# lucidrains/DALLE-pytorch

Hardware: NVIDIA B200
Metric: DALL-E fwd+bwd tokens/sec at seq=1280, dim=1024 (higher is better)
Workload: dtype bf16

## Files before the change

dalle_pytorch_b200/_lib.py:

```python
import ctypes
import os
import subprocess
import threading

_HERE = os.path.dirname(os.path.abspath(__file__))
LIB_PATH = os.environ.get('DALLE_B200_LIB') or os.path.join(_HERE, 'libdalle_b200.so')
CSRC = os.path.join(_HERE, 'csrc')

c_int, c_float, c_void_p, c_int64 = ctypes.c_int, ctypes.c_float, ctypes.c_void_p, ctypes.c_int64

F32, BF16 = 0, 1
ATTN_FULL, ATTN_AXIAL_ROW, ATTN_AXIAL_COL, ATTN_CONV_LIKE, ATTN_STATIC = 0, 1, 2, 3, 4
EPI_STORE, EPI_QKV, EPI_RESID, EPI_GEGLU, EPI_GEGLU_BWD = 0, 1, 2, 3, 4
GEMM_AUTO, GEMM_SIMT, GEMM_TCGEN05, GEMM_SMALLM = 0, 1, 2, 3


class LnShiftFwdParams(ctypes.Structure):
    _fields_ = [('batch', c_int), ('n', c_int), ('d', c_int), ('text_len', c_int), ('fmap', c_int),
                ('do_ln', c_int), ('do_shift', c_int), ('out_dtype', c_int), ('eps', c_float),
                ('x', c_void_p), ('gamma', c_void_p), ('beta', c_void_p), ('out', c_void_p),
                ('mean', c_void_p), ('rstd', c_void_p)]


class LnShiftBwdParams(ctypes.Structure):
    _fields_ = [('batch', c_int), ('n', c_int), ('d', c_int), ('text_len', c_int), ('fmap', c_int),
                ('do_ln', c_int), ('do_shift', c_int), ('dout_dtype', c_int),
                ('d_out', c_void_p), ('x', c_void_p), ('mean', c_void_p), ('rstd', c_void_p), ('gamma', c_void_p),
                ('dres', c_void_p), ('dx', c_void_p), ('dgamma', c_void_p), ('dbeta', c_void_p),
                ('up_y', c_void_p), ('up_scale', c_void_p), ('up_sign', c_float), ('up_dy', c_void_p), ('up_dscale', c_void_p),
                ('up_dbias', c_void_p)]


class GemmParams(ctypes.Structure):
    _fields_ = [('M', c_int), ('N', c_int), ('K', c_int), ('dtype', c_int), ('backend', c_int),
                ('A', c_void_p), ('lda', c_int64), ('a_mn_major', c_int),
                ('B', c_void_p), ('ldb', c_int64), ('b_mn_major', c_int),
                ('epilogue', c_int),
                ('C', c_void_p), ('ldc', c_int64), ('c_dtype', c_int), ('bias', c_void_p), ('split_k_ok', c_int),
                ('C_multicast', c_void_p), ('c_scale', c_float),
                ('q', c_void_p), ('k', c_void_p), ('v', c_void_p), ('cos_t', c_void_p), ('sin_t', c_void_p),
                ('seq_n', c_int), ('heads', c_int), ('dim_head', c_int), ('pos_offset', c_int), ('q_scale', c_float),
                ('resid', c_void_p), ('scale', c_void_p), ('sign', c_float), ('y_out', c_void_p), ('out', c_void_p),
                ('u_out', c_void_p), ('h_out', c_void_p), ('hidden', c_int), ('u_in', c_void_p), ('du_out', c_void_p)]


class AttnFwdParams(ctypes.Structure):
    _fields_ = [('batch', c_int), ('heads', c_int), ('n_q', c_int), ('n_k', c_int), ('dim_head', c_int),
                ('dtype', c_int), ('pattern', c_int), ('causal', c_int), ('stable', c_int),
                ('text_len', c_int), ('fmap', c_int), ('kernel_size', c_int), ('dilation', c_int), ('gather', c_int), ('kv_rows', c_int),
                ('key_mask', c_void_p), ('static_mask', c_void_p), ('static_ld', c_int64),
                ('q', c_void_p), ('k', c_void_p), ('v', c_void_p), ('out', c_void_p), ('lse', c_void_p)]


class AttnBwdParams(ctypes.Structure):
    _fields_ = [('f', AttnFwdParams), ('d_out', c_void_p), ('cos_t', c_void_p), ('sin_t', c_void_p),
                ('q_scale', c_float), ('delta', c_void_p), ('dqkv', c_void_p)]


class ScaleBwdParams(ctypes.Structure):
    _fields_ = [('rows', c_int), ('d', c_int), ('dtype', c_int), ('sign', c_float),
                ('d_out', c_void_p), ('y', c_void_p), ('scale', c_void_p), ('dy', c_void_p),
                ('dscale', c_void_p), ('dbias', c_void_p)]


class AdamParams(ctypes.Structure):
    _fields_ = [('p', c_void_p), ('g', c_void_p), ('m', c_void_p), ('v', c_void_p), ('count', c_int64),
                ('lr', c_float), ('beta1', c_float), ('beta2', c_float), ('eps', c_float), ('weight_decay', c_float),
                ('step', c_int), ('max_norm', c_float), ('gnorm_sq', c_void_p)]


_STRUCTS = (LnShiftFwdParams, LnShiftBwdParams, GemmParams, AttnFwdParams, AttnBwdParams, ScaleBwdParams, AdamParams)

_lib = None
_lock = threading.Lock()


def build(force=False, verbose=False):
    if force:
        for f in os.listdir(os.path.join(CSRC, 'build')) if os.path.isdir(os.path.join(CSRC, 'build')) else []:
            if f.endswith('.o'):
                os.remove(os.path.join(CSRC, 'build', f))
    r = subprocess.run(['bash', os.path.join(CSRC, 'build.sh')], capture_output=True, text=True)
    if verbose or r.returncode != 0:
        print(r.stdout)
        print(r.stderr)
    if r.returncode != 0:
        raise RuntimeError('building libdalle_b200.so failed:\n' + r.stdout + r.stderr)
    return LIB_PATH


def _declare(lib):
    lib.dalle_b200_version.restype = c_int
    lib.dalle_b200_last_error.restype = ctypes.c_char_p
    lib.dalle_b200_device_ok.argtypes = [c_int]
    lib.dalle_b200_abi_sizes.argtypes = [ctypes.POINTER(c_int), c_int]
    for name, st in (('ln_shift_fwd', LnShiftFwdParams), ('ln_shift_bwd', LnShiftBwdParams), ('gemm', GemmParams),
                     ('attn_fwd', AttnFwdParams), ('attn_bwd', AttnBwdParams), ('scale_bwd', ScaleBwdParams)):
        fn = getattr(lib, 'dalle_b200_' + name)
        fn.argtypes = [ctypes.POINTER(st), c_void_p]
        fn.restype = c_int
    lib.dalle_b200_gemm_select.argtypes = [ctypes.POINTER(GemmParams)]
    lib.dalle_b200_gemm_select.restype = c_int
    lib.dalle_b200_colsum.argtypes = [c_void_p, c_int, c_int, c_int, c_void_p, c_void_p]
    lib.dalle_b200_qkv_rotary.argtypes = [c_void_p, c_void_p, c_void_p, c_void_p, c_void_p, c_void_p, c_int, c_int, c_int, c_int, c_int, c_int, c_float, c_int, c_void_p]
    lib.dalle_b200_geglu_bwd.argtypes = [c_void_p, c_void_p, c_void_p, c_void_p, c_int, c_int, c_int, c_void_p]
    lib.dalle_b200_ce_fwd.argtypes = [c_void_p, c_int, c_int, c_int, c_void_p, c_float, c_void_p, c_void_p, c_void_p]
    lib.dalle_b200_ce_bwd.argtypes = [c_void_p, c_int, c_int, c_int, c_void_p, c_float, c_void_p, c_void_p, c_void_p]
    lib.dalle_b200_cast_bf16.argtypes = [c_void_p, c_void_p, c_int64, c_void_p]
    lib.dalle_b200_mc_add.argtypes = [c_void_p, c_void_p, c_int64, c_float, c_void_p]
    lib.dalle_b200_split_bf16x3.argtypes = [c_void_p, c_void_p, c_int64, c_int, c_int, c_int, c_void_p]
    lib.dalle_b200_resid_scale.argtypes = [c_void_p, c_int, c_void_p, c_void_p, c_float, c_void_p, c_int64, c_int, c_void_p]
    lib.dalle_b200_sample_topk_gumbel.argtypes = [c_void_p, c_int, c_int, c_int, c_int64, c_int, c_float, c_void_p, ctypes.c_uint64, ctypes.c_uint64, c_void_p, c_void_p]
    lib.dalle_b200_sample_guided_topk_gumbel.argtypes = [c_void_p, c_void_p, c_int, c_int, c_int, c_int64, c_float, c_int, c_float, c_void_p, ctypes.c_uint64, ctypes.c_uint64,
                                                          c_void_p, c_void_p]
    lib.dalle_b200_decode_shift.argtypes = [c_void_p, c_void_p, c_int, c_int, c_int, c_void_p, c_void_p, c_void_p, c_int, c_int, c_void_p]
    lib.dalle_b200_decode_kv_append.argtypes = [c_void_p, c_void_p, c_void_p, c_void_p, c_int, c_int, c_int, c_int, c_void_p, c_void_p]
    lib.dalle_b200_dropout.argtypes = [c_void_p, c_void_p, c_int, c_int64, c_float, ctypes.c_uint64, ctypes.c_uint64, c_void_p]
    lib.dalle_b200_geglu_fwd.argtypes = [c_void_p, c_void_p, c_int64, c_int, c_void_p]
    lib.dalle_b200_axpby.argtypes = [c_void_p, c_void_p, c_float, c_void_p, c_int64, c_void_p]
    lib.dalle_b200_sumsq.argtypes = [c_void_p, c_int64, c_void_p, c_void_p]
    lib.dalle_b200_adam.argtypes = [ctypes.POINTER(AdamParams), c_void_p]
    lib.dalle_b200_embed_fwd.argtypes = [c_void_p, c_void_p, c_void_p, c_int, c_int, c_int, c_int, c_int, c_int, c_void_p]
    lib.dalle_b200_embed_bwd.argtypes = [c_void_p, c_void_p, c_void_p, c_int, c_int, c_int, c_int, c_int, c_int, c_void_p]
    sizes = (c_int * 8)()
    n = lib.dalle_b200_abi_sizes(sizes, 8)
    assert n == len(_STRUCTS)
    for i, st in enumerate(_STRUCTS):
        if ctypes.sizeof(st) != sizes[i]:
            raise RuntimeError(f'ABI mismatch for {st.__name__}: ctypes {ctypes.sizeof(st)} vs C {sizes[i]}')


def lib():
    global _lib
    if _lib is not None:
        return _lib
    with _lock:
        if _lib is None:
            if not os.path.exists(LIB_PATH):
                build()
            l = ctypes.CDLL(LIB_PATH)
            _declare(l)
            _lib = l
    return _lib


def check(rc, what=''):
    if rc != 0:
        msg = lib().dalle_b200_last_error().decode('utf-8', 'replace')
        raise RuntimeError(f'libdalle_b200 {what} failed (status {rc}): {msg}')


EXPORTED = ['dalle_b200_version', 'dalle_b200_last_error', 'dalle_b200_device_ok', 'dalle_b200_abi_sizes',
            'dalle_b200_ln_shift_fwd', 'dalle_b200_ln_shift_bwd', 'dalle_b200_gemm', 'dalle_b200_gemm_select', 'dalle_b200_attn_fwd',
            'dalle_b200_attn_bwd', 'dalle_b200_scale_bwd', 'dalle_b200_colsum', 'dalle_b200_qkv_rotary', 'dalle_b200_geglu_bwd', 'dalle_b200_ce_fwd', 'dalle_b200_ce_bwd', 'dalle_b200_cast_bf16', 'dalle_b200_mc_add', 'dalle_b200_split_bf16x3', 'dalle_b200_resid_scale', 'dalle_b200_dropout', 'dalle_b200_sample_topk_gumbel', 'dalle_b200_sample_guided_topk_gumbel', 'dalle_b200_decode_shift', 'dalle_b200_decode_kv_append', 'dalle_b200_geglu_fwd',
            'dalle_b200_axpby', 'dalle_b200_embed_fwd', 'dalle_b200_embed_bwd', 'dalle_b200_sumsq', 'dalle_b200_adam', 'dalle_b200_debug_attn_timeline']
```

dalle_pytorch_b200/csrc/api.cu:

```cuda
#include <cstdarg>
#include <cstdlib>
#include <cstring>
#include <mutex>

#include "common.cuh"

namespace db200 {
bool pdl_enabled() {
  static const bool on = [] { const char* v = std::getenv("DALLE_B200_PDL"); return !(v && v[0] == '0'); }();
  return on;
}

std::string& last_error_slot() {
  static thread_local std::string s;
  return s;
}

int set_error(int code, const char* fmt, ...) {
  char buf[1024];
  va_list ap;
  va_start(ap, fmt);
  vsnprintf(buf, sizeof(buf), fmt, ap);
  va_end(ap);
  last_error_slot() = buf;
  return code;
}

int sm_count() {
  static std::atomic<int> cached[64];
  int dev = 0;
  if (cudaGetDevice(&dev) != cudaSuccess || dev < 0 || dev >= 64) return 148;
  if (cached[dev] == 0) {
    int n = 0;
    if (cudaDeviceGetAttribute(&n, cudaDevAttrMultiProcessorCount, dev) != cudaSuccess || n <= 0) n = 148;
    cached[dev] = n;
  }
  return cached[dev];
}

int ln_shift_fwd_launch(const db200_ln_shift_fwd_params& P, cudaStream_t st);
int ln_shift_bwd_launch(const db200_ln_shift_bwd_params& P, cudaStream_t st);
int scale_bwd_launch(const db200_scale_bwd_params& P, cudaStream_t st);
int colsum_launch(const void* x, int dtype, int rows, int cols, float* out, cudaStream_t st);
int ce_fwd_launch(const void* logits, int dtype, int rows, int vocab, const long long* labels, float coef, float* row_lse, float* loss_acc, cudaStream_t st);
int ce_bwd_launch(void* logits, int dtype, int rows, int vocab, const long long* labels, float coef, const float* row_lse, const float* upstream, cudaStream_t st);
int qkv_rotary_launch(const void* qkv, void* q, void* k, void* v, const float* cos_t, const float* sin_t, int dtype, int rows, int seq_n, int heads,
                      int dh, int pos_offset, float q_scale, int n_alloc, cudaStream_t st);
int geglu_bwd_launch(const void* dh, const void* u, void* du, float* dbias, int dtype, int rows, int hidden, cudaStream_t st);
int cast_bf16_launch(const float* src, void* dst, int64_t count, cudaStream_t st);
int split_bf16x3_launch(const float* src, void* dst, int64_t rows, int cols, int concat_rows, int pat, cudaStream_t st);
int resid_scale_launch(const void* y, int dtype, const float* resid, const float* scale, float sign, float* out, int64_t rows, int d, cudaStream_t st);
int mc_add_launch(const float* src, void* mc_dst, int64_t count, float scale, cudaStream_t st);
int sample_topk_gumbel_launch(const void* logits, int dtype, int rows, int vocab, long long ld, int k, float temperature, const float* gumbel,
                              unsigned long long seed, unsigned long long offset, long long* out, cudaStream_t st);
int sample_guided_topk_gumbel_launch(const void* cond, const void* null_logits, int dtype, int rows, int vocab, long long ld, float cond_scale, int k,
                                     float temperature, const float* gumbel, unsigned long long seed, unsigned long long offset, long long* out,
                                     cudaStream_t st);
int dropout_launch(const void* x, void* y, int dtype, int64_t count, float p, unsigned long long seed, unsigned long long offset, cudaStream_t st);
int geglu_fwd_launch(const float* u, float* h, int64_t rows, int hidden, cudaStream_t st);
int axpby_launch(const float* a, const float* b, float alpha, float* y, int64_t count, cudaStream_t st);
int sumsq_launch(const float* x, int64_t count, float* out, cudaStream_t st);
int adam_launch(const db200_adam_params& P, cudaStream_t st);
int embed_launch(bool bwd, const long long* ids, const float* a, float* o, int batch, int seg_len, int n, int seg_off, int d, int vocab, cudaStream_t st);
int gemm_simt_launch(const db200_gemm_params& p, cudaStream_t st);
bool gemm_tcgen05_supported(const db200_gemm_params& p, const char** why);
int gemm_tcgen05_launch(const db200_gemm_params& p, cudaStream_t st);
bool gemm_smallm_supported(const db200_gemm_params& p, const char** why);
int gemm_smallm_launch(const db200_gemm_params& p, cudaStream_t st);
int attn_fwd_simt_launch(const db200_attn_fwd_params& p, cudaStream_t st);
int attn_bwd_simt_launch(const db200_attn_bwd_params& p, cudaStream_t st);
bool attn_mma_supported(const db200_attn_fwd_params& p);
int attn_fwd_mma_launch(const db200_attn_fwd_params& p, cudaStream_t st);
int attn_bwd_mma_launch(const db200_attn_bwd_params& p, cudaStream_t st);
bool attn_tc_supported(const db200_attn_fwd_params& p);
bool attn_gather_ok(const db200_attn_fwd_params& p, const char** why);
int attn_fwd_tc_launch(const db200_attn_fwd_params& p, cudaStream_t st);
int attn_bwd_tc_launch(const db200_attn_bwd_params& p, cudaStream_t st);
int attn_debug_timeline(long long* out, int count);
bool attn_decode_supported(const db200_attn_fwd_params& p);
int attn_decode_launch(const db200_attn_fwd_params& p, cudaStream_t st);
int decode_shift_launch(const float* h, void* y, int out_dtype, int batch, int d, float* ring_top, float* ring_left, const long long* pos,
                        int text_len, int fmap, cudaStream_t st);
int decode_kv_append_launch(const void* k_new, const void* v_new, void* k_cache, void* v_cache, int dtype, int bh, int dh, int kv_rows,
                            const long long* pos, cudaStream_t st);

static bool dtype_ok(int d) { return d == DB200_F32 || d == DB200_BF16; }
static bool aligned16(const void* p) { return (reinterpret_cast<uintptr_t>(p) & 15) == 0; }

static int env_choice(const char* name, const char* a, const char* b) {
  const char* v = getenv(name);
  if (!v) return 0;
  if (!strcmp(v, a)) return 1;
  if (!strcmp(v, b)) return 2;
  return 0;
}

}

using namespace db200;

extern "C" {

int dalle_b200_version(void) { return DALLE_B200_VERSION; }
int dalle_b200_debug_attn_timeline(long long* out, int count) { return db200::attn_debug_timeline(out, count); }

const char* dalle_b200_last_error(void) { return last_error_slot().c_str(); }

int dalle_b200_device_ok(int dev) {
  cudaDeviceProp prop;
  if (cudaGetDeviceProperties(&prop, dev) != cudaSuccess) return 0;
  return prop.major == 10 ? 1 : 0;
}

int dalle_b200_abi_sizes(int* out, int capacity) {
  const int sizes[7] = {(int)sizeof(db200_ln_shift_fwd_params), (int)sizeof(db200_ln_shift_bwd_params), (int)sizeof(db200_gemm_params),
                        (int)sizeof(db200_attn_fwd_params),     (int)sizeof(db200_attn_bwd_params),     (int)sizeof(db200_scale_bwd_params),
                        (int)sizeof(db200_adam_params)};
  for (int i = 0; i < 7 && i < capacity; ++i) out[i] = sizes[i];
  return 7;
}

int dalle_b200_ln_shift_fwd(const db200_ln_shift_fwd_params* p, void* stream) {
  DB200_CHECK_ARG(p != nullptr, "ln_shift_fwd: null params");
  DB200_CHECK_ARG(p->batch >= 0 && p->n >= 0 && p->d > 0, "ln_shift_fwd: bad shape b=%d n=%d d=%d", p->batch, p->n, p->d);
  DB200_CHECK_ARG(dtype_ok(p->out_dtype), "ln_shift_fwd: bad dtype %d", p->out_dtype);
  DB200_CHECK_ARG(p->d % (p->do_shift ? 16 : 4) == 0, "ln_shift_fwd: d=%d must be a multiple of %d", p->d, p->do_shift ? 16 : 4);
  DB200_CHECK_ARG(p->x && p->out, "ln_shift_fwd: null tensor");
  DB200_CHECK_ARG(aligned16(p->x) && aligned16(p->out), "ln_shift_fwd: tensors must be 16-byte aligned");
  if (p->do_ln) DB200_CHECK_ARG(p->gamma && p->beta && p->mean && p->rstd, "ln_shift_fwd: LayerNorm needs gamma/beta/mean/rstd");
  if (p->do_shift) {
    DB200_CHECK_ARG(p->fmap > 0 && p->text_len > 0, "ln_shift_fwd: shift needs text_len/fmap");
    DB200_CHECK_ARG(p->n >= p->text_len, "ln_shift_fwd: n=%d < text_len=%d is the no-shift case (transformer.py:160)", p->n, p->text_len);
    DB200_CHECK_ARG(p->n <= p->text_len + p->fmap * p->fmap, "ln_shift_fwd: n=%d exceeds text_len + fmap^2", p->n);
  }
  return ln_shift_fwd_launch(*p, (cudaStream_t)stream);
}

int dalle_b200_ln_shift_bwd(const db200_ln_shift_bwd_params* p, void* stream) {
  DB200_CHECK_ARG(p != nullptr, "ln_shift_bwd: null params");
  DB200_CHECK_ARG(p->batch >= 0 && p->n >= 0 && p->d > 0, "ln_shift_bwd: bad shape");
  DB200_CHECK_ARG(dtype_ok(p->dout_dtype), "ln_shift_bwd: bad dtype %d", p->dout_dtype);
  DB200_CHECK_ARG(p->d % (p->do_shift ? 16 : 4) == 0, "ln_shift_bwd: d=%d alignment", p->d);
  DB200_CHECK_ARG(p->d_out && p->dx, "ln_shift_bwd: null tensor");
  if (p->do_ln) DB200_CHECK_ARG(p->x && p->mean && p->rstd && p->gamma && p->dgamma && p->dbeta, "ln_shift_bwd: LayerNorm needs x/mean/rstd/gamma/dgamma/dbeta");
  if (p->do_shift) DB200_CHECK_ARG(p->fmap > 0 && p->n >= p->text_len && p->n <= p->text_len + p->fmap * p->fmap, "ln_shift_bwd: bad shift geometry");
  if (p->up_dy) {
    DB200_CHECK_ARG(p->d == 1024, "ln_shift_bwd: the fused upstream LayerScale adjoint needs d = 1024 (got %d)", p->d);
    DB200_CHECK_ARG(aligned16(p->up_dy) && aligned16(p->up_y) && aligned16(p->d_out) && aligned16(p->x) && aligned16(p->dres),
                    "ln_shift_bwd: fused path needs 16-byte aligned tensors");
    DB200_CHECK_ARG(p->up_dscale == nullptr || p->up_y != nullptr, "ln_shift_bwd: up_dscale needs up_y");
  }
  return ln_shift_bwd_launch(*p, (cudaStream_t)stream);
}

int dalle_b200_gemm(const db200_gemm_params* p, void* stream) {
  DB200_CHECK_ARG(p != nullptr, "gemm: null params");
  DB200_CHECK_ARG(p->M >= 0 && p->N > 0 && p->K > 0, "gemm: bad shape M=%d N=%d K=%d", p->M, p->N, p->K);
  DB200_CHECK_ARG(dtype_ok(p->dtype), "gemm: bad dtype %d", p->dtype);
  DB200_CHECK_ARG(p->A && p->B, "gemm: null operand");
  DB200_CHECK_ARG((p->N & 1) == 0, "gemm: N=%d must be even (epilogues work on column pairs)", p->N);
  switch (p->epilogue) {
    case DB200_EPI_STORE:
      DB200_CHECK_ARG(p->C && dtype_ok(p->c_dtype) && (p->ldc & 1) == 0, "gemm/STORE: bad C");
      if (p->C_multicast)
        DB200_CHECK_ARG(p->c_dtype == DB200_F32 && p->bias == nullptr && aligned16(p->C_multicast) && (p->ldc & 3) == 0 && p->backend != DB200_GEMM_SIMT,
                        "gemm/STORE: the multicast reduction needs an fp32 result, no bias, 16-byte aligned rows and the tcgen05 kernel");
      break;
    case DB200_EPI_QKV:
      DB200_CHECK_ARG(p->q && p->k && p->v, "gemm/QKV: null q/k/v");
      DB200_CHECK_ARG(p->heads > 0 && p->dim_head > 0 && (p->dim_head & 1) == 0 && p->N == 3 * p->heads * p->dim_head,
                      "gemm/QKV: N=%d != 3*heads*dim_head (%d*%d)", p->N, p->heads, p->dim_head);
      DB200_CHECK_ARG(p->seq_n > 0 && p->M % p->seq_n == 0, "gemm/QKV: M=%d not a multiple of seq_n=%d", p->M, p->seq_n);
      DB200_CHECK_ARG((p->cos_t == nullptr) == (p->sin_t == nullptr), "gemm/QKV: cos/sin tables must come together");
      break;
    case DB200_EPI_RESID:
      DB200_CHECK_ARG(p->out != nullptr, "gemm/RESID: null out");
      break;
    case DB200_EPI_GEGLU:
      DB200_CHECK_ARG(p->h_out && p->hidden > 0 && p->N == 2 * p->hidden && (p->hidden & 1) == 0, "gemm/GEGLU: N must equal 2*hidden");
      break;
    case DB200_EPI_GEGLU_BWD:
      DB200_CHECK_ARG(p->u_in && p->du_out && p->hidden == p->N, "gemm/GEGLU_BWD: N must equal hidden");
      break;
    default:
      return set_error(DB200_ERR_BAD_ARG, "gemm: unknown epilogue %d", p->epilogue);
  }
  if (p->M == 0) return DB200_OK;
  int backend = p->backend;
  if (backend == DB200_GEMM_SMALLM) {
    const char* why = "";
    if (!gemm_smallm_supported(*p, &why)) return set_error(DB200_ERR_UNSUPPORTED, "gemm: the small-M kernel cannot run this problem: %s", why);
    return gemm_smallm_launch(*p, (cudaStream_t)stream);
  }
  if (backend == DB200_GEMM_AUTO) {
    const int env = env_choice("DALLE_B200_GEMM", "simt", "tcgen05");
    if (env == 1) backend = DB200_GEMM_SIMT;
    else {
      const char* why = nullptr;
      backend = gemm_tcgen05_supported(*p, &why) ? DB200_GEMM_TCGEN05 : DB200_GEMM_SIMT;
    }
  }
  if (p->C_multicast && backend != DB200_GEMM_TCGEN05)
    return set_error(DB200_ERR_UNSUPPORTED, "gemm/STORE: the multicast reduction is implemented by the tcgen05 kernel only (shape / alignment did not qualify)");
  if (backend == DB200_GEMM_TCGEN05) {
    const char* why = "";
    if (!gemm_tcgen05_supported(*p, &why)) return set_error(DB200_ERR_UNSUPPORTED, "gemm: tcgen05 backend cannot run this problem: %s", why);
    return gemm_tcgen05_launch(*p, (cudaStream_t)stream);
  }
  return gemm_simt_launch(*p, (cudaStream_t)stream);
}

int dalle_b200_gemm_select(const db200_gemm_params* p) {
  if (!p) return DB200_GEMM_SIMT;
  if (p->backend != DB200_GEMM_AUTO) return p->backend;
  if (env_choice("DALLE_B200_GEMM", "simt", "tcgen05") == 1) return DB200_GEMM_SIMT;
  const char* why = nullptr;
  return gemm_tcgen05_supported(*p, &why) ? DB200_GEMM_TCGEN05 : DB200_GEMM_SIMT;
}

static int attn_backend(const db200_attn_fwd_params& f) {
  const char* v = getenv("DALLE_B200_ATTN");
  int want = 2;
  if (f.gather) return 2;
  if (v) want = !strcmp(v, "simt") ? 0 : !strcmp(v, "tc") ? 2 : 1;
  if (want == 2 && !attn_tc_supported(f)) want = 1;
  if (want == 1 && !attn_mma_supported(f)) want = 0;
  return want;
}

static int check_attn(const db200_attn_fwd_params& f, const char* who) {
  DB200_CHECK_ARG(f.batch >= 0 && f.heads > 0 && f.n_q >= 0 && f.n_k >= f.n_q, "%s: bad shape", who);
  if (f.dim_head != 64) return set_error(DB200_ERR_UNSUPPORTED, "%s: dim_head=%d, kernels are specialised for 64", who, f.dim_head);
  DB200_CHECK_ARG(dtype_ok(f.dtype), "%s: bad dtype", who);
  DB200_CHECK_ARG(f.q && f.k && f.v && f.out && f.lse, "%s: null tensor", who);
  DB200_CHECK_ARG(f.pattern >= DB200_ATTN_FULL && f.pattern <= DB200_ATTN_STATIC, "%s: bad pattern %d", who, f.pattern);
  if (f.pattern == DB200_ATTN_STATIC) DB200_CHECK_ARG(f.static_mask && f.static_ld >= f.n_k, "%s: STATIC needs static_mask", who);
  if (f.pattern == DB200_ATTN_AXIAL_ROW || f.pattern == DB200_ATTN_AXIAL_COL || f.pattern == DB200_ATTN_CONV_LIKE)
    DB200_CHECK_ARG(f.fmap > 0 && f.text_len > 0, "%s: sparse pattern needs text_len / fmap", who);
  if (f.pattern == DB200_ATTN_CONV_LIKE) DB200_CHECK_ARG(f.kernel_size > 0 && (f.kernel_size & 1) && f.dilation > 0, "%s: conv_like kernel_size must be odd", who);
  DB200_CHECK_ARG(f.kv_rows == 0 || (f.kv_rows >= f.n_k && !f.gather), "%s: kv_rows must be >= n_k (and is not combined with gather)", who);
  if (f.gather) {
    const char* why = nullptr;
    if (!attn_gather_ok(f, &why)) return set_error(DB200_ERR_UNSUPPORTED, "%s: %s", who, why);
    if (!attn_tc_supported(f)) return set_error(DB200_ERR_UNSUPPORTED, "%s: gathered axial attention needs the tcgen05 path (sm_100, 16-byte aligned tensors)", who);
  }
  return DB200_OK;
}

int dalle_b200_attn_fwd(const db200_attn_fwd_params* p, void* stream) {
  DB200_CHECK_ARG(p != nullptr, "attn_fwd: null params");
  const int rc = check_attn(*p, "attn_fwd");
  if (rc) return rc;
  if (p->batch == 0 || p->n_q == 0) return DB200_OK;
  if (attn_decode_supported(*p)) return attn_decode_launch(*p, (cudaStream_t)stream);
  const int be = attn_backend(*p);
  if (be == 2) return attn_fwd_tc_launch(*p, (cudaStream_t)stream);
  if (be == 1) return attn_fwd_mma_launch(*p, (cudaStream_t)stream);
  return attn_fwd_simt_launch(*p, (cudaStream_t)stream);
}

int dalle_b200_attn_bwd(const db200_attn_bwd_params* p, void* stream) {
  DB200_CHECK_ARG(p != nullptr, "attn_bwd: null params");
  const int rc = check_attn(p->f, "attn_bwd");
  if (rc) return rc;
  DB200_CHECK_ARG(p->f.kv_rows == 0 || p->f.kv_rows == p->f.n_k, "attn_bwd: kv_rows (in-place KV cache) is a forward-only layout");
  DB200_CHECK_ARG(p->f.n_q == p->f.n_k, "attn_bwd: training only (n_q == n_k)");
  DB200_CHECK_ARG(p->d_out && p->delta && p->dqkv, "attn_bwd: null tensor");
  DB200_CHECK_ARG((p->cos_t == nullptr) == (p->sin_t == nullptr), "attn_bwd: cos/sin tables must come together");
  if (p->f.batch == 0 || p->f.n_q == 0) return DB200_OK;
  const int be = attn_backend(p->f);
  if (be == 2) return attn_bwd_tc_launch(*p, (cudaStream_t)stream);
  if (be == 1) return attn_bwd_mma_launch(*p, (cudaStream_t)stream);
  return attn_bwd_simt_launch(*p, (cudaStream_t)stream);
}

int dalle_b200_scale_bwd(const db200_scale_bwd_params* p, void* stream) {
  DB200_CHECK_ARG(p != nullptr, "scale_bwd: null params");
  DB200_CHECK_ARG(p->rows >= 0 && p->d > 0 && (p->d & 1) == 0, "scale_bwd: bad shape");
  DB200_CHECK_ARG(dtype_ok(p->dtype) && p->d_out && p->dy, "scale_bwd: bad args");
  return scale_bwd_launch(*p, (cudaStream_t)stream);
}

int dalle_b200_colsum(const void* x, int dtype, int rows, int cols, float* out, void* stream) {
  DB200_CHECK_ARG(x && out && rows >= 0 && cols > 0 && (cols & 1) == 0 && dtype_ok(dtype), "colsum: bad args");
  return colsum_launch(x, dtype, rows, cols, out, (cudaStream_t)stream);
}

int dalle_b200_geglu_bwd(const void* dh, const void* u, void* du, float* dbias, int dtype, int rows, int hidden, void* stream) {
  DB200_CHECK_ARG(dh && u && du && rows >= 0 && hidden > 0 && (hidden & 7) == 0 && dtype_ok(dtype), "geglu_bwd: bad args (hidden must be a multiple of 8)");
  DB200_CHECK_ARG(aligned16(dh) && aligned16(u) && aligned16(du), "geglu_bwd: tensors must be 16-byte aligned");
  return geglu_bwd_launch(dh, u, du, dbias, dtype, rows, hidden, (cudaStream_t)stream);
}

int dalle_b200_qkv_rotary(const void* qkv, void* q, void* k, void* v, const float* cos_t, const float* sin_t, int dtype, int rows, int seq_n,
                          int heads, int dim_head, int pos_offset, float q_scale, int n_alloc, void* stream) {
  if (n_alloc == 0) n_alloc = seq_n;
  DB200_CHECK_ARG(n_alloc >= seq_n, "qkv_rotary: n_alloc must be >= seq_n");
  DB200_CHECK_ARG(qkv && q && k && v && dtype_ok(dtype) && rows >= 0 && seq_n > 0 && heads > 0 && dim_head > 0 && (dim_head & 7) == 0 &&
                      rows % seq_n == 0,
                  "qkv_rotary: bad args (dim_head must be a multiple of 8, rows a multiple of seq_n)");
  DB200_CHECK_ARG((cos_t == nullptr) == (sin_t == nullptr), "qkv_rotary: cos/sin tables must come together");
  DB200_CHECK_ARG(aligned16(qkv) && aligned16(q) && aligned16(k) && aligned16(v) && (!cos_t || (aligned16(cos_t) && aligned16(sin_t))),
                  "qkv_rotary: tensors must be 16-byte aligned");
  return qkv_rotary_launch(qkv, q, k, v, cos_t, sin_t, dtype, rows, seq_n, heads, dim_head, pos_offset, q_scale, n_alloc, (cudaStream_t)stream);
}

int dalle_b200_split_bf16x3(const float* src, void* dst, int64_t rows, int cols, int concat_rows, int operand, void* stream) {
  DB200_CHECK_ARG(src && dst && rows >= 0 && cols > 0 && (cols & 1) == 0 && (operand == 0 || operand == 1), "split_bf16x3: bad args (cols must be even)");
  DB200_CHECK_ARG(aligned16(src) && aligned16(dst), "split_bf16x3: tensors must be 16-byte aligned");
  const int pat = operand == 0 ? 0x201100 : 0x021010;
  return split_bf16x3_launch(src, dst, rows, cols, concat_rows != 0, pat, (cudaStream_t)stream);
}

int dalle_b200_resid_scale(const void* y, int dtype, const float* resid, const float* scale, float sign, float* out, int64_t rows, int d, void* stream) {
  DB200_CHECK_ARG(y && out && rows >= 0 && d > 0 && (d & 1) == 0 && dtype_ok(dtype), "resid_scale: bad args (d must be even)");
  return resid_scale_launch(y, dtype, resid, scale, sign, out, rows, d, (cudaStream_t)stream);
}

int dalle_b200_mc_add(const float* src, void* mc_dst, int64_t count, float scale, void* stream) {
  DB200_CHECK_ARG(src && mc_dst && count >= 0 && aligned16(src) && aligned16(mc_dst), "mc_add: bad args (16-byte aligned fp32 buffers)");
  return mc_add_launch(src, mc_dst, count, scale, (cudaStream_t)stream);
}

int dalle_b200_sample_topk_gumbel(const void* logits, int dtype, int rows, int vocab, int64_t ld, int k, float temperature, const float* gumbel,
                                  uint64_t seed, uint64_t offset, int64_t* out, void* stream) {
  DB200_CHECK_ARG(logits && out && rows >= 0 && vocab > 0 && ld >= vocab && dtype_ok(dtype), "sample_topk_gumbel: bad args");
  DB200_CHECK_ARG(k >= 1 && k <= vocab && temperature > 0.f, "sample_topk_gumbel: need 1 <= k <= vocab and temperature > 0");
  if ((size_t)vocab * 4 > 200 * 1024) return set_error(DB200_ERR_UNSUPPORTED, "sample_topk_gumbel: vocab=%d does not fit the shared-memory row buffer", vocab);
  return sample_topk_gumbel_launch(logits, dtype, rows, vocab, ld, k, temperature, gumbel, seed, offset, reinterpret_cast<long long*>(out), (cudaStream_t)stream);
}

int dalle_b200_sample_guided_topk_gumbel(const void* cond, const void* null_logits, int dtype, int rows, int vocab, int64_t ld, float cond_scale, int k,
                                         float temperature, const float* gumbel, uint64_t seed, uint64_t offset, int64_t* out, void* stream) {
  DB200_CHECK_ARG(cond && null_logits && out && rows >= 0 && vocab > 0 && ld >= vocab && dtype_ok(dtype), "sample_guided_topk_gumbel: bad args");
  DB200_CHECK_ARG(k >= 1 && k <= vocab && temperature > 0.f, "sample_guided_topk_gumbel: need 1 <= k <= vocab and temperature > 0");
  if ((size_t)vocab * 4 > 200 * 1024) return set_error(DB200_ERR_UNSUPPORTED, "sample_guided_topk_gumbel: vocab=%d does not fit the shared-memory row buffer", vocab);
  return sample_guided_topk_gumbel_launch(cond, null_logits, dtype, rows, vocab, ld, cond_scale, k, temperature, gumbel, seed, offset,
                                          reinterpret_cast<long long*>(out), (cudaStream_t)stream);
}

int dalle_b200_decode_shift(const float* h, void* y, int out_dtype, int batch, int d, float* ring_top, float* ring_left, const int64_t* pos,
                            int text_len, int fmap, void* stream) {
  DB200_CHECK_ARG(h && y && ring_top && ring_left && pos && dtype_ok(out_dtype), "decode_shift: null tensor / bad dtype");
  DB200_CHECK_ARG(batch >= 0 && d > 0 && (d & 3) == 0 && fmap > 0 && text_len >= 0, "decode_shift: bad shape (d must be a multiple of 4)");
  return decode_shift_launch(h, y, out_dtype, batch, d, ring_top, ring_left, reinterpret_cast<const long long*>(pos), text_len, fmap, (cudaStream_t)stream);
}

int dalle_b200_decode_kv_append(const void* k_new, const void* v_new, void* k_cache, void* v_cache, int dtype, int batch_heads, int dim_head,
                                int kv_rows, const int64_t* pos, void* stream) {
  DB200_CHECK_ARG(k_new && v_new && k_cache && v_cache && pos && dtype_ok(dtype), "decode_kv_append: null tensor / bad dtype");
  DB200_CHECK_ARG(batch_heads >= 0 && dim_head > 0 && kv_rows > 0, "decode_kv_append: bad shape");
  return decode_kv_append_launch(k_new, v_new, k_cache, v_cache, dtype, batch_heads, dim_head, kv_rows, reinterpret_cast<const long long*>(pos), (cudaStream_t)stream);
}

int dalle_b200_dropout(const void* x, void* y, int dtype, int64_t count, float p, uint64_t seed, uint64_t offset, void* stream) {
  DB200_CHECK_ARG(x && y && count >= 0 && dtype_ok(dtype) && p >= 0.f && p <= 1.f, "dropout: bad args (0 <= p <= 1)");
  return dropout_launch(x, y, dtype, count, p, seed, offset, (cudaStream_t)stream);
}

int dalle_b200_geglu_fwd(const float* u, float* h, int64_t rows, int hidden, void* stream) {
  DB200_CHECK_ARG(u && h && rows >= 0 && hidden > 0, "geglu_fwd: bad args");
  return geglu_fwd_launch(u, h, rows, hidden, (cudaStream_t)stream);
}

int dalle_b200_ce_fwd(const void* logits, int dtype, int rows, int vocab, const int64_t* labels, float coef, float* row_lse, float* loss_acc,
                      void* stream) {
  DB200_CHECK_ARG(logits && labels && row_lse && loss_acc && rows >= 0 && vocab > 0 && (vocab & 7) == 0 && dtype_ok(dtype),
                  "ce_fwd: bad args (vocab must be a multiple of 8)");
  DB200_CHECK_ARG(aligned16(logits), "ce_fwd: logits must be 16-byte aligned");
  return ce_fwd_launch(logits, dtype, rows, vocab, reinterpret_cast<const long long*>(labels), coef, row_lse, loss_acc, (cudaStream_t)stream);
}

int dalle_b200_ce_bwd(void* logits, int dtype, int rows, int vocab, const int64_t* labels, float coef, const float* row_lse, const float* upstream,
                      void* stream) {
  DB200_CHECK_ARG(logits && labels && row_lse && upstream && rows >= 0 && vocab > 0 && (vocab & 7) == 0 && dtype_ok(dtype), "ce_bwd: bad args");
  DB200_CHECK_ARG(aligned16(logits), "ce_bwd: logits must be 16-byte aligned");
  return ce_bwd_launch(logits, dtype, rows, vocab, reinterpret_cast<const long long*>(labels), coef, row_lse, upstream, (cudaStream_t)stream);
}

int dalle_b200_cast_bf16(const float* src, void* dst, int64_t count, void* stream) {
  DB200_CHECK_ARG(src && dst && count >= 0, "cast_bf16: bad args");
  DB200_CHECK_ARG(aligned16(src) && (reinterpret_cast<uintptr_t>(dst) & 7) == 0, "cast_bf16: alignment");
  return cast_bf16_launch(src, dst, count, (cudaStream_t)stream);
}

int dalle_b200_sumsq(const float* x, int64_t count, float* out, void* stream) {
  DB200_CHECK_ARG(x && out && count >= 0, "sumsq: bad args");
  DB200_CHECK_ARG(aligned16(x), "sumsq: x must be 16-byte aligned");
  return sumsq_launch(x, count, out, (cudaStream_t)stream);
}
int dalle_b200_adam(const db200_adam_params* p, void* stream) {
  DB200_CHECK_ARG(p != nullptr, "adam: null params");
  DB200_CHECK_ARG(p->p && p->g && p->m && p->v && p->count >= 0, "adam: null tensor / bad count");
  DB200_CHECK_ARG(aligned16(p->p) && aligned16(p->g) && aligned16(p->m) && aligned16(p->v), "adam: buffers must be 16-byte aligned");
  DB200_CHECK_ARG(p->step >= 1 && p->beta1 >= 0.f && p->beta1 < 1.f && p->beta2 >= 0.f && p->beta2 < 1.f && p->eps > 0.f, "adam: bad hyper-parameters");
  DB200_CHECK_ARG(p->max_norm <= 0.f || p->gnorm_sq != nullptr, "adam: clipping needs the gradient-norm scalar");
  return adam_launch(*p, (cudaStream_t)stream);
}
int dalle_b200_embed_fwd(const int64_t* ids, const float* weight, float* out, int batch, int seg_len, int n, int seg_off, int d, int vocab,
                         void* stream) {
  DB200_CHECK_ARG(ids && weight && out, "embed_fwd: null pointer");
  DB200_CHECK_ARG(batch >= 0 && seg_len >= 0 && n > 0 && seg_off >= 0 && seg_off + seg_len <= n && vocab > 0, "embed_fwd: bad geometry");
  DB200_CHECK_ARG(d > 0 && d % 4 == 0 && aligned16(weight) && aligned16(out), "embed_fwd: d must be a multiple of 4, pointers 16-byte aligned");
  return embed_launch(false, reinterpret_cast<const long long*>(ids), weight, out, batch, seg_len, n, seg_off, d, vocab, (cudaStream_t)stream);
}
int dalle_b200_embed_bwd(const int64_t* ids, const float* d_out, float* dweight, int batch, int seg_len, int n, int seg_off, int d, int vocab,
                         void* stream) {
  DB200_CHECK_ARG(ids && d_out && dweight, "embed_bwd: null pointer");
  DB200_CHECK_ARG(batch >= 0 && seg_len >= 0 && n > 0 && seg_off >= 0 && seg_off + seg_len <= n && vocab > 0, "embed_bwd: bad geometry");
  DB200_CHECK_ARG(d > 0 && d % 4 == 0 && aligned16(d_out) && aligned16(dweight), "embed_bwd: d must be a multiple of 4, pointers 16-byte aligned");
  return embed_launch(true, reinterpret_cast<const long long*>(ids), d_out, dweight, batch, seg_len, n, seg_off, d, vocab, (cudaStream_t)stream);
}
int dalle_b200_axpby(const float* a, const float* b, float alpha, float* y, int64_t count, void* stream) {
  DB200_CHECK_ARG(a && b && y && count >= 0, "axpby: bad args");
  DB200_CHECK_ARG(aligned16(a) && aligned16(b) && aligned16(y), "axpby: alignment");
  return axpby_launch(a, b, alpha, y, count, (cudaStream_t)stream);
}

}
```

dalle_pytorch_b200/csrc/common.cuh:

```cuda
#pragma once
#include <cuda_runtime.h>
#include <cuda_bf16.h>
#include <stdint.h>
#include <stdio.h>
#include <atomic>
#include <string>

#include "../../include/dalle_b200.h"

namespace db200 {

std::string& last_error_slot();
int set_error(int code, const char* fmt, ...);

#define DB200_CHECK_ARG(cond, ...)                                                   \
  do {                                                                               \
    if (!(cond)) return ::db200::set_error(DB200_ERR_BAD_ARG, __VA_ARGS__);          \
  } while (0)

#define DB200_CUDA_OK(expr)                                                          \
  do {                                                                               \
    cudaError_t _e = (expr);                                                         \
    if (_e != cudaSuccess)                                                           \
      return ::db200::set_error(DB200_ERR_CUDA, "%s failed: %s (%s:%d)", #expr,      \
                                cudaGetErrorString(_e), __FILE__, __LINE__);         \
  } while (0)

#define DB200_LAUNCH_OK(what)                                                        \
  do {                                                                               \
    cudaError_t _e = cudaGetLastError();                                             \
    if (_e != cudaSuccess)                                                           \
      return ::db200::set_error(DB200_ERR_CUDA, "launch of %s failed: %s", what,     \
                                cudaGetErrorString(_e));                             \
  } while (0)

__device__ __forceinline__ float to_f32(float v) { return v; }
__device__ __forceinline__ float to_f32(__nv_bfloat16 v) { return __bfloat162float(v); }

template <typename T> __device__ __forceinline__ T from_f32(float v);
template <> __device__ __forceinline__ float from_f32<float>(float v) { return v; }
template <> __device__ __forceinline__ __nv_bfloat16 from_f32<__nv_bfloat16>(float v) { return __float2bfloat16_rn(v); }

template <typename T> __device__ __forceinline__ void store2(T* p, float a, float b);
template <> __device__ __forceinline__ void store2<float>(float* p, float a, float b) {
  *reinterpret_cast<float2*>(p) = make_float2(a, b);
}
template <> __device__ __forceinline__ void store2<__nv_bfloat16>(__nv_bfloat16* p, float a, float b) {
  *reinterpret_cast<__nv_bfloat162*>(p) = __floats2bfloat162_rn(a, b);
}

template <typename T> __device__ __forceinline__ float2 load2(const T* p);
template <> __device__ __forceinline__ float2 load2<float>(const float* p) { return *reinterpret_cast<const float2*>(p); }
template <> __device__ __forceinline__ float2 load2<__nv_bfloat16>(const __nv_bfloat16* p) {
  return __bfloat1622float2(*reinterpret_cast<const __nv_bfloat162*>(p));
}

__device__ __forceinline__ float gelu_erf(float g) { return 0.5f * g * (1.0f + erff(g * 0.70710678118654752440f)); }
__device__ __forceinline__ float gelu_erf_grad(float g) {
  const float cdf = 0.5f * (1.0f + erff(g * 0.70710678118654752440f));
  const float pdf = 0.39894228040143267794f * expf(-0.5f * g * g);
  return cdf + g * pdf;
}

__device__ __forceinline__ void gelu_fast(float g, float& gelu, float& dgelu) {
  const float x = g * 0.70710678118654752440f;
  const float ax = fabsf(x);
  float t;
  asm("rcp.approx.ftz.f32 %0, %1;" : "=f"(t) : "f"(fmaf(0.3275911f, ax, 1.0f)));
  const float ex = __expf(-ax * ax);
  float poly = fmaf(t, 1.061405429f, -1.453152027f);
  poly = fmaf(t, poly, 1.421413741f);
  poly = fmaf(t, poly, -0.284496736f);
  poly = fmaf(t, poly, 0.254829592f);
  const float erf_abs = fmaf(-poly * t, ex, 1.0f);
  const float cdf = fmaf(0.5f, copysignf(erf_abs, x), 0.5f);
  gelu = g * cdf;
  dgelu = fmaf(g * 0.39894228040143267794f, ex, cdf);
}
__device__ __forceinline__ float2 fma2(float2 a, float2 b, float2 c) {
  float2 d;
  asm("{\n\t.reg .b64 ra, rb, rc, rd;\n\tmov.b64 ra, {%2, %3};\n\tmov.b64 rb, {%4, %5};\n\tmov.b64 rc, {%6, %7};\n\t"
      "fma.rn.f32x2 rd, ra, rb, rc;\n\tmov.b64 {%0, %1}, rd;\n\t}"
      : "=f"(d.x), "=f"(d.y)
      : "f"(a.x), "f"(a.y), "f"(b.x), "f"(b.y), "f"(c.x), "f"(c.y));
  return d;
}
__device__ __forceinline__ float2 mul2(float2 a, float2 b) {
  float2 d;
  asm("{\n\t.reg .b64 ra, rb, rd;\n\tmov.b64 ra, {%2, %3};\n\tmov.b64 rb, {%4, %5};\n\tmul.f32x2 rd, ra, rb;\n\tmov.b64 {%0, %1}, rd;\n\t}"
      : "=f"(d.x), "=f"(d.y)
      : "f"(a.x), "f"(a.y), "f"(b.x), "f"(b.y));
  return d;
}
__device__ __forceinline__ float2 add2(float2 a, float2 b) {
  float2 d;
  asm("{\n\t.reg .b64 ra, rb, rd;\n\tmov.b64 ra, {%2, %3};\n\tmov.b64 rb, {%4, %5};\n\tadd.f32x2 rd, ra, rb;\n\tmov.b64 {%0, %1}, rd;\n\t}"
      : "=f"(d.x), "=f"(d.y)
      : "f"(a.x), "f"(a.y), "f"(b.x), "f"(b.y));
  return d;
}
__device__ __forceinline__ float2 splat2(float v) { return make_float2(v, v); }

__device__ __forceinline__ void gelu_fast2(float2 g, float2& gelu, float2& dgelu) {
  const float2 x = mul2(g, splat2(0.70710678118654752440f));
  const float2 ax = make_float2(fabsf(x.x), fabsf(x.y));
  const float2 den = fma2(ax, splat2(0.3275911f), splat2(1.0f));
  float2 t, ex;
  asm("rcp.approx.ftz.f32 %0, %1;" : "=f"(t.x) : "f"(den.x));
  asm("rcp.approx.ftz.f32 %0, %1;" : "=f"(t.y) : "f"(den.y));
  const float2 q = mul2(mul2(ax, ax), splat2(-1.4426950408889634f));
  asm("ex2.approx.ftz.f32 %0, %1;" : "=f"(ex.x) : "f"(q.x));
  asm("ex2.approx.ftz.f32 %0, %1;" : "=f"(ex.y) : "f"(q.y));
  float2 poly = fma2(t, splat2(1.061405429f), splat2(-1.453152027f));
  poly = fma2(t, poly, splat2(1.421413741f));
  poly = fma2(t, poly, splat2(-0.284496736f));
  poly = fma2(t, poly, splat2(0.254829592f));
  const float2 m = mul2(mul2(poly, t), ex);
  const float2 erf_abs = fma2(m, splat2(-1.0f), splat2(1.0f));
  const float2 cs = make_float2(copysignf(erf_abs.x, x.x), copysignf(erf_abs.y, x.y));
  const float2 cdf = fma2(cs, splat2(0.5f), splat2(0.5f));
  gelu = mul2(g, cdf);
  dgelu = fma2(mul2(g, splat2(0.39894228040143267794f)), ex, cdf);
}

template <typename T> __device__ __forceinline__ void gelu_pair(float g, float& gelu, float& dgelu);
template <> __device__ __forceinline__ void gelu_pair<float>(float g, float& gelu, float& dgelu) { gelu = gelu_erf(g); dgelu = gelu_erf_grad(g); }
template <> __device__ __forceinline__ void gelu_pair<__nv_bfloat16>(float g, float& gelu, float& dgelu) { gelu_fast(g, gelu, dgelu); }
template <typename T> __device__ __forceinline__ float gelu_fwd(float g);
template <> __device__ __forceinline__ float gelu_fwd<float>(float g) { return gelu_erf(g); }
template <> __device__ __forceinline__ float gelu_fwd<__nv_bfloat16>(float g) { float a, b; gelu_fast(g, a, b); return a; }
template <typename T> __device__ __forceinline__ void gelu_pair2(float2 g, float2& gelu, float2& dgelu);
template <> __device__ __forceinline__ void gelu_pair2<float>(float2 g, float2& gelu, float2& dgelu) {
  gelu = make_float2(gelu_erf(g.x), gelu_erf(g.y)); dgelu = make_float2(gelu_erf_grad(g.x), gelu_erf_grad(g.y));
}
template <> __device__ __forceinline__ void gelu_pair2<__nv_bfloat16>(float2 g, float2& gelu, float2& dgelu) { gelu_fast2(g, gelu, dgelu); }

__device__ __forceinline__ float warp_sum(float v) {
#pragma unroll
  for (int o = 16; o > 0; o >>= 1) v += __shfl_xor_sync(0xffffffffu, v, o);
  return v;
}
__device__ __forceinline__ float warp_max(float v) {
#pragma unroll
  for (int o = 16; o > 0; o >>= 1) v = fmaxf(v, __shfl_xor_sync(0xffffffffu, v, o));
  return v;
}

__device__ __forceinline__ void pdl_wait() { asm volatile("griddepcontrol.wait;" ::: "memory"); }
__device__ __forceinline__ void pdl_launch() { asm volatile("griddepcontrol.launch_dependents;" ::: "memory"); }
bool pdl_enabled();
template <typename... KArgs, typename... Args>
inline cudaError_t launch_pdl(void (*kern)(KArgs...), dim3 grid, dim3 block, size_t smem, cudaStream_t st, Args&&... args) {
  cudaLaunchConfig_t cfg = {};
  cfg.gridDim = grid; cfg.blockDim = block; cfg.dynamicSmemBytes = smem; cfg.stream = st;
  cudaLaunchAttribute attr[1];
  attr[0].id = cudaLaunchAttributeProgrammaticStreamSerialization;
  attr[0].val.programmaticStreamSerializationAllowed = pdl_enabled() ? 1 : 0;
  cfg.attrs = attr; cfg.numAttrs = 1;
  return cudaLaunchKernelEx(&cfg, kern, static_cast<KArgs>(args)...);
}

inline int ceil_div(int a, int b) { return (a + b - 1) / b; }
inline int64_t ceil_div64(int64_t a, int64_t b) { return (a + b - 1) / b; }

int sm_count();

}
```

dalle_pytorch_b200/csrc/epilogue.cuh:

```cuda
#pragma once
#include <cstdlib>
#include <cstring>

#include "common.cuh"

namespace db200 {

struct EpiArgs {
  int M, N;
  void* C; long long ldc; int c_is_f32; const float* bias; int atomic_c;
  float c_scale;
  int tma_store;
  void* q; void* k; void* v; const float* cos_t; const float* sin_t;
  int seq_n, heads, dim_head, pos_offset; float q_scale;
  const float* resid; const float* scale; float sign; void* y_out; float* out;
  void* u_out; void* h_out; int hidden; const void* u_in; void* du_out;
};

inline EpiArgs make_epi_args(const db200_gemm_params& p) {
  EpiArgs e;
  e.M = p.M; e.N = p.N;
  e.C = p.C; e.ldc = p.ldc; e.c_is_f32 = (p.c_dtype == DB200_F32); e.bias = p.bias; e.atomic_c = 0; e.c_scale = 1.0f; e.tma_store = 0;
  if (p.C_multicast) { e.C = p.C_multicast; e.atomic_c = 2; e.c_scale = p.c_scale; }
  static const int dbg = [] { const char* v = getenv("DALLE_B200_GEMM_DBG"); return !v ? 0 : !strcmp(v, "nostore") ? 3 : !strcmp(v, "noepi") ? 4 : 0; }();
  if (dbg && p.epilogue == DB200_EPI_STORE && !p.C_multicast) e.atomic_c = dbg;
  e.q = p.q; e.k = p.k; e.v = p.v; e.cos_t = p.cos_t; e.sin_t = p.sin_t;
  e.seq_n = p.seq_n; e.heads = p.heads; e.dim_head = p.dim_head; e.pos_offset = p.pos_offset; e.q_scale = p.q_scale;
  e.resid = p.resid; e.scale = p.scale; e.sign = p.sign; e.y_out = p.y_out; e.out = p.out;
  e.u_out = p.u_out; e.h_out = p.h_out; e.hidden = p.hidden; e.u_in = p.u_in; e.du_out = p.du_out;
  return e;
}

__device__ __forceinline__ void mc_red_add_v4(float* mc, float a, float b, float c, float d) {
  asm volatile("multimem.red.relaxed.sys.global.add.v4.f32 [%0], {%1, %2, %3, %4};" ::"l"(mc), "f"(a), "f"(b), "f"(c), "f"(d) : "memory");
}
__device__ __forceinline__ void mc_red_add_v2(float* mc, float a, float b) {
  asm volatile("multimem.red.relaxed.sys.global.add.v2.f32 [%0], {%1, %2};" ::"l"(mc), "f"(a), "f"(b) : "memory");
}

template <typename T>
__device__ __forceinline__ void epi_store_pair(const EpiArgs& e, int m, int n, float v0, float v1) {
  if (e.bias) { const float2 bb = __ldg(reinterpret_cast<const float2*>(e.bias + n)); v0 += bb.x; v1 += bb.y; }
  const long long off = (long long)m * e.ldc + n;
  if (e.c_is_f32) store2<float>(reinterpret_cast<float*>(e.C) + off, v0, v1);
  else            store2<T>(reinterpret_cast<T*>(e.C) + off, v0, v1);
}

template <typename T>
__device__ __forceinline__ void epi_qkv_pair(const EpiArgs& e, int m, int n, float v0, float v1) {
  const int inner = e.heads * e.dim_head;
  const int which = n / inner;
  const int rem = n - which * inner;
  const int head = rem / e.dim_head;
  const int d = rem - head * e.dim_head;
  const int b = m / e.seq_n;
  const int p = m - b * e.seq_n;
  if (e.cos_t) {
    const int ti = (p + e.pos_offset) * (e.dim_head >> 1) + (d >> 1);
    const float c = __ldg(e.cos_t + ti), s = __ldg(e.sin_t + ti);
    const float r0 = v0 * c + (-v1) * s;
    const float r1 = v1 * c + v0 * s;
    v0 = r0; v1 = r1;
  }
  if (which == 0) { v0 *= e.q_scale; v1 *= e.q_scale; }
  T* base = reinterpret_cast<T*>(which == 0 ? e.q : (which == 1 ? e.k : e.v));
  const long long off = (((long long)b * e.heads + head) * e.seq_n + p) * e.dim_head + d;
  store2<T>(base + off, v0, v1);
}

template <typename T>
__device__ __forceinline__ void epi_resid_pair(const EpiArgs& e, int m, int n, float v0, float v1) {
  if (e.bias) { const float2 bb = __ldg(reinterpret_cast<const float2*>(e.bias + n)); v0 += bb.x; v1 += bb.y; }
  const long long off = (long long)m * e.N + n;
  if (e.y_out) store2<T>(reinterpret_cast<T*>(e.y_out) + off, v0, v1);
  float s0 = e.sign, s1 = e.sign;
  if (e.scale) { const float2 sc = __ldg(reinterpret_cast<const float2*>(e.scale + n)); s0 *= sc.x; s1 *= sc.y; }
  float r0 = 0.f, r1 = 0.f;
  if (e.resid) { const float2 r = *reinterpret_cast<const float2*>(e.resid + off); r0 = r.x; r1 = r.y; }
  *reinterpret_cast<float2*>(e.out + off) = make_float2(r0 + s0 * v0, r1 + s1 * v1);
}

template <typename T>
__device__ __forceinline__ void epi_geglu_pair(const EpiArgs& e, int m, int j, float a0, float a1, float g0, float g1) {
  if (e.bias) {
    const float2 ba = __ldg(reinterpret_cast<const float2*>(e.bias + j));
    const float2 bg = __ldg(reinterpret_cast<const float2*>(e.bias + e.hidden + j));
    a0 += ba.x; a1 += ba.y;
    g0 += bg.x; g1 += bg.y;
  }
  if (e.u_out) {
    T* u = reinterpret_cast<T*>(e.u_out) + (long long)m * (2 * e.hidden);
    store2<T>(u + j, a0, a1);
    store2<T>(u + e.hidden + j, g0, g1);
  }
  T* h = reinterpret_cast<T*>(e.h_out) + (long long)m * e.hidden;
  store2<T>(h + j, a0 * gelu_fwd<T>(g0), a1 * gelu_fwd<T>(g1));
}

template <typename T>
__device__ __forceinline__ void epi_geglu_bwd_pair(const EpiArgs& e, int m, int j, float d0, float d1) {
  const T* u = reinterpret_cast<const T*>(e.u_in) + (long long)m * (2 * e.hidden);
  const float2 a = load2<T>(u + j);
  const float2 g = load2<T>(u + e.hidden + j);
  T* du = reinterpret_cast<T*>(e.du_out) + (long long)m * (2 * e.hidden);
  float f0, f1, df0, df1;
  gelu_pair<T>(g.x, f0, df0);
  gelu_pair<T>(g.y, f1, df1);
  store2<T>(du + j, d0 * f0, d1 * f1);
  store2<T>(du + e.hidden + j, d0 * a.x * df0, d1 * a.y * df1);
}

template <int EPI, typename T>
__device__ __forceinline__ void epi_pair(const EpiArgs& e, int m, int n, float v0, float v1) {
  if constexpr (EPI == DB200_EPI_STORE) epi_store_pair<T>(e, m, n, v0, v1);
  else if constexpr (EPI == DB200_EPI_QKV) epi_qkv_pair<T>(e, m, n, v0, v1);
  else if constexpr (EPI == DB200_EPI_RESID) epi_resid_pair<T>(e, m, n, v0, v1);
  else if constexpr (EPI == DB200_EPI_GEGLU_BWD) epi_geglu_bwd_pair<T>(e, m, n, v0, v1);
}


template <typename T> struct Vec8;
template <> struct Vec8<__nv_bfloat16> {
  static __device__ __forceinline__ void store(__nv_bfloat16* p, const float* v) {
    uint4 u;
    __nv_bfloat162 a = __floats2bfloat162_rn(v[0], v[1]), b = __floats2bfloat162_rn(v[2], v[3]);
    __nv_bfloat162 c = __floats2bfloat162_rn(v[4], v[5]), d = __floats2bfloat162_rn(v[6], v[7]);
    u.x = *reinterpret_cast<uint32_t*>(&a); u.y = *reinterpret_cast<uint32_t*>(&b);
    u.z = *reinterpret_cast<uint32_t*>(&c); u.w = *reinterpret_cast<uint32_t*>(&d);
    *reinterpret_cast<uint4*>(p) = u;
  }
  static __device__ __forceinline__ void load(const __nv_bfloat16* p, float* v) {
    const uint4 u = *reinterpret_cast<const uint4*>(p);
    const float2 a = __bfloat1622float2(*reinterpret_cast<const __nv_bfloat162*>(&u.x));
    const float2 b = __bfloat1622float2(*reinterpret_cast<const __nv_bfloat162*>(&u.y));
    const float2 c = __bfloat1622float2(*reinterpret_cast<const __nv_bfloat162*>(&u.z));
    const float2 d = __bfloat1622float2(*reinterpret_cast<const __nv_bfloat162*>(&u.w));
    v[0] = a.x; v[1] = a.y; v[2] = b.x; v[3] = b.y; v[4] = c.x; v[5] = c.y; v[6] = d.x; v[7] = d.y;
  }
};
template <> struct Vec8<float> {
  static __device__ __forceinline__ void store(float* p, const float* v) {
    *reinterpret_cast<float4*>(p) = make_float4(v[0], v[1], v[2], v[3]);
    *reinterpret_cast<float4*>(p + 4) = make_float4(v[4], v[5], v[6], v[7]);
  }
  static __device__ __forceinline__ void load(const float* p, float* v) {
    const float4 a = *reinterpret_cast<const float4*>(p), b = *reinterpret_cast<const float4*>(p + 4);
    v[0] = a.x; v[1] = a.y; v[2] = a.z; v[3] = a.w; v[4] = b.x; v[5] = b.y; v[6] = b.z; v[7] = b.w;
  }
};

__device__ __forceinline__ void st_global_v8(void* p, const uint32_t* w) {
  asm volatile("st.global.v8.b32 [%0], {%1, %2, %3, %4, %5, %6, %7, %8};" ::"l"(p), "r"(w[0]), "r"(w[1]), "r"(w[2]), "r"(w[3]), "r"(w[4]), "r"(w[5]),
               "r"(w[6]), "r"(w[7])
               : "memory");
}
template <typename T>
__device__ __forceinline__ bool epi_store16(const EpiArgs& e, int m, int n, const uint32_t* acc) {
  if (e.atomic_c != 0) return false;
  const long long off = (long long)m * e.ldc + n;
  float v[16];
#pragma unroll
  for (int i = 0; i < 16; ++i) v[i] = __uint_as_float(acc[i]);
  if (e.bias) {
#pragma unroll
    for (int i = 0; i < 16; i += 4) {
      const float4 bb = __ldg(reinterpret_cast<const float4*>(e.bias + n + i));
      v[i] += bb.x; v[i + 1] += bb.y; v[i + 2] += bb.z; v[i + 3] += bb.w;
    }
  }
  if (e.c_is_f32) {
    float* c = reinterpret_cast<float*>(e.C) + off;
    if (reinterpret_cast<uintptr_t>(c) & 31) return false;
    uint32_t w[8];
#pragma unroll
    for (int h = 0; h < 2; ++h) {
#pragma unroll
      for (int i = 0; i < 8; ++i) w[i] = __float_as_uint(v[8 * h + i]);
      st_global_v8(c + 8 * h, w);
    }
  } else {
    T* c = reinterpret_cast<T*>(e.C) + off;
    if (reinterpret_cast<uintptr_t>(c) & 31) return false;
    uint32_t w[8];
#pragma unroll
    for (int i = 0; i < 8; ++i) {
      const __nv_bfloat162 b2 = __floats2bfloat162_rn(v[2 * i], v[2 * i + 1]);
      w[i] = *reinterpret_cast<const uint32_t*>(&b2);
    }
    st_global_v8(c, w);
  }
  return true;
}

__device__ __forceinline__ void ld_global_v8(const void* p, uint32_t* w) {
  asm volatile("ld.global.v8.b32 {%0, %1, %2, %3, %4, %5, %6, %7}, [%8];"
               : "=r"(w[0]), "=r"(w[1]), "=r"(w[2]), "=r"(w[3]), "=r"(w[4]), "=r"(w[5]), "=r"(w[6]), "=r"(w[7])
               : "l"(p));
}
template <typename T>
__device__ __forceinline__ void epi_resid16(const EpiArgs& e, int m, int n, const uint32_t* acc) {
  const long long off = (long long)m * e.N + n;
  float v[16];
#pragma unroll
  for (int i = 0; i < 16; ++i) v[i] = __uint_as_float(acc[i]);
  if (e.bias) {
#pragma unroll
    for (int i = 0; i < 16; i += 4) {
      const float4 bb = __ldg(reinterpret_cast<const float4*>(e.bias + n + i));
      v[i] += bb.x; v[i + 1] += bb.y; v[i + 2] += bb.z; v[i + 3] += bb.w;
    }
  }
  uint32_t rr[16];
  if (e.resid) { ld_global_v8(e.resid + off, rr); ld_global_v8(e.resid + off + 8, rr + 8); }
  if (e.y_out) {
    uint32_t w[8];
#pragma unroll
    for (int i = 0; i < 8; ++i) {
      const __nv_bfloat162 b2 = __floats2bfloat162_rn(v[2 * i], v[2 * i + 1]);
      w[i] = *reinterpret_cast<const uint32_t*>(&b2);
    }
    st_global_v8(reinterpret_cast<T*>(e.y_out) + off, w);
  }
  uint32_t o[16];
#pragma unroll
  for (int i = 0; i < 16; i += 4) {
    float4 sc = make_float4(1.f, 1.f, 1.f, 1.f);
    if (e.scale) sc = __ldg(reinterpret_cast<const float4*>(e.scale + n + i));
    const float s4[4] = {sc.x, sc.y, sc.z, sc.w};
#pragma unroll
    for (int k = 0; k < 4; ++k) {
      const float r = e.resid ? __uint_as_float(rr[i + k]) : 0.f;
      o[i + k] = __float_as_uint(r + e.sign * s4[k] * v[i + k]);
    }
  }
  st_global_v8(e.out + off, o);
  st_global_v8(e.out + off + 8, o + 8);
}

template <typename T>
__device__ __forceinline__ void epi_geglu16(const EpiArgs& e, int m, int j, const uint32_t* acc_a, const uint32_t* acc_g) {
  float a[16], g[16];
#pragma unroll
  for (int i = 0; i < 16; ++i) { a[i] = __uint_as_float(acc_a[i]); g[i] = __uint_as_float(acc_g[i]); }
  if (e.bias) {
#pragma unroll
    for (int i = 0; i < 16; i += 4) {
      const float4 ba = __ldg(reinterpret_cast<const float4*>(e.bias + j + i));
      const float4 bg = __ldg(reinterpret_cast<const float4*>(e.bias + e.hidden + j + i));
      a[i] += ba.x; a[i + 1] += ba.y; a[i + 2] += ba.z; a[i + 3] += ba.w;
      g[i] += bg.x; g[i + 1] += bg.y; g[i + 2] += bg.z; g[i + 3] += bg.w;
    }
  }
  uint32_t w[8];
  if (e.u_out) {
    T* u = reinterpret_cast<T*>(e.u_out) + (long long)m * (2 * e.hidden);
#pragma unroll
    for (int i = 0; i < 8; ++i) { const __nv_bfloat162 b2 = __floats2bfloat162_rn(a[2 * i], a[2 * i + 1]); w[i] = *reinterpret_cast<const uint32_t*>(&b2); }
    st_global_v8(u + j, w);
#pragma unroll
    for (int i = 0; i < 8; ++i) { const __nv_bfloat162 b2 = __floats2bfloat162_rn(g[2 * i], g[2 * i + 1]); w[i] = *reinterpret_cast<const uint32_t*>(&b2); }
    st_global_v8(u + e.hidden + j, w);
  }
#pragma unroll
  for (int i = 0; i < 8; ++i) {
    float2 f, df;
    gelu_pair2<T>(make_float2(g[2 * i], g[2 * i + 1]), f, df);
    const __nv_bfloat162 b2 = __floats2bfloat162_rn(a[2 * i] * f.x, a[2 * i + 1] * f.y);
    w[i] = *reinterpret_cast<const uint32_t*>(&b2);
  }
  st_global_v8(reinterpret_cast<T*>(e.h_out) + (long long)m * e.hidden + j, w);
}

template <int EPI, typename T>
__device__ __forceinline__ void epi_vec8(const EpiArgs& e, int m, int n, float* v) {
  if constexpr (EPI == DB200_EPI_STORE) {
    if (e.bias) {
      float bb[8]; Vec8<float>::load(e.bias + n, bb);
#pragma unroll
      for (int i = 0; i < 8; ++i) v[i] += bb[i];
    }
    const long long off = (long long)m * e.ldc + n;
    if (e.atomic_c >= 3) return;
    if (e.atomic_c == 2) {
      float* c = reinterpret_cast<float*>(e.C) + off;
      mc_red_add_v4(c, v[0] * e.c_scale, v[1] * e.c_scale, v[2] * e.c_scale, v[3] * e.c_scale);
      mc_red_add_v4(c + 4, v[4] * e.c_scale, v[5] * e.c_scale, v[6] * e.c_scale, v[7] * e.c_scale);
    } else if (e.atomic_c) {
      float* c = reinterpret_cast<float*>(e.C) + off;
#pragma unroll
      for (int i = 0; i < 8; ++i) atomicAdd(c + i, v[i]);
    } else if (e.c_is_f32) Vec8<float>::store(reinterpret_cast<float*>(e.C) + off, v);
    else Vec8<T>::store(reinterpret_cast<T*>(e.C) + off, v);
  } else if constexpr (EPI == DB200_EPI_QKV) {
    const int inner = e.heads * e.dim_head;
    const int which = n / inner;
    const int rem = n - which * inner;
    const int head = rem / e.dim_head;
    const int d = rem - head * e.dim_head;
    const int b = m / e.seq_n;
    const int p = m - b * e.seq_n;
    if (e.cos_t) {
      const int ti = (p + e.pos_offset) * (e.dim_head >> 1) + (d >> 1);
      const float4 c = *reinterpret_cast<const float4*>(e.cos_t + ti);
      const float4 s = *reinterpret_cast<const float4*>(e.sin_t + ti);
      const float cc[4] = {c.x, c.y, c.z, c.w}, ss[4] = {s.x, s.y, s.z, s.w};
#pragma unroll
      for (int i = 0; i < 4; ++i) {
        const float x0 = v[2 * i], x1 = v[2 * i + 1];
        v[2 * i] = x0 * cc[i] + (-x1) * ss[i];
        v[2 * i + 1] = x1 * cc[i] + x0 * ss[i];
      }
    }
    if (which == 0) {
#pragma unroll
      for (int i = 0; i < 8; ++i) v[i] *= e.q_scale;
    }
    T* base = reinterpret_cast<T*>(which == 0 ? e.q : (which == 1 ? e.k : e.v));
    Vec8<T>::store(base + (((long long)b * e.heads + head) * e.seq_n + p) * e.dim_head + d, v);
  } else if constexpr (EPI == DB200_EPI_RESID) {
    if (e.bias) {
      float bb[8]; Vec8<float>::load(e.bias + n, bb);
#pragma unroll
      for (int i = 0; i < 8; ++i) v[i] += bb[i];
    }
    const long long off = (long long)m * e.N + n;
    if (e.y_out) Vec8<T>::store(reinterpret_cast<T*>(e.y_out) + off, v);
    float sc[8], rr[8];
    if (e.scale) Vec8<float>::load(e.scale + n, sc);
    if (e.resid) Vec8<float>::load(e.resid + off, rr);
#pragma unroll
    for (int i = 0; i < 8; ++i) {
      const float s = e.scale ? e.sign * sc[i] : e.sign;
      const float r = e.resid ? rr[i] : 0.f;
      v[i] = r + s * v[i];
    }
    Vec8<float>::store(e.out + off, v);
  } else if constexpr (EPI == DB200_EPI_GEGLU_BWD) {
    const T* u = reinterpret_cast<const T*>(e.u_in) + (long long)m * (2 * e.hidden);
    float a[8], g[8], da[8], dg[8];
    Vec8<T>::load(u + n, a);
    Vec8<T>::load(u + e.hidden + n, g);
#pragma unroll
    for (int i = 0; i < 8; ++i) {
      float f, df;
      gelu_pair<T>(g[i], f, df);
      da[i] = v[i] * f;
      dg[i] = v[i] * a[i] * df;
    }
    T* du = reinterpret_cast<T*>(e.du_out) + (long long)m * (2 * e.hidden);
    Vec8<T>::store(du + n, da);
    Vec8<T>::store(du + e.hidden + n, dg);
  }
}

template <typename T>
__device__ __forceinline__ void epi_geglu_vec8(const EpiArgs& e, int m, int j, float* a, float* g) {
  if (e.bias) {
    float ba[8], bg[8];
    Vec8<float>::load(e.bias + j, ba);
    Vec8<float>::load(e.bias + e.hidden + j, bg);
#pragma unroll
    for (int i = 0; i < 8; ++i) { a[i] += ba[i]; g[i] += bg[i]; }
  }
  if (e.u_out) {
    T* u = reinterpret_cast<T*>(e.u_out) + (long long)m * (2 * e.hidden);
    Vec8<T>::store(u + j, a);
    Vec8<T>::store(u + e.hidden + j, g);
  }
  float h[8];
#pragma unroll
  for (int i = 0; i < 8; ++i) h[i] = a[i] * gelu_fwd<T>(g[i]);
  Vec8<T>::store(reinterpret_cast<T*>(e.h_out) + (long long)m * e.hidden + j, h);
}


template <int EPI, typename T>
__device__ __forceinline__ void epi_chunk_cols(const EpiArgs& e, int mbase, int n, const float* t, int M) {
  if constexpr (EPI == DB200_EPI_STORE) {
    float b0 = 0.f, b1 = 0.f;
    if (e.bias) { const float2 bb = __ldg(reinterpret_cast<const float2*>(e.bias + n)); b0 = bb.x; b1 = bb.y; }
#pragma unroll
    for (int it = 0; it < 16; ++it) {
      const int m = mbase + 2 * it;
      if (m < M) {
        const long long off = (long long)m * e.ldc + n;
        if (e.atomic_c == 2) mc_red_add_v2(reinterpret_cast<float*>(e.C) + off, t[2 * it] * e.c_scale, t[2 * it + 1] * e.c_scale);
        else if (e.atomic_c) { atomicAdd(reinterpret_cast<float*>(e.C) + off, t[2 * it]); atomicAdd(reinterpret_cast<float*>(e.C) + off + 1, t[2 * it + 1]); }
        else if (e.c_is_f32) store2<float>(reinterpret_cast<float*>(e.C) + off, t[2 * it] + b0, t[2 * it + 1] + b1);
        else store2<T>(reinterpret_cast<T*>(e.C) + off, t[2 * it] + b0, t[2 * it + 1] + b1);
      }
    }
  } else if constexpr (EPI == DB200_EPI_RESID) {
    float b0 = 0.f, b1 = 0.f, s0 = e.sign, s1 = e.sign;
    if (e.bias) { const float2 bb = __ldg(reinterpret_cast<const float2*>(e.bias + n)); b0 = bb.x; b1 = bb.y; }
    if (e.scale) { const float2 sc = __ldg(reinterpret_cast<const float2*>(e.scale + n)); s0 *= sc.x; s1 *= sc.y; }
    float2 rr[16];
#pragma unroll
    for (int it = 0; it < 16; ++it) {
      const int m = mbase + 2 * it;
      rr[it] = make_float2(0.f, 0.f);
      if (e.resid && m < M) rr[it] = __ldg(reinterpret_cast<const float2*>(e.resid + (long long)m * e.N + n));
    }
#pragma unroll
    for (int it = 0; it < 16; ++it) {
      const int m = mbase + 2 * it;
      if (m < M) {
        const long long off = (long long)m * e.N + n;
        const float v0 = t[2 * it] + b0, v1 = t[2 * it + 1] + b1;
        if (e.y_out) store2<T>(reinterpret_cast<T*>(e.y_out) + off, v0, v1);
        *reinterpret_cast<float2*>(e.out + off) = make_float2(rr[it].x + s0 * v0, rr[it].y + s1 * v1);
      }
    }
  } else if constexpr (EPI == DB200_EPI_QKV) {
    const int inner = e.heads * e.dim_head;
    const int which = n / inner;
    const int rem = n - which * inner;
    const int head = rem / e.dim_head;
    const int d = rem - head * e.dim_head;
    const float qs = which == 0 ? e.q_scale : 1.0f;
    T* base = reinterpret_cast<T*>(which == 0 ? e.q : (which == 1 ? e.k : e.v));
    const int b0 = mbase / e.seq_n;
    const int p0 = mbase - b0 * e.seq_n;
    float cs[16], sn[16];
    {
      int b = b0, p = p0;
#pragma unroll
      for (int it = 0; it < 16; ++it) {
        while (p >= e.seq_n) { p -= e.seq_n; ++b; }
        cs[it] = 1.f; sn[it] = 0.f;
        if (e.cos_t && mbase + 2 * it < M) {
          const int ti = (p + e.pos_offset) * (e.dim_head >> 1) + (d >> 1);
          cs[it] = __ldg(e.cos_t + ti);
          sn[it] = __ldg(e.sin_t + ti);
        }
        p += 2;
      }
    }
    int b = b0, p = p0;
#pragma unroll
    for (int it = 0; it < 16; ++it) {
      while (p >= e.seq_n) { p -= e.seq_n; ++b; }
      if (mbase + 2 * it < M) {
        const float x0 = t[2 * it], x1 = t[2 * it + 1];
        T* dst = base + (((long long)b * e.heads + head) * e.seq_n + p) * e.dim_head + d;
        store2<T>(dst, (x0 * cs[it] + (-x1) * sn[it]) * qs, (x1 * cs[it] + x0 * sn[it]) * qs);
      }
      p += 2;
    }
  } else if constexpr (EPI == DB200_EPI_GEGLU_BWD) {
    float2 a[16], g[16];
#pragma unroll
    for (int it = 0; it < 16; ++it) {
      const int m = mbase + 2 * it;
      a[it] = make_float2(0.f, 0.f); g[it] = make_float2(0.f, 0.f);
      if (m < M) {
        const T* u = reinterpret_cast<const T*>(e.u_in) + (long long)m * (2 * e.hidden);
        a[it] = load2<T>(u + n);
        g[it] = load2<T>(u + e.hidden + n);
      }
    }
#pragma unroll
    for (int it = 0; it < 16; ++it) {
      const int m = mbase + 2 * it;
      if (m < M) {
        float f0, f1, df0, df1;
        gelu_pair<T>(g[it].x, f0, df0);
        gelu_pair<T>(g[it].y, f1, df1);
        T* du = reinterpret_cast<T*>(e.du_out) + (long long)m * (2 * e.hidden);
        store2<T>(du + n, t[2 * it] * f0, t[2 * it + 1] * f1);
        store2<T>(du + e.hidden + n, t[2 * it] * a[it].x * df0, t[2 * it + 1] * a[it].y * df1);
      }
    }
  }
}

template <typename T>
__device__ __forceinline__ void epi_chunk_cols_geglu(const EpiArgs& e, int mbase, int j, const float* ta, const float* tg, int M) {
  float ba0 = 0.f, ba1 = 0.f, bg0 = 0.f, bg1 = 0.f;
  if (e.bias) {
    const float2 ba = __ldg(reinterpret_cast<const float2*>(e.bias + j));
    const float2 bg = __ldg(reinterpret_cast<const float2*>(e.bias + e.hidden + j));
    ba0 = ba.x; ba1 = ba.y; bg0 = bg.x; bg1 = bg.y;
  }
#pragma unroll
  for (int it = 0; it < 16; ++it) {
    const int m = mbase + 2 * it;
    if (m < M) {
      const float a0 = ta[2 * it] + ba0, a1 = ta[2 * it + 1] + ba1, g0 = tg[2 * it] + bg0, g1 = tg[2 * it + 1] + bg1;
      if (e.u_out) {
        T* u = reinterpret_cast<T*>(e.u_out) + (long long)m * (2 * e.hidden);
        store2<T>(u + j, a0, a1);
        store2<T>(u + e.hidden + j, g0, g1);
      }
      float2 f, df;
      gelu_pair2<T>(make_float2(g0, g1), f, df);
      store2<T>(reinterpret_cast<T*>(e.h_out) + (long long)m * e.hidden + j, a0 * f.x, a1 * f.y);
    }
  }
}

}
```

dalle_pytorch_b200/csrc/gemm_tcgen05.cu:

```cuda
#include <cuda.h>
#include <atomic>

#include <cstdlib>
#include <cstring>
#include <mutex>

#include "common.cuh"
#include "epilogue.cuh"
#include "tc_common.cuh"

namespace db200 {

using namespace tc;

namespace {

constexpr int BLOCK_M = 128;
constexpr int BLOCK_K = 64;
constexpr int UMMA_K = 16;
constexpr int NUM_THREADS = 320;
constexpr int NUM_EPI_WARPS = 8;
constexpr int SCHED_DEPTH = 4;
constexpr int EPI_STAGE_BYTES = 32 * 32 * 4;
constexpr int A_STAGE_BYTES = BLOCK_M * BLOCK_K * 2;
constexpr int BOX_MN_BYTES = 64 * BLOCK_K * 2;
constexpr int SMEM_BUDGET = 193 * 1024;

__device__ __forceinline__ void transpose_chunk(const uint32_t* in, float* out, float* stage, int lane) {
  __syncwarp();
#pragma unroll
  for (int j = 0; j < 8; ++j)
    *reinterpret_cast<uint4*>(stage + lane * 32 + ((j ^ (lane & 7)) << 2)) = make_uint4(in[4 * j], in[4 * j + 1], in[4 * j + 2], in[4 * j + 3]);
  __syncwarp();
  const int j = (lane & 15) >> 1, sub = (lane & 1) << 1;
#pragma unroll
  for (int it = 0; it < 16; ++it) {
    const int rr = 2 * it + (lane >> 4);
    const float2 v = *reinterpret_cast<const float2*>(stage + rr * 32 + ((j ^ (rr & 7)) << 2) + sub);
    out[2 * it] = v.x;
    out[2 * it + 1] = v.y;
  }
}

template <int BLOCK_N>
struct SmemLayout {
  static constexpr int B_STAGE_BYTES = BLOCK_N * BLOCK_K * 2;
  static constexpr int STAGE_BYTES = A_STAGE_BYTES + B_STAGE_BYTES;
  static constexpr int STAGES = (SMEM_BUDGET / STAGE_BYTES) > 8 ? 8 : (SMEM_BUDGET / STAGE_BYTES);
  static constexpr int BAR_BYTES = (2 * STAGES + 4 + 2 * SCHED_DEPTH) * 8 + 16 + SCHED_DEPTH * 4 + 12;
  static constexpr int EPI_OFFSET = STAGES * STAGE_BYTES;
  static constexpr int BAR_OFFSET = EPI_OFFSET + NUM_EPI_WARPS * EPI_STAGE_BYTES;
  static constexpr int TOTAL = BAR_OFFSET + BAR_BYTES + 1024;
};

constexpr int SCHED_SLOTS = 256;
__device__ unsigned int g_sched_counter[SCHED_SLOTS];
static std::atomic<unsigned int> g_launch_seq{0};

template <int BLOCK_N, int EPI, bool A_MN, bool B_MN, bool EPI_COLS>
__global__ void __launch_bounds__(NUM_THREADS, 1)
gemm_tcgen05_kernel(const __grid_constant__ CUtensorMap tmA, const __grid_constant__ CUtensorMap tmB, const __grid_constant__ CUtensorMap tmC,
                    int M, int N, int K, int k_splits, int sched_slot, EpiArgs e) {
  using L = SmemLayout<BLOCK_N>;
  constexpr int STAGES = L::STAGES;
  constexpr int B_STAGE_BYTES = L::B_STAGE_BYTES;
  constexpr uint32_t TMEM_COLS = 2 * BLOCK_N;
  static_assert(BLOCK_N == 128 || BLOCK_N == 256, "BLOCK_N");
  static_assert(EPI != DB200_EPI_GEGLU || (BLOCK_N == 256 && !B_MN), "GEGLU pairs the two 128-column halves of a 256 tile");

  extern __shared__ uint8_t smem_raw[];
  uint8_t* smem = reinterpret_cast<uint8_t*>((reinterpret_cast<uintptr_t>(smem_raw) + 1023) & ~static_cast<uintptr_t>(1023));
  uint8_t* smem_a = smem;
  uint8_t* smem_b = smem + STAGES * A_STAGE_BYTES;
  uint64_t* bars = reinterpret_cast<uint64_t*>(smem + L::BAR_OFFSET);
  const uint32_t full_bar = smem_u32(bars);
  const uint32_t empty_bar = smem_u32(bars + STAGES);
  const uint32_t tfull_bar = smem_u32(bars + 2 * STAGES);
  const uint32_t tempty_bar = smem_u32(bars + 2 * STAGES + 2);
  const uint32_t sfull_bar = smem_u32(bars + 2 * STAGES + 4);
  const uint32_t sempty_bar = smem_u32(bars + 2 * STAGES + 4 + SCHED_DEPTH);
  uint32_t* tmem_slot = reinterpret_cast<uint32_t*>(bars + 2 * STAGES + 4 + 2 * SCHED_DEPTH);
  volatile int* sched_tile = reinterpret_cast<volatile int*>(tmem_slot + 4);

  const int warp = threadIdx.x >> 5, lane = threadIdx.x & 31;

  pdl_launch();
  unsigned int first_draw = 0;
  const bool dyn = sched_slot >= 0;
  if (threadIdx.x == 0) first_draw = dyn ? atomicAdd(&g_sched_counter[sched_slot], 1u) : blockIdx.x;
  if (warp == 0 && lane == 0) {
    tma_prefetch_desc(&tmA);
    tma_prefetch_desc(&tmB);
    for (int s = 0; s < STAGES; ++s) { mbar_init(full_bar + 8 * s, 1); mbar_init(empty_bar + 8 * s, 1); }
    for (int s = 0; s < 2; ++s) { mbar_init(tfull_bar + 8 * s, 1); mbar_init(tempty_bar + 8 * s, NUM_EPI_WARPS * 32); }
    for (int s = 0; s < SCHED_DEPTH; ++s) { mbar_init(sfull_bar + 8 * s, 1); mbar_init(sempty_bar + 8 * s, 1 + NUM_EPI_WARPS); }
    asm volatile("fence.mbarrier_init.release.cluster;" ::: "memory");
  }
  if (warp == 1) {
    asm volatile("tcgen05.alloc.cta_group::1.sync.aligned.shared::cta.b32 [%0], %1;" ::"r"(smem_u32(tmem_slot)), "r"(TMEM_COLS) : "memory");
    asm volatile("tcgen05.relinquish_alloc_permit.cta_group::1.sync.aligned;" ::: "memory");
  }
  tc_fence_before();
  __syncthreads();
  tc_fence_after();
  const uint32_t tmem_base = *tmem_slot;
  pdl_wait();

  const int num_m = (M + BLOCK_M - 1) / BLOCK_M;
  const int num_n = (N + BLOCK_N - 1) / BLOCK_N;
  const int num_mn = num_m * num_n;
  const int num_tiles = num_mn * k_splits;
  const int total_kb = (K + BLOCK_K - 1) / BLOCK_K;
  const int kb_per = (total_kb + k_splits - 1) / k_splits;

  if (warp == 0) {
    {
      int s = 0; uint32_t ph = 0;
      int ss = 0; uint32_t sph = 0;
      unsigned int* counter = &g_sched_counter[dyn ? sched_slot : 0];
      const unsigned int last_draw = dyn ? static_cast<unsigned int>(num_tiles) + gridDim.x - 1u : 0xffffffffu;
      if (lane == 0 && first_draw == last_draw) atomicExch(counter, 0u);
      int tile = static_cast<int>(__shfl_sync(0xffffffffu, first_draw, 0));
      while (true) {
        mbar_wait(sempty_bar + 8 * ss, sph ^ 1);
        if (lane == 0) {
          sched_tile[ss] = tile;
          mbar_arrive(sfull_bar + 8 * ss);
        }
        __syncwarp();
        if (++ss == SCHED_DEPTH) { ss = 0; sph ^= 1; }
        if (tile >= num_tiles) break;
        unsigned int drawn = 0;
        if (lane == 0) drawn = dyn ? atomicAdd(counter, 1u) : static_cast<unsigned int>(tile) + gridDim.x;
        const int mn = tile % num_mn, split = tile / num_mn;
        const int m0 = (mn / num_n) * BLOCK_M;
        const int n0 = (mn % num_n) * BLOCK_N;
        const int kb0 = split * kb_per, kb1 = min(total_kb, kb0 + kb_per);
        for (int kb = kb0; kb < kb1; ++kb) {
          mbar_wait(empty_bar + 8 * s, ph ^ 1);
          const uint32_t fb = full_bar + 8 * s;
          const uint32_t sa = smem_u32(smem_a + s * A_STAGE_BYTES);
          const uint32_t sb = smem_u32(smem_b + s * B_STAGE_BYTES);
          const int k0 = kb * BLOCK_K;
          if (elect_one()) {
            mbar_expect_tx(fb, L::STAGE_BYTES);
            if constexpr (!A_MN) {
              tma_load_2d(sa, &tmA, fb, k0, m0);
            } else {
#pragma unroll
              for (int c = 0; c < BLOCK_M / 64; ++c) tma_load_2d(sa + c * BOX_MN_BYTES, &tmA, fb, m0 + c * 64, k0);
            }
            if constexpr (!B_MN) {
#pragma unroll
              for (int c = 0; c < BLOCK_N / 128; ++c) {
                int row = n0 + c * 128;
                if constexpr (EPI == DB200_EPI_GEGLU) row = (c == 0) ? (n0 >> 1) : e.hidden + (n0 >> 1);
                tma_load_2d(sb + c * (128 * BLOCK_K * 2), &tmB, fb, k0, row);
              }
            } else {
#pragma unroll
              for (int c = 0; c < BLOCK_N / 64; ++c) tma_load_2d(sb + c * BOX_MN_BYTES, &tmB, fb, n0 + c * 64, k0);
            }
          }
          __syncwarp();
          if (++s == STAGES) { s = 0; ph ^= 1; }
        }
        drawn = __shfl_sync(0xffffffffu, drawn, 0);
        if (lane == 0 && drawn == last_draw) atomicExch(counter, 0u);
        tile = static_cast<int>(drawn);
      }
    }
  } else if (warp == 1) {
    {
      const uint32_t idesc = (1u << 4) | (1u << 7) | (1u << 10) | (A_MN ? (1u << 15) : 0u) | (B_MN ? (1u << 16) : 0u) |
                             (static_cast<uint32_t>(BLOCK_N >> 3) << 17) | (static_cast<uint32_t>(BLOCK_M >> 4) << 24);
      constexpr uint32_t A_LBO = A_MN ? BOX_MN_BYTES : 16, B_LBO = B_MN ? BOX_MN_BYTES : 16;
      constexpr uint32_t A_KSTEP = A_MN ? (UMMA_K * 128) >> 4 : (UMMA_K * 2) >> 4;
      constexpr uint32_t B_KSTEP = B_MN ? (UMMA_K * 128) >> 4 : (UMMA_K * 2) >> 4;
      int s = 0; uint32_t ph = 0;
      int as = 0; uint32_t aph = 0;
      int ss = 0; uint32_t sph = 0;
      while (true) {
        mbar_wait(sfull_bar + 8 * ss, sph);
        const int tile = sched_tile[ss];
        __syncwarp();
        if (lane == 0) mbar_arrive(sempty_bar + 8 * ss);
        if (++ss == SCHED_DEPTH) { ss = 0; sph ^= 1; }
        if (tile >= num_tiles) break;
        mbar_wait(tempty_bar + 8 * as, aph ^ 1);
        tc_fence_after();
        const uint32_t tmem_c = tmem_base + as * BLOCK_N;
        const int split = tile / num_mn;
        const int kb0 = split * kb_per, kb1 = min(total_kb, kb0 + kb_per);
        for (int kb = kb0; kb < kb1; ++kb) {
          mbar_wait(full_bar + 8 * s, ph);
          tc_fence_after();
          const uint64_t da = make_smem_desc(smem_u32(smem_a + s * A_STAGE_BYTES), A_LBO, 1024);
          const uint64_t db = make_smem_desc(smem_u32(smem_b + s * B_STAGE_BYTES), B_LBO, 1024);
          if (elect_one()) {
#pragma unroll
            for (int k = 0; k < BLOCK_K / UMMA_K; ++k)
              umma_bf16(tmem_c, da + static_cast<uint64_t>(k * A_KSTEP), db + static_cast<uint64_t>(k * B_KSTEP), idesc, (kb > kb0) || (k != 0));
            umma_commit(empty_bar + 8 * s);
            if (kb == kb1 - 1) umma_commit(tfull_bar + 8 * as);
          }
          __syncwarp();
          if (++s == STAGES) { s = 0; ph ^= 1; }
        }
        if (++as == 2) { as = 0; aph ^= 1; }
      }
    }
  } else {
    const int ew = warp - 2;
    const int quarter = warp & 3;
    const int half = ew >> 2;
    float* stage = reinterpret_cast<float*>(smem + L::EPI_OFFSET + ew * EPI_STAGE_BYTES);
    const int lrow = lane >> 4, lcol = (lane & 15) << 1;
    int as = 0; uint32_t aph = 0;
    int ss = 0; uint32_t sph = 0;
    while (true) {
      mbar_wait(sfull_bar + 8 * ss, sph);
      const int tile = sched_tile[ss];
      __syncwarp();
      if (lane == 0) mbar_arrive(sempty_bar + 8 * ss);
      if (++ss == SCHED_DEPTH) { ss = 0; sph ^= 1; }
      if (tile >= num_tiles) break;
      const int mn = tile % num_mn;
      const int m0 = (mn / num_n) * BLOCK_M;
      const int n0 = (mn % num_n) * BLOCK_N;
      const int mbase = m0 + quarter * 32 + lrow;
      mbar_wait(tfull_bar + 8 * as, aph);
      tc_fence_after();
      const uint32_t taddr = tmem_base + (static_cast<uint32_t>(quarter * 32) << 16) + as * BLOCK_N;
      if (e.atomic_c == 4) {
      } else if (EPI == DB200_EPI_STORE && !EPI_COLS && e.tma_store) {
        constexpr int NCH = (BLOCK_N / 2) / 32;
        const uint32_t stage_u32 = smem_u32(stage);
        uint32_t r[2][32];
        tmem_ld32(taddr + half * (BLOCK_N / 2), r[0]);
#pragma unroll
        for (int ch = 0; ch < NCH; ++ch) {
          tmem_ld_wait();
          if (ch + 1 < NCH) tmem_ld32(taddr + half * (BLOCK_N / 2) + (ch + 1) * 32, r[(ch + 1) & 1]);
          const int n = n0 + half * (BLOCK_N / 2) + ch * 32;
          uint32_t w[16];
#pragma unroll
          for (int i = 0; i < 16; ++i) {
            float a = __uint_as_float(r[ch & 1][2 * i]), b = __uint_as_float(r[ch & 1][2 * i + 1]);
            if (e.bias && n + 2 * i < N) { const float2 bb = __ldg(reinterpret_cast<const float2*>(e.bias + n + 2 * i)); a += bb.x; b += bb.y; }
            const __nv_bfloat162 p2 = __floats2bfloat162_rn(a, b);
            w[i] = *reinterpret_cast<const uint32_t*>(&p2);
          }
          if ((ch & 1) == 0) {
            if (lane == 0) bulk_wait_group_read0();
            __syncwarp();
          }
#pragma unroll
          for (int j = 0; j < 4; ++j) {
            const int unit = (ch & 1) * 4 + j;
            asm volatile("st.shared.v4.b32 [%0], {%1, %2, %3, %4};" ::"r"(stage_u32 + lane * 128 + ((unit ^ (lane & 7)) << 4)), "r"(w[4 * j]),
                         "r"(w[4 * j + 1]), "r"(w[4 * j + 2]), "r"(w[4 * j + 3])
                         : "memory");
          }
          if (ch & 1) {
            fence_proxy_async();
            __syncwarp();
            if (lane == 0) {
              tma_store_2d(&tmC, stage_u32, n0 + half * (BLOCK_N / 2) + (ch >> 1) * 64, m0 + quarter * 32);
              bulk_commit_group();
            }
          }
        }
      } else
      if constexpr (!EPI_COLS) {
        const int m = m0 + quarter * 32 + lane;
        if constexpr (EPI == DB200_EPI_GEGLU) {
          uint32_t ra[2][32], rg[2][32];
          tmem_ld32(taddr + half * 64, ra[0]);
          tmem_ld32(taddr + 128 + half * 64, rg[0]);
#pragma unroll
          for (int ch = 0; ch < 2; ++ch) {
            tmem_ld_wait();
            if (ch + 1 < 2) {
              tmem_ld32(taddr + half * 64 + 32, ra[1]);
              tmem_ld32(taddr + 128 + half * 64 + 32, rg[1]);
            }
            const int j0 = (n0 >> 1) + half * 64 + ch * 32;
            if (m < M) {
              if ((e.hidden & 15) == 0) {
#pragma unroll
                for (int o2 = 0; o2 < 2; ++o2)
                  if (j0 + o2 * 16 < e.hidden) epi_geglu16<__nv_bfloat16>(e, m, j0 + o2 * 16, &ra[ch][o2 * 16], &rg[ch][o2 * 16]);
              } else {
#pragma unroll
                for (int o = 0; o < 4; ++o) {
                  const int j = j0 + o * 8;
                  if (j < e.hidden) {
                    float a[8], g[8];
#pragma unroll
                    for (int i = 0; i < 8; ++i) { a[i] = __uint_as_float(ra[ch][o * 8 + i]); g[i] = __uint_as_float(rg[ch][o * 8 + i]); }
                    epi_geglu_vec8<__nv_bfloat16>(e, m, j, a, g);
                  }
                }
              }
            }
          }
        } else {
          constexpr int NCH = (BLOCK_N / 2) / 32;
          uint32_t r[2][32];
          tmem_ld32(taddr + half * (BLOCK_N / 2), r[0]);
#pragma unroll
          for (int ch = 0; ch < NCH; ++ch) {
            tmem_ld_wait();
            if (ch + 1 < NCH) tmem_ld32(taddr + half * (BLOCK_N / 2) + (ch + 1) * 32, r[(ch + 1) & 1]);
            if (m < M) {
#pragma unroll
              for (int o2 = 0; o2 < 2; ++o2) {
                const int nn = n0 + half * (BLOCK_N / 2) + ch * 32 + o2 * 16;
                bool done = false;
                if constexpr (EPI == DB200_EPI_STORE) {
                  if (nn + 16 <= N) done = epi_store16<__nv_bfloat16>(e, m, nn, &r[ch & 1][o2 * 16]);
                }
                if constexpr (EPI == DB200_EPI_RESID) {
                  if (nn + 16 <= N) { epi_resid16<__nv_bfloat16>(e, m, nn, &r[ch & 1][o2 * 16]); done = true; }
                }
                if (!done) {
#pragma unroll
                  for (int o = 2 * o2; o < 2 * o2 + 2; ++o) {
                    const int n = n0 + half * (BLOCK_N / 2) + ch * 32 + o * 8;
                    if (n < N) {
                      float v[8];
#pragma unroll
                      for (int i = 0; i < 8; ++i) v[i] = __uint_as_float(r[ch & 1][o * 8 + i]);
                      epi_vec8<EPI, __nv_bfloat16>(e, m, n, v);
                    }
                  }
                }
              }
            }
          }
        }
      } else
      if constexpr (EPI == DB200_EPI_GEGLU) {
        uint32_t ra[32], rg[32];
        tmem_ld32(taddr + half * 64, ra);
        tmem_ld32(taddr + 128 + half * 64, rg);
#pragma unroll
        for (int ch = 0; ch < 2; ++ch) {
          tmem_ld_wait();
          float ta[32], tg[32];
          transpose_chunk(ra, ta, stage, lane);
          transpose_chunk(rg, tg, stage, lane);
          if (ch + 1 < 2) {
            tmem_ld32(taddr + half * 64 + 32, ra);
            tmem_ld32(taddr + 128 + half * 64 + 32, rg);
          }
          const int j = (n0 >> 1) + half * 64 + ch * 32 + lcol;
          if (j < e.hidden) epi_chunk_cols_geglu<__nv_bfloat16>(e, mbase, j, ta, tg, M);
        }
      } else {
        constexpr int NCH = (BLOCK_N / 2) / 32;
        uint32_t r[32];
        tmem_ld32(taddr + half * (BLOCK_N / 2), r);
#pragma unroll
        for (int ch = 0; ch < NCH; ++ch) {
          tmem_ld_wait();
          float t[32];
          transpose_chunk(r, t, stage, lane);
          if (ch + 1 < NCH) tmem_ld32(taddr + half * (BLOCK_N / 2) + (ch + 1) * 32, r);
          const int n = n0 + half * (BLOCK_N / 2) + ch * 32 + lcol;
          if (n < N) epi_chunk_cols<EPI, __nv_bfloat16>(e, mbase, n, t, M);
        }
      }
      tc_fence_before();
      mbar_arrive(tempty_bar + 8 * as);
      if (++as == 2) { as = 0; aph ^= 1; }
    }
    if (EPI == DB200_EPI_STORE && !EPI_COLS && e.tma_store && lane == 0) bulk_wait_group0();
  }

  tc_fence_before();
  __syncthreads();
  if (warp == 1) {
    tc_fence_after();
    asm volatile("tcgen05.dealloc.cta_group::1.sync.aligned.b32 %0, %1;" ::"r"(tmem_base), "r"(TMEM_COLS) : "memory");
  }
}

inline bool al16(const void* p);
inline bool tma_store_env() {
  static const bool on = [] { const char* v = getenv("DALLE_B200_GEMM_TMA_STORE"); return !(v && !strcmp(v, "0")); }();
  return on;
}

template <int BLOCK_N, int EPI, bool A_MN, bool B_MN, bool EPI_COLS>
int launch_cfg_mode(const db200_gemm_params& p, cudaStream_t st) {
  using L = SmemLayout<BLOCK_N>;
  CUtensorMap tmA, tmB;
  int rc;
  if (!A_MN) rc = make_tensor_map_bf16(&tmA, p.A, p.K, p.M, p.lda, BLOCK_K, BLOCK_M);
  else rc = make_tensor_map_bf16(&tmA, p.A, p.M, p.K, p.lda, 64, BLOCK_K);
  if (rc) return rc;
  if (!B_MN) rc = make_tensor_map_bf16(&tmB, p.B, p.K, p.N, p.ldb, BLOCK_K, 128);
  else rc = make_tensor_map_bf16(&tmB, p.B, p.N, p.K, p.ldb, 64, BLOCK_K);
  if (rc) return rc;
  CUtensorMap tmC = tmA;
  EpiArgs e = make_epi_args(p);
  if (EPI == DB200_EPI_STORE && !EPI_COLS && e.atomic_c == 0 && p.c_dtype == DB200_BF16 && !p.split_k_ok && al16(p.C) && (p.ldc % 8) == 0 &&
      tma_store_env()) {
    if ((rc = make_tensor_map_bf16(&tmC, p.C, p.N, p.M, p.ldc, 64, 32))) return rc;
    e.tma_store = 1;
  }
  auto kern = gemm_tcgen05_kernel<BLOCK_N, EPI, A_MN, B_MN, EPI_COLS>;
  static std::atomic<bool> attr_done{false};
  if (!attr_done.load(std::memory_order_acquire)) {
    DB200_CUDA_OK(cudaFuncSetAttribute(kern, cudaFuncAttributeMaxDynamicSharedMemorySize, L::TOTAL));
    attr_done.store(true, std::memory_order_release);
  }
  const int num_mn = ceil_div(p.M, BLOCK_M) * ceil_div(p.N, BLOCK_N);
  int k_splits = 1;
  if (EPI == DB200_EPI_STORE && p.split_k_ok && p.c_dtype == DB200_F32 && p.bias == nullptr) {
    const int total_kb = ceil_div(p.K, BLOCK_K);
    k_splits = sm_count() / num_mn;
    if (k_splits > 8) k_splits = 8;
    if (k_splits > total_kb / 8) k_splits = total_kb / 8;
    if (k_splits < 1) k_splits = 1;
  }
  const int num_tiles = num_mn * k_splits;
  const int grid = num_tiles < sm_count() ? num_tiles : sm_count();
  if (e.atomic_c < 2) e.atomic_c = k_splits > 1;
  static const bool static_sched = [] { const char* v = std::getenv("DALLE_B200_SCHED"); return v && !std::strcmp(v, "static"); }();
  const int sched_slot = static_sched ? -1 : static_cast<int>(g_launch_seq.fetch_add(1, std::memory_order_relaxed) % SCHED_SLOTS);
  DB200_CUDA_OK(launch_pdl(kern, dim3(grid), dim3(NUM_THREADS), L::TOTAL, st, tmA, tmB, tmC, p.M, p.N, p.K, k_splits, sched_slot, e));
  DB200_LAUNCH_OK("gemm_tcgen05_kernel");
  return DB200_OK;
}

inline int epi_mode_env() {
  static const int mode = [] {
    const char* v = getenv("DALLE_B200_EPI");
    return (v && !strcmp(v, "rows")) ? 1 : (v && !strcmp(v, "cols")) ? 2 : 0;
  }();
  return mode;
}

template <int BLOCK_N, int EPI, bool A_MN, bool B_MN>
int launch_cfg(const db200_gemm_params& p, cudaStream_t st) {
  const int env = epi_mode_env();
  const bool cols = env == 2 || (env == 0 && EPI == DB200_EPI_RESID) ||
                    (EPI == DB200_EPI_STORE && p.C_multicast != nullptr);
  if (cols) return launch_cfg_mode<BLOCK_N, EPI, A_MN, B_MN, true>(p, st);
  return launch_cfg_mode<BLOCK_N, EPI, A_MN, B_MN, false>(p, st);
}

template <int EPI, bool A_MN, bool B_MN>
int launch_bn(const db200_gemm_params& p, cudaStream_t st) {
  if constexpr (EPI == DB200_EPI_GEGLU) {
    return launch_cfg<256, EPI, A_MN, B_MN>(p, st);
  } else {
    const long long tiles256 = (long long)ceil_div(p.M, BLOCK_M) * ceil_div(p.N, 256);
    if (p.N >= 256 && (p.N % 256 == 0 || p.N > 1024) && tiles256 >= sm_count() / 2) return launch_cfg<256, EPI, A_MN, B_MN>(p, st);
    return launch_cfg<128, EPI, A_MN, B_MN>(p, st);
  }
}

bool device_is_sm100() {
  static std::atomic<int> cached[64];
  int dev = 0;
  if (cudaGetDevice(&dev) != cudaSuccess || dev < 0 || dev >= 64) return false;
  if (cached[dev] == 0) {
    int major = 0;
    cudaDeviceGetAttribute(&major, cudaDevAttrComputeCapabilityMajor, dev);
    cached[dev] = (major == 10) ? 1 : -1;
  }
  return cached[dev] == 1;
}

inline bool al16(const void* p) { return (reinterpret_cast<uintptr_t>(p) & 15) == 0; }

}

namespace {
typedef CUresult (*EncodeTiledFn)(CUtensorMap*, CUtensorMapDataType, cuuint32_t, void*, const cuuint64_t*, const cuuint64_t*,
                                  const cuuint32_t*, const cuuint32_t*, CUtensorMapInterleave, CUtensorMapSwizzle,
                                  CUtensorMapL2promotion, CUtensorMapFloatOOBfill);

EncodeTiledFn get_encode_fn() {
  static EncodeTiledFn fn = nullptr;
  static std::once_flag once;
  std::call_once(once, [] {
    void* p = nullptr;
    cudaDriverEntryPointQueryResult q;
    if (cudaGetDriverEntryPoint("cuTensorMapEncodeTiled", &p, cudaEnableDefault, &q) == cudaSuccess && q == cudaDriverEntryPointSuccess)
      fn = reinterpret_cast<EncodeTiledFn>(p);
  });
  return fn;
}

int make_tensor_map_bf16_impl(CUtensorMap* map, const void* base, uint64_t inner, uint64_t outer, uint64_t ld, uint32_t box_inner, uint32_t box_outer) {
  EncodeTiledFn fn = get_encode_fn();
  if (!fn) return set_error(DB200_ERR_NO_DEVICE, "cuTensorMapEncodeTiled entry point not available");
  cuuint64_t gdim[2] = {inner, outer};
  cuuint64_t gstride[1] = {ld * 2};
  cuuint32_t box[2] = {box_inner, box_outer};
  cuuint32_t estr[2] = {1, 1};
  const CUresult r = fn(map, CU_TENSOR_MAP_DATA_TYPE_BFLOAT16, 2, const_cast<void*>(base), gdim, gstride, box, estr,
                        CU_TENSOR_MAP_INTERLEAVE_NONE, CU_TENSOR_MAP_SWIZZLE_128B, CU_TENSOR_MAP_L2_PROMOTION_L2_256B,
                        CU_TENSOR_MAP_FLOAT_OOB_FILL_NONE);
  if (r != CUDA_SUCCESS) return set_error(DB200_ERR_CUDA, "cuTensorMapEncodeTiled failed with CUresult %d (inner=%llu outer=%llu ld=%llu)", (int)r,
                                          (unsigned long long)inner, (unsigned long long)outer, (unsigned long long)ld);
  return DB200_OK;
}

int make_tensor_map_bf16_nd_impl(CUtensorMap* map, const void* base, int rank, const uint64_t* dims, const uint64_t* strides_elems,
                                 const uint32_t* box) {
  EncodeTiledFn fn = get_encode_fn();
  if (!fn) return set_error(DB200_ERR_NO_DEVICE, "cuTensorMapEncodeTiled entry point not available");
  if (rank < 2 || rank > 5) return set_error(DB200_ERR_BAD_ARG, "tensor map rank %d", rank);
  cuuint64_t gdim[5], gstride[4];
  cuuint32_t bx[5], estr[5];
  for (int i = 0; i < rank; ++i) { gdim[i] = dims[i]; bx[i] = box[i]; estr[i] = 1; }
  for (int i = 1; i < rank; ++i) gstride[i - 1] = strides_elems[i] * 2;
  const CUresult r = fn(map, CU_TENSOR_MAP_DATA_TYPE_BFLOAT16, rank, const_cast<void*>(base), gdim, gstride, bx, estr,
                        CU_TENSOR_MAP_INTERLEAVE_NONE, CU_TENSOR_MAP_SWIZZLE_128B, CU_TENSOR_MAP_L2_PROMOTION_L2_256B,
                        CU_TENSOR_MAP_FLOAT_OOB_FILL_NONE);
  if (r != CUDA_SUCCESS) return set_error(DB200_ERR_CUDA, "cuTensorMapEncodeTiled (rank %d) failed with CUresult %d", rank, (int)r);
  return DB200_OK;
}

}

namespace tc {
int make_tensor_map_bf16(CUtensorMap* map, const void* base, uint64_t inner, uint64_t outer, uint64_t ld, uint32_t box_inner,
                         uint32_t box_outer) {
  return make_tensor_map_bf16_impl(map, base, inner, outer, ld, box_inner, box_outer);
}
int make_tensor_map_bf16_nd(CUtensorMap* map, const void* base, int rank, const uint64_t* dims, const uint64_t* strides_elems,
                            const uint32_t* box) {
  return make_tensor_map_bf16_nd_impl(map, base, rank, dims, strides_elems, box);
}
}

bool gemm_tcgen05_supported(const db200_gemm_params& p, const char** why) {
  const char* w = nullptr;
  if (p.dtype != DB200_BF16) w = "operands are not bf16";
  else if (!device_is_sm100()) w = "device is not sm_100";
  else if (!al16(p.A) || !al16(p.B)) w = "A/B not 16-byte aligned";
  else if (p.lda % 8 || p.ldb % 8) w = "leading dimensions must be multiples of 8 elements";
  else if (p.K % 8 || p.N % 8) w = "K and N must be multiples of 8";
  else if (p.a_mn_major && p.M % 8) w = "M-major A needs M % 8 == 0";
  else if (p.a_mn_major && !p.b_mn_major && p.epilogue != DB200_EPI_STORE) w = "M-major A x K-major B only with the STORE epilogue";
  else {
    switch (p.epilogue) {
      case DB200_EPI_STORE:
        if (!al16(p.C) || p.ldc % 8 || (p.bias && !al16(p.bias))) w = "C/bias alignment";
        break;
      case DB200_EPI_QKV:
        if (p.a_mn_major || p.b_mn_major) w = "QKV epilogue is forward-only (K-major operands)";
        else if (p.dim_head % 8 || !al16(p.q) || !al16(p.k) || !al16(p.v) || (p.cos_t && (!al16(p.cos_t) || !al16(p.sin_t) || p.dim_head % 16)))
          w = "q/k/v/rotary alignment";
        break;
      case DB200_EPI_RESID:
        if (p.a_mn_major || p.b_mn_major) w = "RESID epilogue is forward-only";
        else if (!al16(p.out) || (p.resid && !al16(p.resid)) || (p.scale && !al16(p.scale)) || (p.bias && !al16(p.bias)) || (p.y_out && !al16(p.y_out)))
          w = "RESID tensor alignment";
        break;
      case DB200_EPI_GEGLU:
        if (p.a_mn_major || p.b_mn_major) w = "GEGLU epilogue is forward-only";
        else if (p.hidden % 128) w = "GEGLU needs hidden % 128 == 0";
        else if (!al16(p.h_out) || (p.u_out && !al16(p.u_out)) || (p.bias && !al16(p.bias))) w = "GEGLU tensor alignment";
        break;
      case DB200_EPI_GEGLU_BWD:
        if (p.a_mn_major) w = "GEGLU_BWD expects K-major A";
        else if (!al16(p.u_in) || !al16(p.du_out) || p.hidden % 8) w = "GEGLU_BWD tensor alignment";
        break;
      default: w = "unknown epilogue";
    }
  }
  if (why) *why = w ? w : "";
  return w == nullptr;
}

int gemm_tcgen05_launch(const db200_gemm_params& p, cudaStream_t st) {
  const bool a = p.a_mn_major != 0, b = p.b_mn_major != 0;
  switch (p.epilogue) {
    case DB200_EPI_STORE:
      if (!a && !b) return launch_bn<DB200_EPI_STORE, false, false>(p, st);
      if (!a && b) return launch_bn<DB200_EPI_STORE, false, true>(p, st);
      if (a && b) return launch_bn<DB200_EPI_STORE, true, true>(p, st);
      return launch_bn<DB200_EPI_STORE, true, false>(p, st);
    case DB200_EPI_QKV: return launch_bn<DB200_EPI_QKV, false, false>(p, st);
    case DB200_EPI_RESID: return launch_bn<DB200_EPI_RESID, false, false>(p, st);
    case DB200_EPI_GEGLU: return launch_bn<DB200_EPI_GEGLU, false, false>(p, st);
    case DB200_EPI_GEGLU_BWD:
      if (!b) return launch_bn<DB200_EPI_GEGLU_BWD, false, false>(p, st);
      return launch_bn<DB200_EPI_GEGLU_BWD, false, true>(p, st);
    default: break;
  }
  return set_error(DB200_ERR_BAD_ARG, "gemm_tcgen05: unsupported epilogue/major combination");
}

}
```

dalle_pytorch_b200/csrc/tc_common.cuh:

```cuda
#pragma once
#include <cuda.h>

#include "common.cuh"

namespace db200 {
namespace tc {

__device__ __forceinline__ uint32_t smem_u32(const void* p) { return static_cast<uint32_t>(__cvta_generic_to_shared(p)); }

__device__ __forceinline__ void mbar_init(uint32_t bar, uint32_t count) {
  asm volatile("mbarrier.init.shared::cta.b64 [%0], %1;" ::"r"(bar), "r"(count) : "memory");
}
__device__ __forceinline__ void mbar_expect_tx(uint32_t bar, uint32_t bytes) {
  asm volatile("mbarrier.arrive.expect_tx.shared::cta.b64 _, [%0], %1;" ::"r"(bar), "r"(bytes) : "memory");
}
__device__ __forceinline__ void mbar_arrive(uint32_t bar) {
  asm volatile("mbarrier.arrive.shared::cta.b64 _, [%0];" ::"r"(bar) : "memory");
}
__device__ __forceinline__ bool mbar_try_wait(uint32_t bar, uint32_t parity) {
  uint32_t ok;
  asm volatile(
      "{\n\t.reg .pred p;\n\t"
      "mbarrier.try_wait.parity.shared::cta.b64 p, [%1], %2, %3;\n\t"
      "selp.u32 %0, 1, 0, p;\n\t}"
      : "=r"(ok)
      : "r"(bar), "r"(parity), "r"(0x989680u)
      : "memory");
  return ok != 0;
}
__device__ __forceinline__ void mbar_wait(uint32_t bar, uint32_t parity) {
  if (mbar_try_wait(bar, parity)) return;
  const long long t0 = clock64();
  while (!mbar_try_wait(bar, parity)) {
    if (clock64() - t0 > 4000000000LL) {
      printf("dalle_b200 tcgen05 kernel: mbarrier timeout (block %d thread %d bar 0x%x parity %u)\n", blockIdx.x, threadIdx.x, bar,
             parity);
      __trap();
    }
  }
}

__device__ __forceinline__ void mbar_wait_mode(uint32_t bar, uint32_t parity, int mode) {
  if (mode == 0) { mbar_wait(bar, parity); return; }
  uint32_t ok = 0;
  const long long t0 = clock64();
  while (true) {
    asm volatile(
        "{\n\t.reg .pred p;\n\t"
        "mbarrier.try_wait.parity.shared::cta.b64 p, [%1], %2;\n\t"
        "selp.u32 %0, 1, 0, p;\n\t}"
        : "=r"(ok)
        : "r"(bar), "r"(parity)
        : "memory");
    if (ok) return;
    if (clock64() - t0 > 4000000000LL) __trap();
  }
}

__device__ __forceinline__ void tma_load_2d(uint32_t dst, const CUtensorMap* map, uint32_t bar, int c0, int c1) {
  asm volatile(
      "cp.async.bulk.tensor.2d.shared::cluster.global.mbarrier::complete_tx::bytes [%0], [%1, {%3, %4}], [%2];" ::"r"(dst),
      "l"(map), "r"(bar), "r"(c0), "r"(c1)
      : "memory");
}
__device__ __forceinline__ void tma_load_4d(uint32_t dst, const CUtensorMap* map, uint32_t bar, int c0, int c1, int c2, int c3) {
  asm volatile(
      "cp.async.bulk.tensor.4d.shared::cluster.global.mbarrier::complete_tx::bytes [%0], [%1, {%3, %4, %5, %6}], [%2];" ::"r"(dst),
      "l"(map), "r"(bar), "r"(c0), "r"(c1), "r"(c2), "r"(c3)
      : "memory");
}
__device__ __forceinline__ void tma_load_5d(uint32_t dst, const CUtensorMap* map, uint32_t bar, int c0, int c1, int c2, int c3, int c4) {
  asm volatile(
      "cp.async.bulk.tensor.5d.shared::cluster.global.mbarrier::complete_tx::bytes [%0], [%1, {%3, %4, %5, %6, %7}], [%2];" ::"r"(dst),
      "l"(map), "r"(bar), "r"(c0), "r"(c1), "r"(c2), "r"(c3), "r"(c4)
      : "memory");
}
__device__ __forceinline__ void tma_store_2d(const CUtensorMap* map, uint32_t src, int c0, int c1) {
  asm volatile("cp.async.bulk.tensor.2d.global.shared::cta.bulk_group [%0, {%2, %3}], [%1];" ::"l"(map), "r"(src), "r"(c0), "r"(c1) : "memory");
}
__device__ __forceinline__ void bulk_commit_group() { asm volatile("cp.async.bulk.commit_group;" ::: "memory"); }
__device__ __forceinline__ void bulk_wait_group_read0() { asm volatile("cp.async.bulk.wait_group.read 0;" ::: "memory"); }
__device__ __forceinline__ void bulk_wait_group0() { asm volatile("cp.async.bulk.wait_group 0;" ::: "memory"); }
__device__ __forceinline__ void tma_prefetch_desc(const CUtensorMap* map) {
  asm volatile("prefetch.tensormap [%0];" ::"l"(map) : "memory");
}

__device__ __forceinline__ void tc_fence_before() { asm volatile("tcgen05.fence::before_thread_sync;" ::: "memory"); }
__device__ __forceinline__ void tc_fence_after() { asm volatile("tcgen05.fence::after_thread_sync;" ::: "memory"); }

__device__ __forceinline__ void umma_bf16(uint32_t tmem_c, uint64_t desc_a, uint64_t desc_b, uint32_t idesc, uint32_t accumulate) {
  asm volatile(
      "{\n\t.reg .pred p;\n\t"
      "setp.ne.b32 p, %4, 0;\n\t"
      "tcgen05.mma.cta_group::1.kind::f16 [%0], %1, %2, %3, p;\n\t}" ::"r"(tmem_c),
      "l"(desc_a), "l"(desc_b), "r"(idesc), "r"(accumulate)
      : "memory");
}
__device__ __forceinline__ void umma_commit(uint32_t bar) {
  asm volatile("tcgen05.commit.cta_group::1.mbarrier::arrive::one.shared::cluster.b64 [%0];" ::"r"(bar) : "memory");
}
__device__ __forceinline__ void tmem_ld32(uint32_t taddr, uint32_t* r) {
  asm volatile(
      "tcgen05.ld.sync.aligned.32x32b.x32.b32 "
      "{%0, %1, %2, %3, %4, %5, %6, %7, %8, %9, %10, %11, %12, %13, %14, %15, "
      "%16, %17, %18, %19, %20, %21, %22, %23, %24, %25, %26, %27, %28, %29, %30, %31}, [%32];"
      : "=r"(r[0]), "=r"(r[1]), "=r"(r[2]), "=r"(r[3]), "=r"(r[4]), "=r"(r[5]), "=r"(r[6]), "=r"(r[7]), "=r"(r[8]), "=r"(r[9]),
        "=r"(r[10]), "=r"(r[11]), "=r"(r[12]), "=r"(r[13]), "=r"(r[14]), "=r"(r[15]), "=r"(r[16]), "=r"(r[17]), "=r"(r[18]),
        "=r"(r[19]), "=r"(r[20]), "=r"(r[21]), "=r"(r[22]), "=r"(r[23]), "=r"(r[24]), "=r"(r[25]), "=r"(r[26]), "=r"(r[27]),
        "=r"(r[28]), "=r"(r[29]), "=r"(r[30]), "=r"(r[31])
      : "r"(taddr));
}
__device__ __forceinline__ void tmem_ld_wait() { asm volatile("tcgen05.wait::ld.sync.aligned;" ::: "memory"); }

__device__ __forceinline__ uint64_t make_smem_desc(uint32_t saddr, uint32_t lbo_bytes, uint32_t sbo_bytes) {
  uint64_t d = 0;
  d |= static_cast<uint64_t>((saddr & 0x3FFFFu) >> 4);
  d |= static_cast<uint64_t>((lbo_bytes >> 4) & 0x3FFFu) << 16;
  d |= static_cast<uint64_t>((sbo_bytes >> 4) & 0x3FFFu) << 32;
  d |= static_cast<uint64_t>(1) << 46;
  d |= static_cast<uint64_t>(2) << 61;
  return d;
}


__device__ __forceinline__ void tmem_ld16(uint32_t taddr, uint32_t* r) {
  asm volatile(
      "tcgen05.ld.sync.aligned.32x32b.x16.b32 "
      "{%0, %1, %2, %3, %4, %5, %6, %7, %8, %9, %10, %11, %12, %13, %14, %15}, [%16];"
      : "=r"(r[0]), "=r"(r[1]), "=r"(r[2]), "=r"(r[3]), "=r"(r[4]), "=r"(r[5]), "=r"(r[6]), "=r"(r[7]), "=r"(r[8]), "=r"(r[9]),
        "=r"(r[10]), "=r"(r[11]), "=r"(r[12]), "=r"(r[13]), "=r"(r[14]), "=r"(r[15])
      : "r"(taddr));
}
__device__ __forceinline__ void tmem_st16(uint32_t taddr, const uint32_t* r) {
  asm volatile(
      "tcgen05.st.sync.aligned.32x32b.x16.b32 [%0], "
      "{%1, %2, %3, %4, %5, %6, %7, %8, %9, %10, %11, %12, %13, %14, %15, %16};" ::"r"(taddr),
      "r"(r[0]), "r"(r[1]), "r"(r[2]), "r"(r[3]), "r"(r[4]), "r"(r[5]), "r"(r[6]), "r"(r[7]), "r"(r[8]), "r"(r[9]), "r"(r[10]),
      "r"(r[11]), "r"(r[12]), "r"(r[13]), "r"(r[14]), "r"(r[15])
      : "memory");
}
__device__ __forceinline__ void tmem_st8(uint32_t taddr, const uint32_t* r) {
  asm volatile("tcgen05.st.sync.aligned.32x32b.x8.b32 [%0], {%1, %2, %3, %4, %5, %6, %7, %8};" ::"r"(taddr), "r"(r[0]), "r"(r[1]), "r"(r[2]),
               "r"(r[3]), "r"(r[4]), "r"(r[5]), "r"(r[6]), "r"(r[7])
               : "memory");
}
__device__ __forceinline__ void bulk_load_1d(uint32_t dst, const void* src, uint32_t bytes, uint32_t bar) {
  asm volatile("cp.async.bulk.shared::cluster.global.mbarrier::complete_tx::bytes [%0], [%1], %2, [%3];" ::"r"(dst), "l"(src), "r"(bytes),
               "r"(bar)
               : "memory");
}
__device__ __forceinline__ void tmem_st32(uint32_t taddr, const uint32_t* r) {
  asm volatile(
      "tcgen05.st.sync.aligned.32x32b.x32.b32 [%0], "
      "{%1, %2, %3, %4, %5, %6, %7, %8, %9, %10, %11, %12, %13, %14, %15, %16, "
      "%17, %18, %19, %20, %21, %22, %23, %24, %25, %26, %27, %28, %29, %30, %31, %32};" ::"r"(taddr),
      "r"(r[0]), "r"(r[1]), "r"(r[2]), "r"(r[3]), "r"(r[4]), "r"(r[5]), "r"(r[6]), "r"(r[7]), "r"(r[8]), "r"(r[9]), "r"(r[10]),
      "r"(r[11]), "r"(r[12]), "r"(r[13]), "r"(r[14]), "r"(r[15]), "r"(r[16]), "r"(r[17]), "r"(r[18]), "r"(r[19]), "r"(r[20]),
      "r"(r[21]), "r"(r[22]), "r"(r[23]), "r"(r[24]), "r"(r[25]), "r"(r[26]), "r"(r[27]), "r"(r[28]), "r"(r[29]), "r"(r[30]),
      "r"(r[31])
      : "memory");
}
__device__ __forceinline__ void tmem_st_wait() { asm volatile("tcgen05.wait::st.sync.aligned;" ::: "memory"); }

__device__ __forceinline__ bool elect_one() {
  uint32_t pred;
  asm volatile("{\n\t.reg .pred p;\n\telect.sync _|p, 0xffffffff;\n\tselp.u32 %0, 1, 0, p;\n\t}" : "=r"(pred));
  return pred != 0;
}

__device__ __forceinline__ void umma_bf16_ts(uint32_t tmem_c, uint32_t tmem_a, uint64_t desc_b, uint32_t idesc, uint32_t accumulate) {
  asm volatile(
      "{\n\t.reg .pred p;\n\t"
      "setp.ne.b32 p, %4, 0;\n\t"
      "tcgen05.mma.cta_group::1.kind::f16 [%0], [%1], %2, %3, p;\n\t}" ::"r"(tmem_c),
      "r"(tmem_a), "l"(desc_b), "r"(idesc), "r"(accumulate)
      : "memory");
}

__device__ __forceinline__ void tmem_alloc(uint32_t smem_slot, uint32_t cols) {
  asm volatile("tcgen05.alloc.cta_group::1.sync.aligned.shared::cta.b32 [%0], %1;" ::"r"(smem_slot), "r"(cols) : "memory");
  asm volatile("tcgen05.relinquish_alloc_permit.cta_group::1.sync.aligned;" ::: "memory");
}
__device__ __forceinline__ void tmem_dealloc(uint32_t base, uint32_t cols) {
  asm volatile("tcgen05.dealloc.cta_group::1.sync.aligned.b32 %0, %1;" ::"r"(base), "r"(cols) : "memory");
}
__device__ __forceinline__ void fence_proxy_async() { asm volatile("fence.proxy.async.shared::cta;" ::: "memory"); }

__host__ __device__ constexpr uint32_t make_idesc_bf16(int M, int N, bool a_mn, bool b_mn) {
  return (1u << 4) | (1u << 7) | (1u << 10) | (a_mn ? (1u << 15) : 0u) | (b_mn ? (1u << 16) : 0u) |
         (static_cast<uint32_t>(N >> 3) << 17) | (static_cast<uint32_t>(M >> 4) << 24);
}

int make_tensor_map_bf16(CUtensorMap* map, const void* base, uint64_t inner, uint64_t outer, uint64_t ld, uint32_t box_inner,
                         uint32_t box_outer);
int make_tensor_map_bf16_nd(CUtensorMap* map, const void* base, int rank, const uint64_t* dims, const uint64_t* strides_elems,
                            const uint32_t* box);

}
}
```

dalle_pytorch_b200/functional.py:

```python
import os
import threading

import torch

from . import ops


FUSE_GEGLU_BWD = False
FUSE_UPSTREAM_SCALE_BWD = os.environ.get('DALLE_B200_FUSE_SCALE_BWD', '1') != '0'


class _SubRec:
    __slots__ = ('y', 'scale', 'sign', 'out', 'out_version', 'pre', 'pre_dx', 'pre_version')

    def __init__(self, y, scale, sign, out):
        self.y, self.scale, self.sign = y, scale, sign
        self.out, self.out_version = out, out._version
        self.pre, self.pre_dx, self.pre_version = None, None, -1

    def produced(self, x):
        o = self.out
        return (o is not None and x.data_ptr() == o.data_ptr() and x._version == self.out_version and x.shape == o.shape
                and x.dtype == o.dtype)

    def take_pre(self, d_out):
        pre, dx = self.pre, self.pre_dx
        self.pre = self.pre_dx = None
        if pre is None or dx is None:
            return None
        if d_out.data_ptr() != dx.data_ptr() or d_out._version != self.pre_version or d_out.shape != dx.shape:
            return None
        return pre


_chain = threading.local()


def chain_reset():
    last = getattr(_chain, 'last', None)
    if last is not None:
        last.out = None
    _chain.last = None


def _chain_link(x_in, resid_is_input, rec):
    prev = getattr(_chain, 'last', None)
    _chain.last = rec
    if prev is None:
        return None
    ok = FUSE_UPSTREAM_SCALE_BWD and resid_is_input and x_in.shape[-1] == 1024 and x_in.is_cuda and prev.produced(x_in)
    prev.out = None
    return prev if ok else None


class DropoutRNG:

    @staticmethod
    def draw(numel):
        return (torch.initial_seed(), int(torch.randint(0, 2 ** 62, (1,), dtype=torch.int64).item()))


def draw_dropout(g, kind, x_in, hidden=None):
    if g.p_drop <= 0:
        return None
    b, n, d = x_in.shape
    return DropoutRNG.draw(b * n * (d if kind == 'attn' else hidden))


class SublayerGeom:

    def __init__(self, *, dtype, text_len=0, fmap=0, do_ln=True, do_shift=False, heads=0, dim_head=64, attn_spec=None,
                 q_scale=None, eps=1e-5, p_drop=0.0):
        self.p_drop = float(p_drop)
        self.dtype = dtype
        self.text_len, self.fmap = text_len, fmap
        self.do_ln, self.do_shift = do_ln, do_shift
        self.heads, self.dim_head = heads, dim_head
        self.attn_spec = attn_spec
        self.q_scale = q_scale if q_scale is not None else dim_head ** -0.5
        self.eps = eps

    def shift_active(self, n):
        return self.do_shift and n >= self.text_len


_wcache_on = True
_wcache_epoch = 0


def weight_cache_enabled(flag):
    global _wcache_on
    old, _wcache_on = _wcache_on, bool(flag)
    return old


def invalidate_weight_cache():
    global _wcache_epoch
    _wcache_epoch += 1


def _w(weight, dtype):
    if dtype == torch.float32:
        return weight.detach().contiguous()
    if not _wcache_on or not weight.is_leaf:
        return ops.cast_bf16(weight.detach().contiguous())
    hit = getattr(weight, '_b200_bf16', None)
    if hit is not None and hit[0] == (weight._version, _wcache_epoch, weight.data_ptr()):
        return hit[1]
    c = ops.cast_bf16(weight.detach().contiguous())
    weight._b200_bf16 = ((weight._version, _wcache_epoch, weight.data_ptr()), c)
    return c


def _up_args(up, da):
    if up is None:
        return None
    if up.y is not None and up.y.dtype != da.dtype:
        return None
    return (up.y, up.scale, up.sign)


def _up_store(up, res):
    if not isinstance(res, tuple):
        return res
    dx, up_dy, up_dscale, up_dbias = res
    up.pre, up.pre_dx, up.pre_version = (up_dy, up_dscale, up_dbias), dx, dx._version
    return dx


def attn_sublayer_forward(g: SublayerGeom, x_in, resid, ln_w, ln_b, w_qkv, w_out, b_out, scale, sign, cos_t, sin_t,
                          key_mask=None, save=True, drop=None):
    b, n, d = x_in.shape
    x_in = x_in.contiguous()
    shift = g.shift_active(n)
    a1, mean, rstd = ops.ln_shift_fwd(x_in, ln_w, ln_b, g.dtype, g.text_len, g.fmap, do_ln=g.do_ln, do_shift=shift, eps=g.eps)
    wq, wo = _w(w_qkv, g.dtype), _w(w_out, g.dtype)
    lay = ops.gather_layout(g.attn_spec, g.dtype, n, g.dim_head, key_mask)
    q, k, v = ops.gemm_qkv_auto(a1, wq, b, n, g.heads, g.dim_head, cos_t, sin_t, g.q_scale, n_alloc=None if lay is None else lay.n_alloc)
    o, lse = ops.attn_fwd(g.attn_spec, q, k, v, key_mask, lay=lay)
    keep_y = save and scale is not None
    r2 = None if resid is None else resid.contiguous().view(b * n, d)
    sc = None if scale is None else scale.detach().reshape(-1).contiguous()
    if drop is None:
        out, y = ops.gemm_resid(o.view(b * n, -1), wo, b_out, r2, sc, sign, keep_y=keep_y)
    else:
        y = ops.dropout_(ops.gemm_store(o.view(b * n, -1), wo, bias=b_out), g.p_drop, *drop)
        out = ops.resid_scale(y, r2, sc, sign)
        if not keep_y:
            y = None
    out = out.view(b, n, d)
    ctx = None
    if save:
        ctx = (x_in, mean, rstd, a1, wq, wo, q, k, v, o, lse, y, shift, lay)
    return out, ctx


def attn_sublayer_backward(g: SublayerGeom, ctx, d_out, ln_w, scale, sign, cos_t, sin_t, key_mask=None, dres=None, wslots=None,
                           pre=None, up=None, drop=None):
    x_in, mean, rstd, a1, wq, wo, q, k, v, o, lse, y, shift, lay = ctx
    s_qkv, s_out = wslots if wslots is not None else (None, None)
    b, n, d = x_in.shape
    M = b * n
    d_out = d_out.contiguous().view(M, d)
    sc = None if scale is None else scale.detach().reshape(-1).contiguous()
    pool = torch.zeros(6, d, device=x_in.device, dtype=torch.float32)
    if drop is not None:
        dy, dscale, _ = ops.scale_bwd(d_out, y, sc, sign, g.dtype, want_dbias=False, zeroed=(pool[0], pool[1]))
        ops.dropout_(dy, g.p_drop, *drop)
        db_out = ops.colsum(dy)
    elif pre is not None:
        dy, dscale, db_out = pre
    else:
        dy, dscale, db_out = ops.scale_bwd(d_out, y, sc, sign, g.dtype, zeroed=(pool[0], pool[1]))
    d_o = ops.gemm_store(dy, wo, a_mn=False, b_mn=True, out=ops.attn_dout_buffer(lay, M, wo.shape[1], dy.device, dy.dtype))
    dw_out = ops.gemm_store(dy, o.view(M, -1), a_mn=True, b_mn=True, out_dtype=torch.float32, out=s_out)
    dqkv = ops.attn_bwd(g.attn_spec, q, k, v, o, lse, d_o.view(b, n, -1), cos_t, sin_t, g.q_scale, key_mask, lay=lay)
    da1 = ops.gemm_store(dqkv, wq, a_mn=False, b_mn=True)
    dw_qkv = ops.gemm_store(dqkv, a1, a_mn=True, b_mn=True, out_dtype=torch.float32, out=s_qkv)
    dln_w = dln_b = None
    if g.do_ln:
        dln_w, dln_b = pool[2], pool[3]
    dx = ops.ln_shift_bwd(da1, x_in, mean, rstd, ln_w, None if dres is None else dres.contiguous(), g.text_len, g.fmap,
                          do_ln=g.do_ln, do_shift=shift, dgamma=dln_w, dbeta=dln_b, up=_up_args(up, da1), up_zeroed=pool[4:6])
    if up is not None:
        dx = _up_store(up, dx)
    if dscale is not None:
        dscale = dscale.view_as(scale)
    return dx, dln_w, dln_b, dw_qkv, dw_out, db_out, dscale


def ff_sublayer_forward(g: SublayerGeom, x_in, resid, ln_w, ln_b, w1, b1, w2, b2, scale, sign, save=True, drop=None):
    b, n, d = x_in.shape
    x_in = x_in.contiguous()
    shift = g.shift_active(n)
    a2, mean, rstd = ops.ln_shift_fwd(x_in, ln_w, ln_b, g.dtype, g.text_len, g.fmap, do_ln=g.do_ln, do_shift=shift, eps=g.eps)
    w1c, w2c = _w(w1, g.dtype), _w(w2, g.dtype)
    h, u = ops.gemm_geglu(a2, w1c, b1, keep_u=save)
    if drop is not None:
        ops.dropout_(h, g.p_drop, *drop)
    keep_y = save and scale is not None
    out, y = ops.gemm_resid(h, w2c, b2, None if resid is None else resid.contiguous().view(b * n, d),
                            None if scale is None else scale.detach().reshape(-1).contiguous(), sign, keep_y=keep_y)
    out = out.view(b, n, d)
    ctx = None
    if save:
        ctx = (x_in, mean, rstd, a2, w1c, w2c, u, h, y, shift)
    return out, ctx


def ff_sublayer_backward(g: SublayerGeom, ctx, d_out, ln_w, scale, sign, dres=None, wslots=None, pre=None, up=None, drop=None):
    x_in, mean, rstd, a2, w1c, w2c, u, h, y, shift = ctx
    s_w1, s_w2 = wslots if wslots is not None else (None, None)
    b, n, d = x_in.shape
    M = b * n
    d_out = d_out.contiguous().view(M, d)
    sc = None if scale is None else scale.detach().reshape(-1).contiguous()
    H2 = u.shape[1]
    pool = torch.zeros(6 * d + H2, device=x_in.device, dtype=torch.float32)
    if pre is not None:
        dy, dscale, db2 = pre
    else:
        dy, dscale, db2 = ops.scale_bwd(d_out, y, sc, sign, g.dtype, zeroed=(pool[:d], pool[d:2 * d]))
    if FUSE_GEGLU_BWD:
        du = ops.gemm_geglu_bwd(dy, w2c, u)
        db1 = ops.colsum(du)
    else:
        dh = ops.gemm_store(dy, w2c, a_mn=False, b_mn=True)
        if drop is not None:
            ops.dropout_(dh, g.p_drop, *drop)
        du, db1 = ops.geglu_bwd(dh, u, zeroed=pool[6 * d:])
    dw2 = ops.gemm_store(dy, h, a_mn=True, b_mn=True, out_dtype=torch.float32, out=s_w2)
    da2 = ops.gemm_store(du, w1c, a_mn=False, b_mn=True)
    dw1 = ops.gemm_store(du, a2, a_mn=True, b_mn=True, out_dtype=torch.float32, out=s_w1)
    dln_w = dln_b = None
    if g.do_ln:
        dln_w, dln_b = pool[2 * d:3 * d], pool[3 * d:4 * d]
    dx = ops.ln_shift_bwd(da2, x_in, mean, rstd, ln_w, None if dres is None else dres.contiguous(), g.text_len, g.fmap,
                          do_ln=g.do_ln, do_shift=shift, dgamma=dln_w, dbeta=dln_b, up=_up_args(up, da2),
                          up_zeroed=pool[4 * d:6 * d].view(2, d))
    if up is not None:
        dx = _up_store(up, dx)
    if dscale is not None:
        dscale = dscale.view_as(scale)
    return dx, dln_w, dln_b, dw1, db1, dw2, db2, dscale


def _note_use(*params):
    for p in params:
        if getattr(p, '_b200_reducer', None) is not None:
            p._b200_uses = getattr(p, '_b200_uses', 0) + 1


def _slot(p):
    r = getattr(p, '_b200_reducer', None)
    if r is None or getattr(p, '_b200_uses', 0) != 1:
        return None
    return r.direct_slot(p)


def _commit(p, slot, grad):
    if slot is None:
        return grad
    p._b200_reducer.direct_done(p)
    return None


class AttnSublayerFn(torch.autograd.Function):

    @staticmethod
    def forward(ctx, g, resid_is_input, sign, cos_t, sin_t, key_mask, x_in, resid, ln_w, ln_b, w_qkv, w_out, b_out, scale):
        r = x_in if resid_is_input else resid
        ctx.drop = DropoutRNG.draw(x_in.numel()) if g.p_drop > 0 else None
        out, saved = attn_sublayer_forward(g, x_in, r, ln_w, ln_b, w_qkv, w_out, b_out, scale, sign, cos_t, sin_t, key_mask,
                                           save=True, drop=ctx.drop)
        ctx.g, ctx.resid_is_input, ctx.sign = g, resid_is_input, sign
        ctx.cos_t, ctx.sin_t, ctx.key_mask = cos_t, sin_t, key_mask
        ctx.saved = saved
        ctx.ln_w, ctx.scale = ln_w, scale
        ctx.has_resid = resid is not None
        ctx.wparams = (w_qkv, w_out)
        _note_use(w_qkv, w_out)
        ctx.rec = ctx.up = None
        if ctx.drop is not None:
            chain_reset()
        elif any(ctx.needs_input_grad) and saved is not None:
            y = saved[11]
            ctx.rec = _SubRec(y, None if scale is None else scale.detach().reshape(-1).contiguous(), sign, out)
            ctx.up = _chain_link(x_in, resid_is_input, ctx.rec)
        return out

    @staticmethod
    def backward(ctx, d_out):
        g = ctx.g
        d_out = d_out.contiguous()
        dres = d_out if ctx.resid_is_input else None
        slots = tuple(_slot(p) for p in ctx.wparams)
        rec = ctx.rec
        pre = rec.take_pre(d_out) if rec is not None else None
        dx, dln_w, dln_b, dw_qkv, dw_out, db_out, dscale = attn_sublayer_backward(
            g, ctx.saved, d_out, ctx.ln_w, ctx.scale, ctx.sign, ctx.cos_t, ctx.sin_t, ctx.key_mask, dres=dres, wslots=slots,
            pre=pre, up=ctx.up, drop=ctx.drop)
        ctx.rec = ctx.up = None
        dw_qkv = _commit(ctx.wparams[0], slots[0], dw_qkv)
        dw_out = _commit(ctx.wparams[1], slots[1], dw_out)
        ctx.saved = None
        d_resid = d_out if (ctx.has_resid and not ctx.resid_is_input) else None
        return (None, None, None, None, None, None, dx, d_resid, dln_w, dln_b, dw_qkv, dw_out, db_out, dscale)


class FFSublayerFn(torch.autograd.Function):
    @staticmethod
    def forward(ctx, g, resid_is_input, sign, x_in, resid, ln_w, ln_b, w1, b1, w2, b2, scale):
        r = x_in if resid_is_input else resid
        ctx.drop = DropoutRNG.draw(x_in.shape[0] * x_in.shape[1] * w2.shape[1]) if g.p_drop > 0 else None
        out, saved = ff_sublayer_forward(g, x_in, r, ln_w, ln_b, w1, b1, w2, b2, scale, sign, save=True, drop=ctx.drop)
        ctx.g, ctx.resid_is_input, ctx.sign = g, resid_is_input, sign
        ctx.saved = saved
        ctx.ln_w, ctx.scale = ln_w, scale
        ctx.has_resid = resid is not None
        ctx.wparams = (w1, w2)
        _note_use(w1, w2)
        ctx.rec = ctx.up = None
        if any(ctx.needs_input_grad) and saved is not None:
            y = saved[8]
            ctx.rec = _SubRec(y, None if scale is None else scale.detach().reshape(-1).contiguous(), sign, out)
            ctx.up = _chain_link(x_in, resid_is_input, ctx.rec)
        return out

    @staticmethod
    def backward(ctx, d_out):
        d_out = d_out.contiguous()
        dres = d_out if ctx.resid_is_input else None
        slots = tuple(_slot(p) for p in ctx.wparams)
        rec = ctx.rec
        pre = rec.take_pre(d_out) if rec is not None else None
        dx, dln_w, dln_b, dw1, db1, dw2, db2, dscale = ff_sublayer_backward(ctx.g, ctx.saved, d_out, ctx.ln_w, ctx.scale, ctx.sign,
                                                                              dres=dres, wslots=slots, pre=pre, up=ctx.up, drop=ctx.drop)
        ctx.rec = ctx.up = None
        dw1 = _commit(ctx.wparams[0], slots[0], dw1)
        dw2 = _commit(ctx.wparams[1], slots[1], dw2)
        ctx.saved = None
        d_resid = d_out if (ctx.has_resid and not ctx.resid_is_input) else None
        return (None, None, None, dx, d_resid, dln_w, dln_b, dw1, db1, dw2, db2, dscale)


class EmbedTokensFn(torch.autograd.Function):

    @staticmethod
    def forward(ctx, text_ids, image_ids, w_text, w_image):
        B, Lt = text_ids.shape
        Li = 0 if image_ids is None else image_ids.shape[1]
        d = w_text.shape[1]
        out = torch.empty(B, Lt + Li, d, device=w_text.device, dtype=torch.float32)
        ops.embed_fwd(text_ids, w_text.detach().float(), out, 0)
        if Li:
            ops.embed_fwd(image_ids, w_image.detach().float(), out, Lt)
        ctx.save_for_backward(text_ids, image_ids)
        ctx.shapes = (w_text.shape, None if w_image is None else w_image.shape)
        return out

    @staticmethod
    def backward(ctx, d_out):
        text_ids, image_ids = ctx.saved_tensors
        d_out = d_out.contiguous().float()
        Lt = text_ids.shape[1]
        dw_text = torch.zeros(ctx.shapes[0], device=d_out.device, dtype=torch.float32)
        ops.embed_bwd(text_ids, d_out, dw_text, 0)
        dw_image = None
        if image_ids is not None and image_ids.shape[1] > 0:
            dw_image = torch.zeros(ctx.shapes[1], device=d_out.device, dtype=torch.float32)
            ops.embed_bwd(image_ids, d_out, dw_image, Lt)
        return None, None, dw_text, dw_image


class LayerNormFn(torch.autograd.Function):

    @staticmethod
    def forward(ctx, x, w, b, eps):
        shp = x.shape
        x3 = x.contiguous().view(1, -1, shp[-1]).float()
        out, mean, rstd = ops.ln_shift_fwd(x3, w, b, torch.float32, 0, 1, do_ln=True, do_shift=False, eps=eps)
        ctx.save_for_backward(x3, mean, rstd, w)
        return out.view(shp)

    @staticmethod
    def backward(ctx, d_out):
        x3, mean, rstd, w = ctx.saved_tensors
        d = x3.shape[-1]
        dw = torch.zeros(d, device=x3.device, dtype=torch.float32)
        db = torch.zeros(d, device=x3.device, dtype=torch.float32)
        dx = ops.ln_shift_bwd(d_out.contiguous().view(-1, d).float(), x3, mean, rstd, w, None, 0, 1, do_ln=True, do_shift=False,
                              dgamma=dw, dbeta=db)
        return dx.view(d_out.shape), dw, db, None


class HeadLossFn(torch.autograd.Function):

    @staticmethod
    def forward(ctx, x, ln_w, ln_b, w, bias, labels_text, labels_img, ntt, w_img, dtype, eps):
        M, d = x.shape
        Rt, Ri = labels_text.numel(), labels_img.numel()
        assert Rt + Ri == M
        x3 = x.contiguous().view(1, M, d)
        h, mean, rstd = ops.ln_shift_fwd(x3, ln_w, ln_b, dtype, 0, 1, do_ln=True, do_shift=False, eps=eps)
        wc = _w(w, dtype)
        bias = bias.detach()
        loss = torch.zeros(1, device=x.device, dtype=torch.float32)
        ct, ci = 1.0 / ((w_img + 1) * max(Rt, 1)), w_img / ((w_img + 1) * max(Ri, 1))
        lt = li = lse_t = lse_i = None
        if Rt:
            lt = ops.gemm_store(h[:Rt], wc[:ntt], bias=bias[:ntt])
            lse_t = ops.ce_fwd(lt, labels_text, ct, loss)
        if Ri:
            li = ops.gemm_store(h[Rt:], wc[ntt:], bias=bias[ntt:])
            lse_i = ops.ce_fwd(li, labels_img, ci, loss)
        ctx.saved = (x3, mean, rstd, h, wc, lt, li, lse_t, lse_i, labels_text, labels_img, ln_w)
        ctx.cfg = (ntt, ct, ci, Rt, Ri)
        return loss[0]

    @staticmethod
    def backward(ctx, dloss):
        x3, mean, rstd, h, wc, lt, li, lse_t, lse_i, labels_text, labels_img, ln_w = ctx.saved
        ctx.saved = None
        ntt, ct, ci, Rt, Ri = ctx.cfg
        M, d = h.shape
        V = wc.shape[0]
        up = dloss.detach().reshape(1).float().contiguous()
        dh = torch.empty(M, d, device=h.device, dtype=h.dtype)
        dw = torch.zeros(V, d, device=h.device, dtype=torch.float32) if (not Rt or not Ri) else torch.empty(V, d, device=h.device, dtype=torch.float32)
        db = torch.zeros(V, device=h.device, dtype=torch.float32)
        if Rt:
            ops.ce_bwd_(lt, labels_text, ct, lse_t, up)
            ops.gemm_store(lt, wc[:ntt], a_mn=False, b_mn=True, out=dh[:Rt])
            ops.gemm_store(lt, h[:Rt], a_mn=True, b_mn=True, out=dw[:ntt])
            db[:ntt] = ops.colsum(lt)
        if Ri:
            ops.ce_bwd_(li, labels_img, ci, lse_i, up)
            ops.gemm_store(li, wc[ntt:], a_mn=False, b_mn=True, out=dh[Rt:])
            ops.gemm_store(li, h[Rt:], a_mn=True, b_mn=True, out=dw[ntt:])
            db[ntt:] = ops.colsum(li)
        dln_w = torch.zeros(d, device=h.device, dtype=torch.float32)
        dln_b = torch.zeros(d, device=h.device, dtype=torch.float32)
        dx = ops.ln_shift_bwd(dh, x3, mean, rstd, ln_w, None, 0, 1, do_ln=True, do_shift=False, dgamma=dln_w, dbeta=dln_b)
        return dx.view(M, d), dln_w, dln_b, dw, db, None, None, None, None, None, None
```

dalle_pytorch_b200/ops.py:

```python
import contextlib
import ctypes
import os

import torch

from . import _lib, config
from ._lib import (F32, BF16, EPI_STORE, EPI_QKV, EPI_RESID, EPI_GEGLU, EPI_GEGLU_BWD, GEMM_AUTO,
                   ATTN_FULL, ATTN_AXIAL_ROW, ATTN_AXIAL_COL, ATTN_CONV_LIKE, ATTN_STATIC)

_launch_count = 0


def launches():
    return _launch_count


def _count(n=1):
    global _launch_count
    _launch_count += n


def dt_code(dtype):
    if dtype == torch.float32:
        return F32
    if dtype == torch.bfloat16:
        return BF16
    raise TypeError(f'unsupported compute dtype {dtype}')


def _p(t):
    if t is None:
        return None
    assert t.is_cuda, 'libdalle_b200 operates on CUDA tensors only (no CPU fallback)'
    return ctypes.c_void_p(t.data_ptr())


def _stream():
    return ctypes.c_void_p(torch.cuda.current_stream().cuda_stream)


def _c(t):
    assert t.is_contiguous(), 'expected a contiguous tensor'
    return t


def ln_shift_fwd(x, gamma, beta, out_dtype, text_len, fmap, do_ln=True, do_shift=True, eps=1e-5):
    b, n, d = x.shape
    _c(x)
    assert x.dtype == torch.float32
    out = torch.empty(b * n, d, device=x.device, dtype=out_dtype)
    mean = torch.empty(b * n, device=x.device, dtype=torch.float32) if do_ln else None
    rstd = torch.empty(b * n, device=x.device, dtype=torch.float32) if do_ln else None
    P = _lib.LnShiftFwdParams(batch=b, n=n, d=d, text_len=text_len, fmap=fmap, do_ln=int(do_ln), do_shift=int(do_shift),
                              out_dtype=dt_code(out_dtype), eps=eps, x=_p(x), gamma=_p(gamma), beta=_p(beta), out=_p(out),
                              mean=_p(mean), rstd=_p(rstd))
    _lib.check(_lib.lib().dalle_b200_ln_shift_fwd(ctypes.byref(P), _stream()), 'ln_shift_fwd')
    _count()
    return out, mean, rstd


def ln_shift_bwd(d_out, x, mean, rstd, gamma, dres, text_len, fmap, do_ln=True, do_shift=True, dgamma=None, dbeta=None, up=None,
                 up_zeroed=None):
    b, n, d = x.shape
    dx = torch.empty_like(x)
    P = _lib.LnShiftBwdParams(batch=b, n=n, d=d, text_len=text_len, fmap=fmap, do_ln=int(do_ln), do_shift=int(do_shift),
                              dout_dtype=dt_code(d_out.dtype), d_out=_p(_c(d_out)), x=_p(_c(x)), mean=_p(mean), rstd=_p(rstd),
                              gamma=_p(gamma), dres=_p(dres), dx=_p(dx), dgamma=_p(dgamma), dbeta=_p(dbeta))
    res = None
    if up is not None:
        up_y, up_scale, up_sign = up
        assert d == 1024 and (up_y is None or (up_y.dtype == d_out.dtype and up_y.is_contiguous()))
        up_dy = torch.empty(b * n, d, device=x.device, dtype=d_out.dtype)
        acc = up_zeroed if up_zeroed is not None else torch.zeros(2, d, device=x.device, dtype=torch.float32)
        want_scale = up_scale is not None and up_y is not None
        P.up_y, P.up_scale, P.up_sign, P.up_dy = _p(up_y), _p(up_scale), up_sign, _p(up_dy)
        P.up_dscale, P.up_dbias = (_p(acc[0]) if want_scale else None), _p(acc[1])
        res = (up_dy, acc[0] if want_scale else None, acc[1])
    _lib.check(_lib.lib().dalle_b200_ln_shift_bwd(ctypes.byref(P), _stream()), 'ln_shift_bwd')
    _count()
    return dx if res is None else (dx,) + res


_gemm_events = None


def gemm_timing(enable):
    global _gemm_events
    if enable:
        _gemm_events = []
        return None
    ev, _gemm_events = _gemm_events or [], None
    torch.cuda.synchronize()
    out = {'tcgen05': {'flops': 0.0, 'ms': 0.0, 'launches': 0}, 'simt': {'flops': 0.0, 'ms': 0.0, 'launches': 0},
           'smallm': {'flops': 0.0, 'ms': 0.0, 'launches': 0}, 'by_shape': {}}
    for s, e, flops, backend, key in ev:
        ms = s.elapsed_time(e)
        fam = out['tcgen05' if backend == _lib.GEMM_TCGEN05 else 'smallm' if backend == _lib.GEMM_SMALLM else 'simt']
        fam['flops'] += flops
        fam['ms'] += ms
        fam['launches'] += 1
        b = out['by_shape'].setdefault(key, {'ms': 0.0, 'flops': 0.0, 'launches': 0})
        b['ms'] += ms
        b['flops'] += flops
        b['launches'] += 1
    for b in out['by_shape'].values():
        b['tflops'] = b['flops'] / (b['ms'] * 1e-3) / 1e12 if b['ms'] > 0 else 0.0
        b['ms_per_launch'] = b['ms'] / b['launches']
        del b['flops']
    return out


_EPI_NAMES = {EPI_STORE: 'store', EPI_QKV: 'qkv', EPI_RESID: 'resid', EPI_GEGLU: 'geglu', EPI_GEGLU_BWD: 'geglu_bwd'}


def _gemm(P):
    if _gemm_events is None:
        _lib.check(_lib.lib().dalle_b200_gemm(ctypes.byref(P), _stream()), 'gemm')
        _count()
        return
    backend = _lib.lib().dalle_b200_gemm_select(ctypes.byref(P))
    s, e = torch.cuda.Event(enable_timing=True), torch.cuda.Event(enable_timing=True)
    s.record()
    _lib.check(_lib.lib().dalle_b200_gemm(ctypes.byref(P), _stream()), 'gemm')
    e.record()
    _count()
    key = f"{_EPI_NAMES.get(P.epilogue, '?')}:{'M' if P.a_mn_major else 'K'}{'N' if P.b_mn_major else 'K'}:{P.M}x{P.N}x{P.K}"
    _gemm_events.append((s, e, 2.0 * P.M * P.N * P.K, backend, key))


SMALL_M = os.environ.get('DALLE_B200_SMALLM', '1') != '0'
_small_m_rows = 16


@contextlib.contextmanager
def small_m_rows(rows):
    global _small_m_rows
    assert 1 <= rows <= 32
    prev, _small_m_rows = _small_m_rows, rows
    try:
        yield
    finally:
        _small_m_rows = prev


def _small_m(A, N, a_mn=False, b_mn=False):
    return (SMALL_M and A.dtype == torch.bfloat16 and not a_mn and not b_mn and 1 <= A.shape[0] <= _small_m_rows and A.shape[1] % 256 == 0
            and N % 16 == 0)


def _base(M, N, K, A, lda, a_mn, B, ldb, b_mn, epilogue, backend=GEMM_AUTO):
    assert A.dtype == B.dtype
    return _lib.GemmParams(M=M, N=N, K=K, dtype=dt_code(A.dtype), backend=backend, A=_p(A), lda=lda, a_mn_major=int(a_mn),
                           B=_p(B), ldb=ldb, b_mn_major=int(b_mn), epilogue=epilogue)


def split_bf16x3(x, operand, concat_rows):
    rows, cols = x.shape
    dst = torch.empty((6 * rows, cols) if concat_rows else (rows, 6 * cols), device=x.device, dtype=torch.bfloat16)
    _lib.check(_lib.lib().dalle_b200_split_bf16x3(_p(_c(x)), _p(dst), rows, cols, int(concat_rows), operand, _stream()), 'split_bf16x3')
    _count()
    return dst


def _gemm_x6(A, B, a_mn, b_mn, bias, out):
    if a_mn:
        K, M = A.shape
    else:
        M, K = A.shape
    N = B.shape[1] if b_mn else B.shape[0]
    if K % 8 or N % 8 or (a_mn and M % 8) or not (A.is_cuda and torch.cuda.get_device_capability(A.device)[0] == 10):
        return None
    A6 = split_bf16x3(A, 0, concat_rows=a_mn)
    B6 = split_bf16x3(B, 1, concat_rows=b_mn)
    P = _base(M, N, 6 * K, A6, A6.shape[1], a_mn, B6, B6.shape[1], b_mn, EPI_STORE, GEMM_AUTO)
    C = out if out is not None else torch.empty(M, N, device=A.device, dtype=torch.float32)
    P.C, P.ldc, P.c_dtype, P.bias, P.split_k_ok = _p(C), N, F32, _p(bias), 0
    if _lib.lib().dalle_b200_gemm_select(ctypes.byref(P)) != _lib.GEMM_TCGEN05:
        return None
    _gemm(P)
    return C


def _use_x6(A):
    return A.dtype == torch.float32 and config.fp32_gemm() == 'bf16x6'


def resid_scale(y, resid, scale, sign):
    M, d = y.shape
    out = torch.empty(M, d, device=y.device, dtype=torch.float32)
    _lib.check(_lib.lib().dalle_b200_resid_scale(_p(_c(y)), dt_code(y.dtype), _p(resid), _p(scale), sign, _p(out), M, d, _stream()), 'resid_scale')
    _count()
    return out


def sample_topk_gumbel(logits, thres=0.5, temperature=1.0, seed=0, offset=0, gumbel=None):
    B, V = logits.shape
    assert logits.stride(1) == 1
    k = max(int((1 - thres) * V), 1)
    out = torch.empty(B, device=logits.device, dtype=torch.int64)
    _lib.check(_lib.lib().dalle_b200_sample_topk_gumbel(_p(logits), dt_code(logits.dtype), B, V, logits.stride(0), k, float(temperature), _p(gumbel),
                                                        int(seed) & (2 ** 64 - 1), int(offset), _p(out), _stream()), 'sample_topk_gumbel')
    _count()
    return out


def sample_guided_topk_gumbel(logits, cond_scale, thres=0.5, temperature=1.0, seed=0, offset=0, gumbel=None):
    B2, V = logits.shape
    assert B2 % 2 == 0 and logits.stride(1) == 1
    b = B2 // 2
    k = max(int((1 - thres) * V), 1)
    out = torch.empty(b, device=logits.device, dtype=torch.int64)
    if gumbel is not None:
        assert gumbel.shape == (b, V) and gumbel.dtype == torch.float32 and gumbel.is_contiguous()
    _lib.check(_lib.lib().dalle_b200_sample_guided_topk_gumbel(_p(logits[:b]), _p(logits[b:]), dt_code(logits.dtype), b, V, logits.stride(0),
                                                               float(cond_scale), k, float(temperature), _p(gumbel), int(seed) & (2 ** 64 - 1),
                                                               int(offset), _p(out), _stream()), 'sample_guided_topk_gumbel')
    _count()
    return out


def decode_shift(h, ring_top, ring_left, pos_t, text_len, fmap, out_dtype):
    b, d = h.shape
    assert h.dtype == torch.float32 and ring_top.dtype == torch.float32 and ring_left.dtype == torch.float32 and pos_t.dtype == torch.int64
    assert ring_top.shape == (fmap, b, d // 4) and ring_left.shape == (fmap, b, d // 2 - d // 4) and d % 4 == 0
    y = torch.empty(b, d, device=h.device, dtype=out_dtype)
    _lib.check(_lib.lib().dalle_b200_decode_shift(_p(_c(h)), _p(y), dt_code(out_dtype), b, d, _p(_c(ring_top)), _p(_c(ring_left)), _p(pos_t),
                                                  int(text_len), int(fmap), _stream()), 'decode_shift')
    _count()
    return y


def decode_kv_append(k_new, v_new, k_cache, v_cache, pos_t):
    b, h, one, dh = k_new.shape
    assert one == 1 and v_new.shape == k_new.shape and k_cache.shape == v_cache.shape and k_cache.shape[:2] == (b, h) and k_cache.shape[3] == dh
    assert k_new.dtype == v_new.dtype == k_cache.dtype == v_cache.dtype and pos_t.dtype == torch.int64
    _lib.check(_lib.lib().dalle_b200_decode_kv_append(_p(_c(k_new)), _p(_c(v_new)), _p(_c(k_cache)), _p(_c(v_cache)), dt_code(k_cache.dtype), b * h, dh,
                                                      k_cache.shape[2], _p(pos_t), _stream()), 'decode_kv_append')
    _count()


def dropout_(x, p, seed, offset):
    _lib.check(_lib.lib().dalle_b200_dropout(_p(_c(x)), _p(x), dt_code(x.dtype), x.numel(), float(p), int(seed) & (2 ** 64 - 1), int(offset), _stream()),
               'dropout')
    _count()
    return x


def geglu_fwd(u):
    M, H2 = u.shape
    h = torch.empty(M, H2 // 2, device=u.device, dtype=torch.float32)
    _lib.check(_lib.lib().dalle_b200_geglu_fwd(_p(_c(u)), _p(h), M, H2 // 2, _stream()), 'geglu_fwd')
    _count()
    return h


def gemm_store(A, B, a_mn=False, b_mn=False, out_dtype=None, bias=None, backend=GEMM_AUTO, out=None):
    _c(A), _c(B)
    if backend == GEMM_AUTO and _use_x6(A) and (out is None or out.dtype == torch.float32) and out_dtype in (None, torch.float32):
        C6 = _gemm_x6(A, B, a_mn, b_mn, bias, out)
        if C6 is not None:
            return C6
    if a_mn:
        K, M = A.shape
    else:
        M, K = A.shape
    if b_mn:
        Kb, N = B.shape
    else:
        N, Kb = B.shape
    assert K == Kb, (A.shape, B.shape, a_mn, b_mn)
    if out is not None:
        assert out.shape == (M, N) and out.is_contiguous()
        C, out_dtype = out, out.dtype
    else:
        out_dtype = out_dtype or A.dtype
        C = None
    split_ok = out_dtype == torch.float32 and bias is None and A.dtype == torch.bfloat16 and M * N <= 4096 * 1024 and K >= 4096
    mc = getattr(out, '_b200_mc', None) if out is not None else None
    if backend == GEMM_AUTO and mc is None and _small_m(A, N, a_mn, b_mn):
        backend, split_ok = _lib.GEMM_SMALLM, False
    if C is None:
        C = (torch.zeros if split_ok else torch.empty)(M, N, device=A.device, dtype=out_dtype)
    elif split_ok and mc is None:
        C.zero_()
    P = _base(M, N, K, A, A.shape[1], a_mn, B, B.shape[1], b_mn, EPI_STORE, backend)
    P.C, P.ldc, P.c_dtype, P.bias, P.split_k_ok = _p(C), N, dt_code(out_dtype), _p(bias), int(split_ok)
    if mc is not None:
        assert out_dtype == torch.float32 and bias is None
        P.C_multicast, P.c_scale = ctypes.c_void_p(mc[0]), mc[1]
    _gemm(P)
    return C


def gemm_qkv(A, W, batch, seq_n, heads, dim_head, cos_t, sin_t, q_scale, pos_offset=0, backend=GEMM_AUTO):
    _c(A), _c(W)
    M, K = A.shape
    N = W.shape[0]
    if backend == GEMM_AUTO and _use_x6(A) and dim_head % 8 == 0:
        raw = _gemm_x6(A, W, False, False, None, None)
        if raw is not None:
            qkv = torch.empty(3, batch, heads, seq_n, dim_head, device=A.device, dtype=A.dtype)
            _lib.check(_lib.lib().dalle_b200_qkv_rotary(_p(raw), _p(qkv[0]), _p(qkv[1]), _p(qkv[2]), _p(cos_t), _p(sin_t), F32, M, seq_n, heads,
                                                        dim_head, pos_offset, q_scale, seq_n, _stream()), 'qkv_rotary')
            _count()
            return qkv[0], qkv[1], qkv[2]
    if backend == GEMM_AUTO and _small_m(A, N) and dim_head % 8 == 0:
        return gemm_qkv_auto(A, W, batch, seq_n, heads, dim_head, cos_t, sin_t, q_scale, pos_offset, n_alloc=seq_n)
    qkv = torch.empty(3, batch, heads, seq_n, dim_head, device=A.device, dtype=A.dtype)
    P = _base(M, N, K, A, K, False, W, K, False, EPI_QKV, backend)
    P.q, P.k, P.v = _p(qkv[0]), _p(qkv[1]), _p(qkv[2])
    P.cos_t, P.sin_t = _p(cos_t), _p(sin_t)
    P.seq_n, P.heads, P.dim_head, P.pos_offset, P.q_scale = seq_n, heads, dim_head, pos_offset, q_scale
    _gemm(P)
    return qkv[0], qkv[1], qkv[2]


FUSE_QKV_EPILOGUE = False


def gemm_qkv_auto(A, W, batch, seq_n, heads, dim_head, cos_t, sin_t, q_scale, pos_offset=0, n_alloc=None):
    if n_alloc is None and (FUSE_QKV_EPILOGUE or A.dtype != torch.bfloat16 or dim_head % 8):
        return gemm_qkv(A, W, batch, seq_n, heads, dim_head, cos_t, sin_t, q_scale, pos_offset)
    raw = gemm_store(A, W)
    M = raw.shape[0]
    rows = n_alloc or seq_n
    qkv = torch.empty(3, batch, heads, rows, dim_head, device=A.device, dtype=A.dtype)
    _lib.check(_lib.lib().dalle_b200_qkv_rotary(_p(raw), _p(qkv[0]), _p(qkv[1]), _p(qkv[2]), _p(cos_t), _p(sin_t), dt_code(A.dtype), M, seq_n,
                                                heads, dim_head, pos_offset, q_scale, rows, _stream()), 'qkv_rotary')
    _count()
    return qkv[0], qkv[1], qkv[2]


def gemm_resid(A, W, bias, resid, scale, sign=1.0, keep_y=False, backend=GEMM_AUTO):
    _c(A), _c(W)
    M, K = A.shape
    N = W.shape[0]
    if backend == GEMM_AUTO and _use_x6(A):
        y6 = _gemm_x6(A, W, False, False, bias, None)
        if y6 is not None:
            return resid_scale(y6, resid, scale, sign), (y6 if keep_y else None)
    out = torch.empty(M, N, device=A.device, dtype=torch.float32)
    y = torch.empty(M, N, device=A.device, dtype=A.dtype) if keep_y else None
    if backend == GEMM_AUTO and _small_m(A, N):
        backend = _lib.GEMM_SMALLM
    P = _base(M, N, K, A, K, False, W, K, False, EPI_RESID, backend)
    P.bias, P.resid, P.scale, P.sign, P.y_out, P.out = _p(bias), _p(resid), _p(scale), sign, _p(y), _p(out)
    _gemm(P)
    return out, y


def gemm_geglu(A, W1, b1, keep_u=True, backend=GEMM_AUTO):
    _c(A), _c(W1)
    M, K = A.shape
    N = W1.shape[0]
    H = N // 2
    if backend == GEMM_AUTO and _use_x6(A):
        u6 = _gemm_x6(A, W1, False, False, b1, None)
        if u6 is not None:
            return geglu_fwd(u6), (u6 if keep_u else None)
    h = torch.empty(M, H, device=A.device, dtype=A.dtype)
    u = torch.empty(M, N, device=A.device, dtype=A.dtype) if keep_u else None
    if backend == GEMM_AUTO and _small_m(A, N):
        backend = _lib.GEMM_SMALLM
    P = _base(M, N, K, A, K, False, W1, K, False, EPI_GEGLU, backend)
    P.bias, P.u_out, P.h_out, P.hidden = _p(b1), _p(u), _p(h), H
    _gemm(P)
    return h, u


def gemm_geglu_bwd(dy, W2, u, backend=GEMM_AUTO):
    _c(dy), _c(W2), _c(u)
    M, K = dy.shape
    H = W2.shape[1]
    du = torch.empty_like(u)
    P = _base(M, H, K, dy, K, False, W2, H, True, EPI_GEGLU_BWD, backend)
    P.u_in, P.du_out, P.hidden = _p(u), _p(du), H
    _gemm(P)
    return du


class AttnSpec:

    def __init__(self, pattern=ATTN_FULL, causal=True, stable=False, text_len=0, fmap=0, kernel_size=0, dilation=1,
                 static_mask=None):
        self.pattern, self.causal, self.stable = pattern, causal, stable
        self.text_len, self.fmap, self.kernel_size, self.dilation = text_len, fmap, kernel_size, dilation
        self.static_mask = static_mask


class GatherLayout:
    __slots__ = ('n', 'n_alloc', 'n_stat', 'col', 'pad_dout')

    def __init__(self, spec, n):
        T, fm = spec.text_len, spec.fmap
        self.n, self.n_alloc, self.n_stat = n, T + fm * fm, (T + 63) // 64 * 64 + fm * fm
        self.col = spec.pattern == ATTN_AXIAL_COL
        self.pad_dout = self.col and n < T + fm * fm


GATHER_AXIAL = os.environ.get('DALLE_B200_AXIAL_GATHER', '1') != '0'


def gather_layout(spec, dtype, n, dim_head=64, key_mask=None):
    if not GATHER_AXIAL or spec is None or spec.pattern not in (ATTN_AXIAL_ROW, ATTN_AXIAL_COL):
        return None
    if dtype != torch.bfloat16 or dim_head != 64 or key_mask is not None:
        return None
    if os.environ.get('DALLE_B200_ATTN', 'tc') != 'tc' or spec.fmap not in (16, 32, 64):
        return None
    full = spec.text_len + spec.fmap * spec.fmap
    if n not in (full - 1, full):
        return None
    return GatherLayout(spec, n)


def _attn_params(spec, q, k, v, out, lse, key_mask, lay=None, n_k=None):
    b, h, n_q, dh = q.shape
    kv_rows = 0
    if n_k is not None:
        kv_rows, n_k = k.shape[2], int(n_k)
        assert n_k <= kv_rows
    else:
        n_k = k.shape[2]
    if lay is not None:
        assert n_q == n_k == lay.n_alloc, 'gathered layout: q/k/v must carry n_alloc rows per head'
        n_q = n_k = lay.n
    sm = spec.static_mask
    return _lib.AttnFwdParams(batch=b, heads=h, n_q=n_q, n_k=n_k, dim_head=dh, dtype=dt_code(q.dtype), pattern=spec.pattern,
                              causal=int(spec.causal), stable=int(spec.stable), text_len=spec.text_len, fmap=spec.fmap,
                              kernel_size=spec.kernel_size, dilation=spec.dilation, gather=int(lay is not None), kv_rows=kv_rows,
                              key_mask=_p(key_mask),
                              static_mask=_p(sm), static_ld=(sm.shape[1] if sm is not None else 0),
                              q=_p(_c(q)), k=_p(_c(k)), v=_p(_c(v)), out=_p(out), lse=_p(lse))


def attn_fwd(spec, q, k, v, key_mask=None, lay=None, n_k=None):
    b, h, n_q, dh = q.shape
    if lay is not None:
        n_q = lay.n
    out = torch.empty(b, n_q, h * dh, device=q.device, dtype=q.dtype)
    lse = torch.empty(b, h, lay.n_stat if lay is not None else n_q, device=q.device, dtype=torch.float32)
    P = _attn_params(spec, q, k, v, out, lse, key_mask, lay, n_k)
    _lib.check(_lib.lib().dalle_b200_attn_fwd(ctypes.byref(P), _stream()), 'attn_fwd')
    _count()
    return out, lse


def attn_dout_buffer(lay, rows, inner, device, dtype):
    if lay is not None and lay.pad_dout:
        return torch.empty(rows + 1, inner, device=device, dtype=dtype)[:rows]
    return torch.empty(rows, inner, device=device, dtype=dtype)


def attn_bwd(spec, q, k, v, out, lse, d_out, cos_t, sin_t, q_scale, key_mask=None, lay=None):
    b, h, n, dh = q.shape
    if lay is not None:
        n = lay.n
        if lay.pad_dout:
            assert d_out.untyped_storage().nbytes() - d_out.storage_offset() * d_out.element_size() >= (b * n + 1) * h * dh * d_out.element_size(), \
                'column gather: d_out needs one spare row (ops.attn_dout_buffer)'
    dqkv = torch.empty(b * n, 3 * h * dh, device=q.device, dtype=q.dtype)
    delta = torch.empty(b, h, lay.n_stat if lay is not None else n, device=q.device, dtype=torch.float32)
    P = _lib.AttnBwdParams(f=_attn_params(spec, q, k, v, out, lse, key_mask, lay), d_out=_p(_c(d_out)), cos_t=_p(cos_t), sin_t=_p(sin_t),
                           q_scale=q_scale, delta=_p(delta), dqkv=_p(dqkv))
    _lib.check(_lib.lib().dalle_b200_attn_bwd(ctypes.byref(P), _stream()), 'attn_bwd')
    _count(3)
    return dqkv


def scale_bwd(d_out, y, scale, sign, dtype, want_dscale=True, want_dbias=True, zeroed=None):
    M, d = d_out.shape
    dy = torch.empty(M, d, device=d_out.device, dtype=dtype)
    if zeroed is not None:
        dscale = zeroed[0] if (want_dscale and scale is not None) else None
        dbias = zeroed[1] if want_dbias else None
    else:
        dscale = torch.zeros(d, device=d_out.device, dtype=torch.float32) if (want_dscale and scale is not None) else None
        dbias = torch.zeros(d, device=d_out.device, dtype=torch.float32) if want_dbias else None
    P = _lib.ScaleBwdParams(rows=M, d=d, dtype=dt_code(dtype), sign=sign, d_out=_p(_c(d_out)), y=_p(y), scale=_p(scale), dy=_p(dy),
                            dscale=_p(dscale), dbias=_p(dbias))
    _lib.check(_lib.lib().dalle_b200_scale_bwd(ctypes.byref(P), _stream()), 'scale_bwd')
    _count()
    return dy, dscale, dbias


def geglu_bwd(dh, u, want_dbias=True, zeroed=None):
    M, H = dh.shape
    du = torch.empty_like(u)
    db = (zeroed if zeroed is not None else torch.zeros(2 * H, device=dh.device, dtype=torch.float32)) if want_dbias else None
    _lib.check(_lib.lib().dalle_b200_geglu_bwd(_p(_c(dh)), _p(_c(u)), _p(du), _p(db), dt_code(dh.dtype), M, H, _stream()), 'geglu_bwd')
    _count()
    return du, db


def ce_fwd(logits, labels, coef, loss_acc):
    R, V = logits.shape
    lse = torch.empty(R, device=logits.device, dtype=torch.float32)
    _lib.check(_lib.lib().dalle_b200_ce_fwd(_p(_c(logits)), dt_code(logits.dtype), R, V, _p(_c(labels)), coef, _p(lse), _p(loss_acc), _stream()), 'ce_fwd')
    _count()
    return lse


def ce_bwd_(logits, labels, coef, row_lse, upstream):
    R, V = logits.shape
    _lib.check(_lib.lib().dalle_b200_ce_bwd(_p(_c(logits)), dt_code(logits.dtype), R, V, _p(_c(labels)), coef, _p(row_lse), _p(upstream), _stream()), 'ce_bwd')
    _count()
    return logits


def colsum(x):
    rows, cols = x.shape
    out = torch.zeros(cols, device=x.device, dtype=torch.float32)
    _lib.check(_lib.lib().dalle_b200_colsum(_p(_c(x)), dt_code(x.dtype), rows, cols, _p(out), _stream()), 'colsum')
    _count()
    return out


def mc_add(src, mc_ptr, scale):
    src = _c(src)
    assert src.dtype == torch.float32
    _lib.check(_lib.lib().dalle_b200_mc_add(_p(src), ctypes.c_void_p(mc_ptr), src.numel(), scale, _stream()), 'mc_add')
    _count()


def cast_bf16(src):
    src = _c(src)
    assert src.dtype == torch.float32
    dst = torch.empty(src.shape, device=src.device, dtype=torch.bfloat16)
    _lib.check(_lib.lib().dalle_b200_cast_bf16(_p(src), _p(dst), src.numel(), _stream()), 'cast_bf16')
    _count()
    return dst


def embed_fwd(ids, weight, out, seg_off):
    B, L = ids.shape
    _, n, d = out.shape
    _lib.check(_lib.lib().dalle_b200_embed_fwd(_p(_c(ids)), _p(_c(weight)), _p(out), B, L, n, seg_off, d, weight.shape[0], _stream()), 'embed_fwd')
    _count()


def embed_bwd(ids, d_out, dweight, seg_off):
    B, L = ids.shape
    _, n, d = d_out.shape
    _lib.check(_lib.lib().dalle_b200_embed_bwd(_p(_c(ids)), _p(_c(d_out)), _p(dweight), B, L, n, seg_off, d, dweight.shape[0], _stream()), 'embed_bwd')
    _count()


def sumsq_(x, out):
    _lib.check(_lib.lib().dalle_b200_sumsq(_p(_c(x)), x.numel(), _p(out), _stream()), 'sumsq')
    _count()


def adam_(p, g, m, v, step, lr, beta1, beta2, eps, weight_decay=0.0, max_norm=0.0, gnorm_sq=None):
    for t in (p, g, m, v):
        assert t.is_cuda and t.dtype == torch.float32 and t.is_contiguous() and t.numel() == p.numel()
    P = _lib.AdamParams(p=_p(p), g=_p(g), m=_p(m), v=_p(v), count=p.numel(), lr=lr, beta1=beta1, beta2=beta2, eps=eps,
                        weight_decay=weight_decay, step=step, max_norm=max_norm, gnorm_sq=_p(gnorm_sq))
    _lib.check(_lib.lib().dalle_b200_adam(ctypes.byref(P), _stream()), 'adam')
    _count()


def axpby(a, b, alpha):
    _c(a), _c(b)
    y = torch.empty_like(a)
    _lib.check(_lib.lib().dalle_b200_axpby(_p(a), _p(b), alpha, _p(y), a.numel(), _stream()), 'axpby')
    _count()
    return y
```

include/dalle_b200.h:

```cpp
#ifndef DALLE_B200_H
#define DALLE_B200_H

#include <stddef.h>
#include <stdint.h>

#ifdef __cplusplus
extern "C" {
#endif

#define DALLE_B200_VERSION 112

typedef enum {
  DB200_OK = 0,
  DB200_ERR_BAD_ARG = -1,
  DB200_ERR_UNSUPPORTED = -2,
  DB200_ERR_CUDA = -3,
  DB200_ERR_NO_DEVICE = -4
} db200_status;

typedef enum { DB200_F32 = 0, DB200_BF16 = 1 } db200_dtype;

typedef enum {
  DB200_ATTN_FULL = 0,
  DB200_ATTN_AXIAL_ROW = 1,
  DB200_ATTN_AXIAL_COL = 2,
  DB200_ATTN_CONV_LIKE = 3,
  DB200_ATTN_STATIC = 4
} db200_attn_pattern;

typedef enum {
  DB200_EPI_STORE = 0,
  DB200_EPI_QKV = 1,
  DB200_EPI_RESID = 2,
  DB200_EPI_GEGLU = 3,
  DB200_EPI_GEGLU_BWD = 4
} db200_epilogue;

typedef enum { DB200_GEMM_AUTO = 0, DB200_GEMM_SIMT = 1, DB200_GEMM_TCGEN05 = 2, DB200_GEMM_SMALLM = 3 } db200_gemm_backend;

int dalle_b200_version(void);
const char* dalle_b200_last_error(void);
int dalle_b200_device_ok(int dev);
int dalle_b200_abi_sizes(int* out, int capacity);

typedef struct {
  int batch, n, d;
  int text_len, fmap;
  int do_ln, do_shift;
  int out_dtype;
  float eps;
  const float* x;
  const float* gamma;
  const float* beta;
  void* out;
  float* mean;
  float* rstd;
} db200_ln_shift_fwd_params;
int dalle_b200_ln_shift_fwd(const db200_ln_shift_fwd_params* p, void* stream);

typedef struct {
  int batch, n, d;
  int text_len, fmap;
  int do_ln, do_shift;
  int dout_dtype;
  const void* d_out;
  const float* x;
  const float* mean;
  const float* rstd;
  const float* gamma;
  const float* dres;
  float* dx;
  float* dgamma;
  float* dbeta;
  const void* up_y;
  const float* up_scale;
  float up_sign;
  void* up_dy;
  float* up_dscale;
  float* up_dbias;
} db200_ln_shift_bwd_params;
int dalle_b200_ln_shift_bwd(const db200_ln_shift_bwd_params* p, void* stream);

typedef struct {
  int M, N, K;
  int dtype;
  int backend;
  const void* A; int64_t lda; int a_mn_major;
  const void* B; int64_t ldb; int b_mn_major;
  int epilogue;
  void* C; int64_t ldc; int c_dtype; const float* bias;
  int split_k_ok;
  void* C_multicast;
  float c_scale;
  void* q; void* k; void* v;
  const float* cos_t; const float* sin_t;
  int seq_n, heads, dim_head, pos_offset;
  float q_scale;
  const float* resid; const float* scale; float sign; void* y_out; float* out;
  void* u_out; void* h_out; int hidden;
  const void* u_in; void* du_out;
} db200_gemm_params;
int dalle_b200_gemm(const db200_gemm_params* p, void* stream);
int dalle_b200_gemm_select(const db200_gemm_params* p);

typedef struct {
  int batch, heads, n_q, n_k, dim_head;
  int dtype;
  int pattern;
  int causal;
  int stable;
  int text_len, fmap;
  int kernel_size, dilation;
  int gather;
  int kv_rows;
  const uint8_t* key_mask;
  const uint8_t* static_mask; int64_t static_ld;
  const void* q; const void* k; const void* v;
  void* out;
  float* lse;
} db200_attn_fwd_params;
int dalle_b200_attn_fwd(const db200_attn_fwd_params* p, void* stream);

typedef struct {
  db200_attn_fwd_params f;
  const void* d_out;
  const float* cos_t; const float* sin_t; float q_scale;
  float* delta;
  void* dqkv;
} db200_attn_bwd_params;
int dalle_b200_attn_bwd(const db200_attn_bwd_params* p, void* stream);

typedef struct {
  int rows, d;
  int dtype;
  float sign;
  const float* d_out;
  const void* y;
  const float* scale;
  void* dy;
  float* dscale;
  float* dbias;
} db200_scale_bwd_params;
int dalle_b200_scale_bwd(const db200_scale_bwd_params* p, void* stream);

int dalle_b200_colsum(const void* x, int dtype, int rows, int cols, float* out, void* stream);

int dalle_b200_qkv_rotary(const void* qkv, void* q, void* k, void* v, const float* cos_t, const float* sin_t, int dtype, int rows, int seq_n,
                          int heads, int dim_head, int pos_offset, float q_scale, int n_alloc, void* stream);

int dalle_b200_geglu_bwd(const void* dh, const void* u, void* du, float* dbias, int dtype, int rows, int hidden, void* stream);

int dalle_b200_ce_fwd(const void* logits, int dtype, int rows, int vocab, const int64_t* labels, float coef, float* row_lse, float* loss_acc,
                      void* stream);
int dalle_b200_ce_bwd(void* logits, int dtype, int rows, int vocab, const int64_t* labels, float coef, const float* row_lse, const float* upstream,
                      void* stream);

int dalle_b200_split_bf16x3(const float* src, void* dst, int64_t rows, int cols, int concat_rows, int operand, void* stream);
int dalle_b200_resid_scale(const void* y, int dtype, const float* resid, const float* scale, float sign, float* out, int64_t rows, int d, void* stream);
int dalle_b200_sample_topk_gumbel(const void* logits, int dtype, int rows, int vocab, int64_t ld, int k, float temperature, const float* gumbel,
                                  uint64_t seed, uint64_t offset, int64_t* out, void* stream);
int dalle_b200_sample_guided_topk_gumbel(const void* cond, const void* null_logits, int dtype, int rows, int vocab, int64_t ld, float cond_scale, int k,
                                         float temperature, const float* gumbel, uint64_t seed, uint64_t offset, int64_t* out, void* stream);
int dalle_b200_decode_shift(const float* h, void* y, int out_dtype, int batch, int d, float* ring_top, float* ring_left, const int64_t* pos,
                            int text_len, int fmap, void* stream);
int dalle_b200_decode_kv_append(const void* k_new, const void* v_new, void* k_cache, void* v_cache, int dtype, int batch_heads, int dim_head,
                                int kv_rows, const int64_t* pos, void* stream);

int dalle_b200_dropout(const void* x, void* y, int dtype, int64_t count, float p, uint64_t seed, uint64_t offset, void* stream);
int dalle_b200_geglu_fwd(const float* u, float* h, int64_t rows, int hidden, void* stream);

int dalle_b200_mc_add(const float* src, void* mc_dst, int64_t count, float scale, void* stream);

int dalle_b200_cast_bf16(const float* src, void* dst, int64_t count, void* stream);

int dalle_b200_axpby(const float* a, const float* b, float alpha, float* y, int64_t count, void* stream);

int dalle_b200_embed_fwd(const int64_t* ids, const float* weight, float* out, int batch, int seg_len, int n, int seg_off, int d, int vocab,
                         void* stream);
int dalle_b200_embed_bwd(const int64_t* ids, const float* d_out, float* dweight, int batch, int seg_len, int n, int seg_off, int d, int vocab,
                         void* stream);

int dalle_b200_sumsq(const float* x, int64_t count, float* out, void* stream);
typedef struct {
  float* p; const float* g; float* m; float* v;
  int64_t count;
  float lr, beta1, beta2, eps, weight_decay;
  int step;
  float max_norm;
  const float* gnorm_sq;
} db200_adam_params;
int dalle_b200_adam(const db200_adam_params* p, void* stream);

int dalle_b200_debug_attn_timeline(long long* out, int count);

#ifdef __cplusplus
}
#endif
#endif
```

Before: 538,000.

## Fuse GEGLU backward and bias-gradient colsum into tcgen05 GEMM epilogue with TMA-staged u

```diff
diff --git a/dalle_pytorch_b200/_lib.py b/dalle_pytorch_b200/_lib.py
--- a/dalle_pytorch_b200/_lib.py
+++ b/dalle_pytorch_b200/_lib.py
@@ -41,7 +41,8 @@
                 ('q', c_void_p), ('k', c_void_p), ('v', c_void_p), ('cos_t', c_void_p), ('sin_t', c_void_p),
                 ('seq_n', c_int), ('heads', c_int), ('dim_head', c_int), ('pos_offset', c_int), ('q_scale', c_float),
                 ('resid', c_void_p), ('scale', c_void_p), ('sign', c_float), ('y_out', c_void_p), ('out', c_void_p),
-                ('u_out', c_void_p), ('h_out', c_void_p), ('hidden', c_int), ('u_in', c_void_p), ('du_out', c_void_p)]
+                ('u_out', c_void_p), ('h_out', c_void_p), ('hidden', c_int), ('u_in', c_void_p), ('du_out', c_void_p),
+                ('dbias', c_void_p)]
 
 
 class AttnFwdParams(ctypes.Structure):
diff --git a/dalle_pytorch_b200/csrc/api.cu b/dalle_pytorch_b200/csrc/api.cu
--- a/dalle_pytorch_b200/csrc/api.cu
+++ b/dalle_pytorch_b200/csrc/api.cu
@@ -200,6 +200,8 @@
       backend = gemm_tcgen05_supported(*p, &why) ? DB200_GEMM_TCGEN05 : DB200_GEMM_SIMT;
     }
   }
+  if (p->epilogue == DB200_EPI_GEGLU_BWD && p->dbias && backend != DB200_GEMM_TCGEN05)
+    return set_error(DB200_ERR_UNSUPPORTED, "gemm/GEGLU_BWD: the bias gradient is formed by the tcgen05 kernel only (shape / alignment did not qualify)");
   if (p->C_multicast && backend != DB200_GEMM_TCGEN05)
     return set_error(DB200_ERR_UNSUPPORTED, "gemm/STORE: the multicast reduction is implemented by the tcgen05 kernel only (shape / alignment did not qualify)");
   if (backend == DB200_GEMM_TCGEN05) {
diff --git a/dalle_pytorch_b200/csrc/common.cuh b/dalle_pytorch_b200/csrc/common.cuh
--- a/dalle_pytorch_b200/csrc/common.cuh
+++ b/dalle_pytorch_b200/csrc/common.cuh
@@ -123,6 +123,27 @@
   dgelu = fma2(mul2(g, splat2(0.39894228040143267794f)), ex, cdf);
 }
 
+__device__ __forceinline__ void gelu_fast_x2(float2 g, float2& gelu, float2& dgelu) {
+  const float2 x = mul2(g, splat2(0.70710678118654752440f));
+  const float2 ax = make_float2(fabsf(x.x), fabsf(x.y));
+  const float2 den = fma2(ax, splat2(0.3275911f), splat2(1.0f));
+  float2 t, ex;
+  asm("rcp.approx.ftz.f32 %0, %1;" : "=f"(t.x) : "f"(den.x));
+  asm("rcp.approx.ftz.f32 %0, %1;" : "=f"(t.y) : "f"(den.y));
+  const float2 q = mul2(mul2(ax, ax), splat2(-1.4426950408889634f));
+  asm("ex2.approx.ftz.f32 %0, %1;" : "=f"(ex.x) : "f"(q.x));
+  asm("ex2.approx.ftz.f32 %0, %1;" : "=f"(ex.y) : "f"(q.y));
+  float2 poly = fma2(t, splat2(1.061405429f), splat2(-1.453152027f));
+  poly = fma2(t, poly, splat2(1.421413741f));
+  poly = fma2(t, poly, splat2(-0.284496736f));
+  poly = fma2(t, poly, splat2(0.254829592f));
+  const float2 erf_abs = fma2(mul2(poly, t), make_float2(-ex.x, -ex.y), splat2(1.0f));
+  const float2 cs = make_float2(copysignf(erf_abs.x, x.x), copysignf(erf_abs.y, x.y));
+  const float2 cdf = fma2(cs, splat2(0.5f), splat2(0.5f));
+  gelu = mul2(g, cdf);
+  dgelu = fma2(mul2(g, splat2(0.39894228040143267794f)), ex, cdf);
+}
+
 template <typename T> __device__ __forceinline__ void gelu_pair(float g, float& gelu, float& dgelu);
 template <> __device__ __forceinline__ void gelu_pair<float>(float g, float& gelu, float& dgelu) { gelu = gelu_erf(g); dgelu = gelu_erf_grad(g); }
 template <> __device__ __forceinline__ void gelu_pair<__nv_bfloat16>(float g, float& gelu, float& dgelu) { gelu_fast(g, gelu, dgelu); }
diff --git a/dalle_pytorch_b200/csrc/epilogue.cuh b/dalle_pytorch_b200/csrc/epilogue.cuh
--- a/dalle_pytorch_b200/csrc/epilogue.cuh
+++ b/dalle_pytorch_b200/csrc/epilogue.cuh
@@ -14,7 +14,7 @@
   void* q; void* k; void* v; const float* cos_t; const float* sin_t;
   int seq_n, heads, dim_head, pos_offset; float q_scale;
   const float* resid; const float* scale; float sign; void* y_out; float* out;
-  void* u_out; void* h_out; int hidden; const void* u_in; void* du_out;
+  void* u_out; void* h_out; int hidden; const void* u_in; void* du_out; float* du_colsum;
 };
 
 inline EpiArgs make_epi_args(const db200_gemm_params& p) {
@@ -27,7 +27,7 @@
   e.q = p.q; e.k = p.k; e.v = p.v; e.cos_t = p.cos_t; e.sin_t = p.sin_t;
   e.seq_n = p.seq_n; e.heads = p.heads; e.dim_head = p.dim_head; e.pos_offset = p.pos_offset; e.q_scale = p.q_scale;
   e.resid = p.resid; e.scale = p.scale; e.sign = p.sign; e.y_out = p.y_out; e.out = p.out;
-  e.u_out = p.u_out; e.h_out = p.h_out; e.hidden = p.hidden; e.u_in = p.u_in; e.du_out = p.du_out;
+  e.u_out = p.u_out; e.h_out = p.h_out; e.hidden = p.hidden; e.u_in = p.u_in; e.du_out = p.du_out; e.du_colsum = p.dbias;
   return e;
 }
 
@@ -335,21 +335,6 @@
       v[i] = r + s * v[i];
     }
     Vec8<float>::store(e.out + off, v);
-  } else if constexpr (EPI == DB200_EPI_GEGLU_BWD) {
-    const T* u = reinterpret_cast<const T*>(e.u_in) + (long long)m * (2 * e.hidden);
-    float a[8], g[8], da[8], dg[8];
-    Vec8<T>::load(u + n, a);
-    Vec8<T>::load(u + e.hidden + n, g);
-#pragma unroll
-    for (int i = 0; i < 8; ++i) {
-      float f, df;
-      gelu_pair<T>(g[i], f, df);
-      da[i] = v[i] * f;
-      dg[i] = v[i] * a[i] * df;
-    }
-    T* du = reinterpret_cast<T*>(e.du_out) + (long long)m * (2 * e.hidden);
-    Vec8<T>::store(du + n, da);
-    Vec8<T>::store(du + e.hidden + n, dg);
   }
 }
 
@@ -447,30 +432,6 @@
       }
       p += 2;
     }
-  } else if constexpr (EPI == DB200_EPI_GEGLU_BWD) {
-    float2 a[16], g[16];
-#pragma unroll
-    for (int it = 0; it < 16; ++it) {
-      const int m = mbase + 2 * it;
-      a[it] = make_float2(0.f, 0.f); g[it] = make_float2(0.f, 0.f);
-      if (m < M) {
-        const T* u = reinterpret_cast<const T*>(e.u_in) + (long long)m * (2 * e.hidden);
-        a[it] = load2<T>(u + n);
-        g[it] = load2<T>(u + e.hidden + n);
-      }
-    }
-#pragma unroll
-    for (int it = 0; it < 16; ++it) {
-      const int m = mbase + 2 * it;
-      if (m < M) {
-        float f0, f1, df0, df1;
-        gelu_pair<T>(g[it].x, f0, df0);
-        gelu_pair<T>(g[it].y, f1, df1);
-        T* du = reinterpret_cast<T*>(e.du_out) + (long long)m * (2 * e.hidden);
-        store2<T>(du + n, t[2 * it] * f0, t[2 * it + 1] * f1);
-        store2<T>(du + e.hidden + n, t[2 * it] * a[it].x * df0, t[2 * it + 1] * a[it].y * df1);
-      }
-    }
   }
 }
 
diff --git a/dalle_pytorch_b200/csrc/gemm_tcgen05.cu b/dalle_pytorch_b200/csrc/gemm_tcgen05.cu
--- a/dalle_pytorch_b200/csrc/gemm_tcgen05.cu
+++ b/dalle_pytorch_b200/csrc/gemm_tcgen05.cu
@@ -42,15 +42,23 @@
   }
 }
 
-template <int BLOCK_N>
+constexpr int U_SLOTS = 2;
+constexpr int U_HALF_BYTES = 32 * 32 * 2;
+constexpr int U_SLOT_BYTES = 2 * U_HALF_BYTES;
+constexpr int SMEM_BUDGET_STAGED = 144 * 1024;
+
+template <int BLOCK_N, bool STAGED_U>
 struct SmemLayout {
   static constexpr int B_STAGE_BYTES = BLOCK_N * BLOCK_K * 2;
   static constexpr int STAGE_BYTES = A_STAGE_BYTES + B_STAGE_BYTES;
-  static constexpr int STAGES = (SMEM_BUDGET / STAGE_BYTES) > 8 ? 8 : (SMEM_BUDGET / STAGE_BYTES);
-  static constexpr int BAR_BYTES = (2 * STAGES + 4 + 2 * SCHED_DEPTH) * 8 + 16 + SCHED_DEPTH * 4 + 12;
+  static constexpr int BUDGET = STAGED_U ? SMEM_BUDGET_STAGED : SMEM_BUDGET;
+  static constexpr int STAGES = (BUDGET / STAGE_BYTES) > 8 ? 8 : (BUDGET / STAGE_BYTES);
+  static constexpr int U_BARS = STAGED_U ? NUM_EPI_WARPS * U_SLOTS : 0;
+  static constexpr int BAR_BYTES = (2 * STAGES + 4 + 2 * SCHED_DEPTH + U_BARS) * 8 + 16 + SCHED_DEPTH * 4 + 12;
   static constexpr int EPI_OFFSET = STAGES * STAGE_BYTES;
-  static constexpr int BAR_OFFSET = EPI_OFFSET + NUM_EPI_WARPS * EPI_STAGE_BYTES;
+  static constexpr int BAR_OFFSET = EPI_OFFSET + NUM_EPI_WARPS * (STAGED_U ? U_SLOTS * U_SLOT_BYTES : EPI_STAGE_BYTES);
   static constexpr int TOTAL = BAR_OFFSET + BAR_BYTES + 1024;
+  static_assert(TOTAL <= 227 * 1024, "shared memory");
 };
 
 constexpr int SCHED_SLOTS = 256;
@@ -60,8 +68,9 @@
 template <int BLOCK_N, int EPI, bool A_MN, bool B_MN, bool EPI_COLS>
 __global__ void __launch_bounds__(NUM_THREADS, 1)
 gemm_tcgen05_kernel(const __grid_constant__ CUtensorMap tmA, const __grid_constant__ CUtensorMap tmB, const __grid_constant__ CUtensorMap tmC,
-                    int M, int N, int K, int k_splits, int sched_slot, EpiArgs e) {
-  using L = SmemLayout<BLOCK_N>;
+                    const __grid_constant__ CUtensorMap tmU, int M, int N, int K, int k_splits, int sched_slot, EpiArgs e) {
+  constexpr bool STAGED_U = EPI == DB200_EPI_GEGLU_BWD;
+  using L = SmemLayout<BLOCK_N, STAGED_U>;
   constexpr int STAGES = L::STAGES;
   constexpr int B_STAGE_BYTES = L::B_STAGE_BYTES;
   constexpr uint32_t TMEM_COLS = 2 * BLOCK_N;
@@ -79,7 +88,8 @@
   const uint32_t tempty_bar = smem_u32(bars + 2 * STAGES + 2);
   const uint32_t sfull_bar = smem_u32(bars + 2 * STAGES + 4);
   const uint32_t sempty_bar = smem_u32(bars + 2 * STAGES + 4 + SCHED_DEPTH);
-  uint32_t* tmem_slot = reinterpret_cast<uint32_t*>(bars + 2 * STAGES + 4 + 2 * SCHED_DEPTH);
+  const uint32_t ufull_bar = smem_u32(bars + 2 * STAGES + 4 + 2 * SCHED_DEPTH);
+  uint32_t* tmem_slot = reinterpret_cast<uint32_t*>(bars + 2 * STAGES + 4 + 2 * SCHED_DEPTH + L::U_BARS);
   volatile int* sched_tile = reinterpret_cast<volatile int*>(tmem_slot + 4);
 
   const int warp = threadIdx.x >> 5, lane = threadIdx.x & 31;
@@ -94,6 +104,8 @@
     for (int s = 0; s < STAGES; ++s) { mbar_init(full_bar + 8 * s, 1); mbar_init(empty_bar + 8 * s, 1); }
     for (int s = 0; s < 2; ++s) { mbar_init(tfull_bar + 8 * s, 1); mbar_init(tempty_bar + 8 * s, NUM_EPI_WARPS * 32); }
     for (int s = 0; s < SCHED_DEPTH; ++s) { mbar_init(sfull_bar + 8 * s, 1); mbar_init(sempty_bar + 8 * s, 1 + NUM_EPI_WARPS); }
+    for (int s = 0; s < L::U_BARS; ++s) mbar_init(ufull_bar + 8 * s, 1);
+    if (STAGED_U) { tma_prefetch_desc(&tmU); tma_prefetch_desc(&tmC); }
     asm volatile("fence.mbarrier_init.release.cluster;" ::: "memory");
   }
   if (warp == 1) {
@@ -218,21 +230,145 @@
     const int lrow = lane >> 4, lcol = (lane & 15) << 1;
     int as = 0; uint32_t aph = 0;
     int ss = 0; uint32_t sph = 0;
-    while (true) {
+    constexpr int UCH = (BLOCK_N / 2) / 32;
+    const uint32_t uslots = smem_u32(smem + L::EPI_OFFSET + ew * U_SLOTS * U_SLOT_BYTES);
+    const uint32_t ubar = ufull_bar + 8 * ew * U_SLOTS;
+    uint32_t uq = 0;
+    auto load_u = [&](uint32_t q, int col, int row) {
+      const uint32_t s = q % U_SLOTS, dst = uslots + s * U_SLOT_BYTES, bar = ubar + 8 * s;
+      mbar_expect_tx(bar, U_SLOT_BYTES);
+      tma_load_3d(dst, &tmU, bar, col, 0, row);
+      tma_load_3d(dst + U_HALF_BYTES, &tmU, bar, col, 1, row);
+    };
+    auto take_tile = [&]() {
       mbar_wait(sfull_bar + 8 * ss, sph);
-      const int tile = sched_tile[ss];
+      const int t = sched_tile[ss];
       __syncwarp();
       if (lane == 0) mbar_arrive(sempty_bar + 8 * ss);
       if (++ss == SCHED_DEPTH) { ss = 0; sph ^= 1; }
+      return t;
+    };
+    auto u_tile = [&](int t, int& row, int& col, int from) {
+      if (t >= num_tiles) return 0;
+      const int tmn = t % num_mn;
+      row = (tmn / num_n) * BLOCK_M + quarter * 32;
+      col = (tmn % num_n) * BLOCK_N + half * (BLOCK_N / 2);
+      const int n = (row < M && col < N) ? min(UCH, (N - col + 31) / 32) : 0;
+      if (lane == 0) {
+        for (int c = from; c < n; ++c) {
+          tma_prefetch_l2_3d(&tmU, col + c * 32, 0, row);
+          tma_prefetch_l2_3d(&tmU, col + c * 32, 1, row);
+        }
+      }
+      return n;
+    };
+    int next_tile = -1, next_issued = 0, next_row = 0, next_col = 0, next_nch = 0;
+    while (true) {
+      int tile, issued = 0;
+      if (STAGED_U && next_tile >= 0) {
+        tile = next_tile; issued = next_issued;
+        next_tile = -1; next_issued = 0;
+      } else {
+        tile = take_tile();
+      }
       if (tile >= num_tiles) break;
       const int mn = tile % num_mn;
       const int m0 = (mn / num_n) * BLOCK_M;
       const int n0 = (mn % num_n) * BLOCK_N;
       const int mbase = m0 + quarter * 32 + lrow;
+      int urow = 0, ucol = 0, nch = 0;
+      if constexpr (STAGED_U) {
+        if (issued == 0) nch = u_tile(tile, urow, ucol, U_SLOTS);
+        else { urow = next_row; ucol = next_col; nch = next_nch; }
+        if (issued < min(nch, U_SLOTS)) {
+          if (lane == 0) {
+            bulk_wait_group_read0();
+            for (int c = issued; c < min(nch, U_SLOTS); ++c) load_u(uq + c, ucol + c * 32, urow);
+          }
+          __syncwarp();
+        }
+      }
       mbar_wait(tfull_bar + 8 * as, aph);
       tc_fence_after();
       const uint32_t taddr = tmem_base + (static_cast<uint32_t>(quarter * 32) << 16) + as * BLOCK_N;
-      if (e.atomic_c == 4) {
+      if constexpr (STAGED_U) {
+        next_tile = take_tile();
+        next_nch = u_tile(next_tile, next_row, next_col, 0);
+        for (int c = 0; c < nch; ++c) {
+          const uint32_t q = uq + c, s = q % U_SLOTS;
+          const uint32_t sa = uslots + s * U_SLOT_BYTES, sg = sa + U_HALF_BYTES;
+          uint32_t r[32];
+          tmem_ld32(taddr + half * (BLOCK_N / 2) + c * 32, r);
+          mbar_wait(ubar + 8 * s, (q / U_SLOTS) & 1);
+          tmem_ld_wait();
+          float da[32], dg[32];
+#pragma unroll
+          for (int k = 0; k < 4; ++k) {
+            const uint32_t off = lane * 64 + ((k ^ ((lane >> 1) & 3)) << 4);
+            uint32_t av[4], gv[4];
+            asm volatile("ld.shared.v4.b32 {%0, %1, %2, %3}, [%4];" : "=r"(av[0]), "=r"(av[1]), "=r"(av[2]), "=r"(av[3]) : "r"(sa + off) : "memory");
+            asm volatile("ld.shared.v4.b32 {%0, %1, %2, %3}, [%4];" : "=r"(gv[0]), "=r"(gv[1]), "=r"(gv[2]), "=r"(gv[3]) : "r"(sg + off) : "memory");
+            uint32_t wa[4], wg[4];
+#pragma unroll
+            for (int i = 0; i < 4; ++i) {
+              const float2 a2 = __bfloat1622float2(*reinterpret_cast<const __nv_bfloat162*>(&av[i]));
+              const float2 g2 = __bfloat1622float2(*reinterpret_cast<const __nv_bfloat162*>(&gv[i]));
+              const float2 d2 = __bfloat1622float2(__floats2bfloat162_rn(__uint_as_float(r[8 * k + 2 * i]), __uint_as_float(r[8 * k + 2 * i + 1])));
+              float2 f, df;
+              gelu_fast_x2(g2, f, df);
+              const float2 da2 = mul2(d2, f), dg2 = mul2(mul2(d2, a2), df);
+              const int x = 8 * k + 2 * i;
+              da[x] = da2.x; da[x + 1] = da2.y;
+              dg[x] = dg2.x; dg[x + 1] = dg2.y;
+              const __nv_bfloat162 pa = __floats2bfloat162_rn(da2.x, da2.y), pg = __floats2bfloat162_rn(dg2.x, dg2.y);
+              wa[i] = *reinterpret_cast<const uint32_t*>(&pa);
+              wg[i] = *reinterpret_cast<const uint32_t*>(&pg);
+            }
+            asm volatile("st.shared.v4.b32 [%0], {%1, %2, %3, %4};" ::"r"(sa + off), "r"(wa[0]), "r"(wa[1]), "r"(wa[2]), "r"(wa[3]) : "memory");
+            asm volatile("st.shared.v4.b32 [%0], {%1, %2, %3, %4};" ::"r"(sg + off), "r"(wg[0]), "r"(wg[1]), "r"(wg[2]), "r"(wg[3]) : "memory");
+          }
+          fence_proxy_async();
+          __syncwarp();
+          if (lane == 0) {
+            tma_store_3d(&tmC, sa, ucol + c * 32, 0, urow);
+            tma_store_3d(&tmC, sg, ucol + c * 32, 1, urow);
+            bulk_commit_group();
+          }
+          if (c + U_SLOTS < nch) {
+            if (lane == 0) {
+              bulk_wait_group_read0();
+              load_u(q + U_SLOTS, ucol + (c + U_SLOTS) * 32, urow);
+            }
+            __syncwarp();
+          } else {
+            const int kn = c + U_SLOTS - nch;
+            if (kn == next_issued && kn < next_nch) {
+              if (lane == 0) {
+                bulk_wait_group_read0();
+                load_u(q + U_SLOTS, next_col + kn * 32, next_row);
+              }
+              __syncwarp();
+              next_issued = kn + 1;
+            }
+          }
+          if (e.du_colsum) {
+#pragma unroll
+            for (int o = 16; o >= 1; o >>= 1) {
+              const bool hi = (lane & o) != 0;
+#pragma unroll
+              for (int i = 0; i < o; ++i) {
+                const float sa_ = hi ? da[i] : da[i + o], sg_ = hi ? dg[i] : dg[i + o];
+                const float ka = hi ? da[i + o] : da[i], kg = hi ? dg[i + o] : dg[i];
+                da[i] = ka + __shfl_xor_sync(0xffffffffu, sa_, o);
+                dg[i] = kg + __shfl_xor_sync(0xffffffffu, sg_, o);
+              }
+            }
+            const int j = ucol + c * 32 + lane;
+            if (j < N) { atomicAdd(e.du_colsum + j, da[0]); atomicAdd(e.du_colsum + N + j, dg[0]); }
+          }
+        }
+        uq += nch;
+      } else if (e.atomic_c == 4) {
       } else if (EPI == DB200_EPI_STORE && !EPI_COLS && e.tma_store) {
         constexpr int NCH = (BLOCK_N / 2) / 32;
         const uint32_t stage_u32 = smem_u32(stage);
@@ -376,7 +512,7 @@
       mbar_arrive(tempty_bar + 8 * as);
       if (++as == 2) { as = 0; aph ^= 1; }
     }
-    if (EPI == DB200_EPI_STORE && !EPI_COLS && e.tma_store && lane == 0) bulk_wait_group0();
+    if (((EPI == DB200_EPI_STORE && !EPI_COLS && e.tma_store) || STAGED_U) && lane == 0) bulk_wait_group0();
   }
 
   tc_fence_before();
@@ -395,7 +531,7 @@
 
 template <int BLOCK_N, int EPI, bool A_MN, bool B_MN, bool EPI_COLS>
 int launch_cfg_mode(const db200_gemm_params& p, cudaStream_t st) {
-  using L = SmemLayout<BLOCK_N>;
+  using L = SmemLayout<BLOCK_N, EPI == DB200_EPI_GEGLU_BWD>;
   CUtensorMap tmA, tmB;
   int rc;
   if (!A_MN) rc = make_tensor_map_bf16(&tmA, p.A, p.K, p.M, p.lda, BLOCK_K, BLOCK_M);
@@ -404,12 +540,19 @@
   if (!B_MN) rc = make_tensor_map_bf16(&tmB, p.B, p.K, p.N, p.ldb, BLOCK_K, 128);
   else rc = make_tensor_map_bf16(&tmB, p.B, p.N, p.K, p.ldb, 64, BLOCK_K);
   if (rc) return rc;
-  CUtensorMap tmC = tmA;
+  CUtensorMap tmC = tmA, tmU = tmA;
   EpiArgs e = make_epi_args(p);
   if (EPI == DB200_EPI_STORE && !EPI_COLS && e.atomic_c == 0 && p.c_dtype == DB200_BF16 && !p.split_k_ok && al16(p.C) && (p.ldc % 8) == 0 &&
       tma_store_env()) {
     if ((rc = make_tensor_map_bf16(&tmC, p.C, p.N, p.M, p.ldc, 64, 32))) return rc;
     e.tma_store = 1;
+  }
+  if (EPI == DB200_EPI_GEGLU_BWD) {
+    const uint64_t dims[3] = {static_cast<uint64_t>(p.hidden), 2, static_cast<uint64_t>(p.M)};
+    const uint64_t strides[3] = {1, static_cast<uint64_t>(p.hidden), 2 * static_cast<uint64_t>(p.hidden)};
+    const uint32_t box[3] = {32, 1, 32};
+    if ((rc = make_tensor_map_bf16_nd(&tmU, p.u_in, 3, dims, strides, box, CU_TENSOR_MAP_SWIZZLE_64B))) return rc;
+    if ((rc = make_tensor_map_bf16_nd(&tmC, p.du_out, 3, dims, strides, box, CU_TENSOR_MAP_SWIZZLE_64B))) return rc;
   }
   auto kern = gemm_tcgen05_kernel<BLOCK_N, EPI, A_MN, B_MN, EPI_COLS>;
   static std::atomic<bool> attr_done{false};
@@ -431,7 +574,7 @@
   if (e.atomic_c < 2) e.atomic_c = k_splits > 1;
   static const bool static_sched = [] { const char* v = std::getenv("DALLE_B200_SCHED"); return v && !std::strcmp(v, "static"); }();
   const int sched_slot = static_sched ? -1 : static_cast<int>(g_launch_seq.fetch_add(1, std::memory_order_relaxed) % SCHED_SLOTS);
-  DB200_CUDA_OK(launch_pdl(kern, dim3(grid), dim3(NUM_THREADS), L::TOTAL, st, tmA, tmB, tmC, p.M, p.N, p.K, k_splits, sched_slot, e));
+  DB200_CUDA_OK(launch_pdl(kern, dim3(grid), dim3(NUM_THREADS), L::TOTAL, st, tmA, tmB, tmC, tmU, p.M, p.N, p.K, k_splits, sched_slot, e));
   DB200_LAUNCH_OK("gemm_tcgen05_kernel");
   return DB200_OK;
 }
@@ -449,7 +592,9 @@
   const int env = epi_mode_env();
   const bool cols = env == 2 || (env == 0 && EPI == DB200_EPI_RESID) ||
                     (EPI == DB200_EPI_STORE && p.C_multicast != nullptr);
-  if (cols) return launch_cfg_mode<BLOCK_N, EPI, A_MN, B_MN, true>(p, st);
+  if constexpr (EPI != DB200_EPI_GEGLU_BWD) {
+    if (cols) return launch_cfg_mode<BLOCK_N, EPI, A_MN, B_MN, true>(p, st);
+  }
   return launch_cfg_mode<BLOCK_N, EPI, A_MN, B_MN, false>(p, st);
 }
 
@@ -513,7 +658,7 @@
 }
 
 int make_tensor_map_bf16_nd_impl(CUtensorMap* map, const void* base, int rank, const uint64_t* dims, const uint64_t* strides_elems,
-                                 const uint32_t* box) {
+                                 const uint32_t* box, CUtensorMapSwizzle swizzle) {
   EncodeTiledFn fn = get_encode_fn();
   if (!fn) return set_error(DB200_ERR_NO_DEVICE, "cuTensorMapEncodeTiled entry point not available");
   if (rank < 2 || rank > 5) return set_error(DB200_ERR_BAD_ARG, "tensor map rank %d", rank);
@@ -522,7 +667,7 @@
   for (int i = 0; i < rank; ++i) { gdim[i] = dims[i]; bx[i] = box[i]; estr[i] = 1; }
   for (int i = 1; i < rank; ++i) gstride[i - 1] = strides_elems[i] * 2;
   const CUresult r = fn(map, CU_TENSOR_MAP_DATA_TYPE_BFLOAT16, rank, const_cast<void*>(base), gdim, gstride, bx, estr,
-                        CU_TENSOR_MAP_INTERLEAVE_NONE, CU_TENSOR_MAP_SWIZZLE_128B, CU_TENSOR_MAP_L2_PROMOTION_L2_256B,
+                        CU_TENSOR_MAP_INTERLEAVE_NONE, swizzle, CU_TENSOR_MAP_L2_PROMOTION_L2_256B,
                         CU_TENSOR_MAP_FLOAT_OOB_FILL_NONE);
   if (r != CUDA_SUCCESS) return set_error(DB200_ERR_CUDA, "cuTensorMapEncodeTiled (rank %d) failed with CUresult %d", rank, (int)r);
   return DB200_OK;
@@ -536,8 +681,8 @@
   return make_tensor_map_bf16_impl(map, base, inner, outer, ld, box_inner, box_outer);
 }
 int make_tensor_map_bf16_nd(CUtensorMap* map, const void* base, int rank, const uint64_t* dims, const uint64_t* strides_elems,
-                            const uint32_t* box) {
-  return make_tensor_map_bf16_nd_impl(map, base, rank, dims, strides_elems, box);
+                            const uint32_t* box, CUtensorMapSwizzle swizzle) {
+  return make_tensor_map_bf16_nd_impl(map, base, rank, dims, strides_elems, box, swizzle);
 }
 }
 
@@ -572,7 +717,7 @@
         break;
       case DB200_EPI_GEGLU_BWD:
         if (p.a_mn_major) w = "GEGLU_BWD expects K-major A";
-        else if (!al16(p.u_in) || !al16(p.du_out) || p.hidden % 8) w = "GEGLU_BWD tensor alignment";
+        else if (!al16(p.u_in) || !al16(p.du_out) || p.hidden % 8 || (p.dbias && !al16(p.dbias))) w = "GEGLU_BWD tensor alignment";
         break;
       default: w = "unknown epilogue";
     }
diff --git a/dalle_pytorch_b200/csrc/tc_common.cuh b/dalle_pytorch_b200/csrc/tc_common.cuh
--- a/dalle_pytorch_b200/csrc/tc_common.cuh
+++ b/dalle_pytorch_b200/csrc/tc_common.cuh
@@ -63,6 +63,15 @@
       "l"(map), "r"(bar), "r"(c0), "r"(c1)
       : "memory");
 }
+__device__ __forceinline__ void tma_load_3d(uint32_t dst, const CUtensorMap* map, uint32_t bar, int c0, int c1, int c2) {
+  asm volatile(
+      "cp.async.bulk.tensor.3d.shared::cluster.global.mbarrier::complete_tx::bytes [%0], [%1, {%3, %4, %5}], [%2];" ::"r"(dst),
+      "l"(map), "r"(bar), "r"(c0), "r"(c1), "r"(c2)
+      : "memory");
+}
+__device__ __forceinline__ void tma_prefetch_l2_3d(const CUtensorMap* map, int c0, int c1, int c2) {
+  asm volatile("cp.async.bulk.prefetch.tensor.3d.L2.global.tile [%0, {%1, %2, %3}];" ::"l"(map), "r"(c0), "r"(c1), "r"(c2) : "memory");
+}
 __device__ __forceinline__ void tma_load_4d(uint32_t dst, const CUtensorMap* map, uint32_t bar, int c0, int c1, int c2, int c3) {
   asm volatile(
       "cp.async.bulk.tensor.4d.shared::cluster.global.mbarrier::complete_tx::bytes [%0], [%1, {%3, %4, %5, %6}], [%2];" ::"r"(dst),
@@ -77,6 +86,10 @@
 }
 __device__ __forceinline__ void tma_store_2d(const CUtensorMap* map, uint32_t src, int c0, int c1) {
   asm volatile("cp.async.bulk.tensor.2d.global.shared::cta.bulk_group [%0, {%2, %3}], [%1];" ::"l"(map), "r"(src), "r"(c0), "r"(c1) : "memory");
+}
+__device__ __forceinline__ void tma_store_3d(const CUtensorMap* map, uint32_t src, int c0, int c1, int c2) {
+  asm volatile("cp.async.bulk.tensor.3d.global.shared::cta.bulk_group [%0, {%2, %3, %4}], [%1];" ::"l"(map), "r"(src), "r"(c0), "r"(c1), "r"(c2)
+               : "memory");
 }
 __device__ __forceinline__ void bulk_commit_group() { asm volatile("cp.async.bulk.commit_group;" ::: "memory"); }
 __device__ __forceinline__ void bulk_wait_group_read0() { asm volatile("cp.async.bulk.wait_group.read 0;" ::: "memory"); }
@@ -194,7 +207,7 @@
 int make_tensor_map_bf16(CUtensorMap* map, const void* base, uint64_t inner, uint64_t outer, uint64_t ld, uint32_t box_inner,
                          uint32_t box_outer);
 int make_tensor_map_bf16_nd(CUtensorMap* map, const void* base, int rank, const uint64_t* dims, const uint64_t* strides_elems,
-                            const uint32_t* box);
-
-}
-}
+                            const uint32_t* box, CUtensorMapSwizzle swizzle = CU_TENSOR_MAP_SWIZZLE_128B);
+
+}
+}
diff --git a/dalle_pytorch_b200/functional.py b/dalle_pytorch_b200/functional.py
--- a/dalle_pytorch_b200/functional.py
+++ b/dalle_pytorch_b200/functional.py
@@ -6,7 +6,6 @@
 from . import ops
 
 
-FUSE_GEGLU_BWD = False
 FUSE_UPSTREAM_SCALE_BWD = os.environ.get('DALLE_B200_FUSE_SCALE_BWD', '1') != '0'
 
 
@@ -221,9 +220,9 @@
         dy, dscale, db2 = pre
     else:
         dy, dscale, db2 = ops.scale_bwd(d_out, y, sc, sign, g.dtype, zeroed=(pool[:d], pool[d:2 * d]))
-    if FUSE_GEGLU_BWD:
-        du = ops.gemm_geglu_bwd(dy, w2c, u)
-        db1 = ops.colsum(du)
+    if drop is None and g.dtype == torch.bfloat16:
+        db1 = pool[6 * d:]
+        du = ops.gemm_geglu_bwd(dy, w2c, u, dbias=db1)
     else:
         dh = ops.gemm_store(dy, w2c, a_mn=False, b_mn=True)
         if drop is not None:
diff --git a/dalle_pytorch_b200/ops.py b/dalle_pytorch_b200/ops.py
--- a/dalle_pytorch_b200/ops.py
+++ b/dalle_pytorch_b200/ops.py
@@ -368,13 +368,16 @@
     return h, u
 
 
-def gemm_geglu_bwd(dy, W2, u, backend=GEMM_AUTO):
+def gemm_geglu_bwd(dy, W2, u, backend=GEMM_AUTO, dbias=None):
     _c(dy), _c(W2), _c(u)
     M, K = dy.shape
     H = W2.shape[1]
     du = torch.empty_like(u)
     P = _base(M, H, K, dy, K, False, W2, H, True, EPI_GEGLU_BWD, backend)
     P.u_in, P.du_out, P.hidden = _p(u), _p(du), H
+    if dbias is not None:
+        assert dbias.shape == (2 * H,) and dbias.dtype == torch.float32 and dbias.is_contiguous()
+        P.dbias = _p(dbias)
     _gemm(P)
     return du
 
diff --git a/include/dalle_b200.h b/include/dalle_b200.h
--- a/include/dalle_b200.h
+++ b/include/dalle_b200.h
@@ -99,6 +99,7 @@
   const float* resid; const float* scale; float sign; void* y_out; float* out;
   void* u_out; void* h_out; int hidden;
   const void* u_in; void* du_out;
+  float* dbias;
 } db200_gemm_params;
 int dalle_b200_gemm(const db200_gemm_params* p, void* stream);
 int dalle_b200_gemm_select(const db200_gemm_params* p);
```

Measured after the change: 554,400 (median of 6 runs). +3.1%, better.
